# lisvulaczo/lodestar

Hardware: AMD Instinct MI355X
Metric: BLS signature sets verified/sec (whole node) at 1/2/4/8 MI355X; p50 batch latency (higher is better)
Workload: dtype u32

## Files before the change

include/lodestar_bls.h:

```cpp
#ifndef LODESTAR_BLS_H
#define LODESTAR_BLS_H

#include <stddef.h>
#include <stdint.h>

#ifdef __cplusplus
extern "C" {
#endif

#define LSG_OK 0
#define LSG_ERR_INVALID_ARG 1
#define LSG_ERR_NO_DEVICE 2
#define LSG_ERR_DEVICE 3
#define LSG_ERR_NOMEM 4
#define LSG_ERR_CLOSED 5
#define LSG_ERR_BUSY 6
#define LSG_ERR_ENTROPY 7

#define LSG_BLST_SUCCESS 0
#define LSG_BLST_BAD_ENCODING 1
#define LSG_BLST_POINT_NOT_ON_CURVE 2
#define LSG_BLST_POINT_NOT_IN_GROUP 3
#define LSG_BLST_AGGR_TYPE_MISMATCH 4
#define LSG_BLST_VERIFY_FAIL 5
// ... 98 lines not shown
int lsg_final_verify(lsg_ctx* ctx, const uint8_t* partials576, size_t n_partials, int32_t* valid);
int lsg_final_submit(lsg_ctx* ctx, const uint8_t* partials576, size_t n_partials, lsg_ticket* ticket);
int lsg_final_submit_device(lsg_ctx* ctx, const void* dev_partials576, size_t n_partials, lsg_ticket* ticket);
int lsg_final_wait(lsg_ctx* ctx, lsg_ticket ticket, int32_t* valid);
int lsg_final_submit_groups(lsg_ctx* ctx, const uint8_t* partials576, size_t n_groups, size_t per_group,
                            lsg_ticket* ticket);
int lsg_final_wait_groups(lsg_ctx* ctx, lsg_ticket ticket, int32_t* valid );

int lsg_pubkey_table_set(lsg_ctx* ctx, size_t first_index, const uint8_t* pks, uint32_t pk_len, size_t n,
                         int32_t* err);
int lsg_pubkey_table_size(lsg_ctx* ctx, size_t* n);

int lsg_committees_set(lsg_ctx* ctx, uint32_t first_id, const uint32_t* indices,
                       const uint32_t* offsets , size_t n_committees,
                       int32_t* err );
int lsg_committees_clear(lsg_ctx* ctx, uint32_t first_id, size_t n);
int lsg_committee_count(lsg_ctx* ctx, size_t* n);

typedef struct {
  uint64_t lookups, hits, pending, inserts, evictions, bypassed, full;
  uint32_t entries, capacity;
} lsg_msg_cache_stats;
int lsg_msg_cache_set(lsg_ctx* ctx, size_t capacity);
int lsg_msg_cache_clear(lsg_ctx* ctx);
int lsg_msg_cache_get_stats(lsg_ctx* ctx, lsg_msg_cache_stats* out);

int lsg_pubkey_validate(lsg_ctx* ctx, const uint8_t* pks, uint32_t pk_len, size_t n, uint8_t* out96, int32_t* err);

int lsg_aggregate_signatures(lsg_ctx* ctx, const uint8_t* sigs, uint32_t sig_len, const uint32_t* offsets,
                             size_t n_groups, uint8_t* out96, int32_t* err);

int lsg_signing_roots(lsg_ctx* ctx, const uint8_t* roots32, size_t n, const uint8_t* domain32, uint32_t domain_stride,
                      uint8_t* out32);
int lsg_attestation_signing_roots(lsg_ctx* ctx, const uint8_t* data128, size_t n, const uint8_t* domain32,
                                  uint32_t domain_stride, uint8_t* out32);
int lsg_deposit_signing_roots(lsg_ctx* ctx, const uint8_t* msgs88, size_t n, const uint8_t* domain32,
                              uint32_t domain_stride, uint8_t* out32);
int lsg_object_signing_roots(lsg_ctx* ctx, const uint8_t* objs, uint32_t obj_len, size_t n, const uint8_t* domain32,
                             uint32_t domain_stride, uint8_t* out32);

int lsg_verify_deposits(lsg_ctx* ctx, const uint8_t* data184, size_t n, const uint8_t* domain32, uint64_t seed,
                        uint8_t* valid, int32_t* err);

int lsg_sign(lsg_ctx* ctx, const uint8_t* sks32, const uint8_t* msgs, uint32_t msg_len, size_t n, uint8_t* out96);
int lsg_sk_to_pk(lsg_ctx* ctx, const uint8_t* sks32, size_t n, uint8_t* out96);

int lsg_check_fp2_mul(lsg_ctx* ctx, const uint32_t* in, size_t n, uint32_t* out);
int lsg_check_fp_sqr(lsg_ctx* ctx, const uint32_t* in, size_t n, uint32_t* out);
int lsg_check_fp2_sqr(lsg_ctx* ctx, const uint32_t* in, size_t n, uint32_t* out);
int lsg_check_sums(lsg_ctx* ctx, const uint32_t* in, size_t n, uint32_t* out);
int lsg_check_fp2_lanes(lsg_ctx* ctx, const uint32_t* in, size_t n, uint32_t* out);
int lsg_check_g2_lanes(lsg_ctx* ctx, const uint32_t* in, size_t n, uint32_t* out);
int lsg_check_mf_lanes(lsg_ctx* ctx, const uint32_t* in, size_t n, uint32_t* out);
int lsg_check_canon(lsg_ctx* ctx, const uint32_t* in, size_t n, const uint8_t* bytes48, size_t nb, uint32_t* out,
                    uint32_t* out_limbs);
int lsg_check_fp2_roots(lsg_ctx* ctx, const uint32_t* in, size_t n, uint32_t* out);
int lsg_check_batch_inv(lsg_ctx* ctx, const uint32_t* in, size_t n, uint32_t* out);
int lsg_check_map_uniform(lsg_ctx* ctx, const uint8_t* ub256, size_t n, uint8_t* out192);
int lsg_check_batch_partial_rnd(lsg_ctx* ctx, const lsg_set* sets, size_t n_sets,
                                const uint64_t* rnd , uint8_t* out576,
                                int32_t* set_err, int32_t* any_error);

int lsg_probe_fp_mul_rate(lsg_ctx* ctx, double* fp_mul_per_s, double* mad_per_s);

int lsg_probe_mad_peak(lsg_ctx* ctx, double* mad_per_s);

int lsg_last_kernel_times(lsg_ctx* ctx, const char** names, double* ms, int max);

#ifdef __cplusplus
}
#endif
#endif
```

lodestar_amd/_native.py:

```python
import ctypes
import os
import struct
import threading

HERE = os.path.dirname(os.path.abspath(__file__))
LIB_PATH = os.environ.get("LSG_LIB", os.path.join(HERE, "liblodestar_bls.so"))
AB_LIB_PATH = os.path.join(HERE, "liblodestar_bls_ab.so")

LSG_OK = 0
LSG_ERR_INVALID_ARG = 1
LSG_ERR_NO_DEVICE = 2
LSG_ERR_BUSY = 6
LSG_ERR_ENTROPY = 7

LSG_INVALID = 0
LSG_VALID = 1
LSG_ERROR = 2

LSG_JOB_BATCHABLE = 1
LSG_JOB_PRIORITY = 2
LSG_JOB_VALIDATE_KEYS = 4

BLST_NAMES = {
    0: "BLST_SUCCESS", 1: "BLST_BAD_ENCODING", 2: "BLST_POINT_NOT_ON_CURVE", 3: "BLST_POINT_NOT_IN_GROUP",
# ... 98 lines not shown
def _msg_form(msg):
    if isinstance(msg, MsgObject):
        b = msg.tobytes()
        return b, len(b) | LSG_MSG_OBJECT
    return msg, len(msg)


class LsgSet(ctypes.Structure):
    _fields_ = [
        ("pks", ctypes.c_void_p), ("pk_len", ctypes.c_uint32), ("n_pks", ctypes.c_uint32),
        ("msg", ctypes.c_void_p), ("msg_len", ctypes.c_uint32),
        ("sig", ctypes.c_void_p), ("sig_len", ctypes.c_uint32),
    ]


class LsgJob(ctypes.Structure):
    _fields_ = [("sets", ctypes.POINTER(LsgSet)), ("n_sets", ctypes.c_uint32), ("flags", ctypes.c_uint32)]


class LsgJobResult(ctypes.Structure):
    _fields_ = [("status", ctypes.c_int32), ("err_code", ctypes.c_int32)]


class LsgStats(ctypes.Structure):
    _fields_ = [
        ("batch_retries", ctypes.c_uint32), ("batch_sigs_success", ctypes.c_uint32),
        ("start_ns", ctypes.c_uint64), ("end_ns", ctypes.c_uint64),
        ("n_final_exps", ctypes.c_uint32), ("submit_us", ctypes.c_uint32),
        ("key_error", ctypes.c_int32), ("key_error_job", ctypes.c_uint32),
    ]


class LsgMsgCacheStats(ctypes.Structure):
    _fields_ = [(k, ctypes.c_uint64) for k in ("lookups", "hits", "pending", "inserts", "evictions", "bypassed",
                                                "full")] + [("entries", ctypes.c_uint32), ("capacity", ctypes.c_uint32)]


_lib = None
_lib_lock = threading.Lock()

EXPORTS = [
    "lsg_init", "lsg_init_devices", "lsg_destroy", "lsg_device_count", "lsg_last_error", "lsg_device_name",
    "lsg_reserve", "lsg_allocation_count", "lsg_verify_jobs", "lsg_verify_sets",
    "lsg_aggregate_pubkeys", "lsg_hash_to_g2", "lsg_sig_decode", "lsg_batch_partial", "lsg_final_verify",
    "lsg_probe_fp_mul_rate", "lsg_last_kernel_times", "lsg_sign", "lsg_sk_to_pk",
    "lsg_submit_jobs", "lsg_wait_jobs", "lsg_wait_jobs_node", "lsg_jobs_partial", "lsg_assign_jobs", "lsg_poll",
    "lsg_final_submit", "lsg_final_wait", "lsg_pipeline_slots", "lsg_probe_mad_peak",
    "lsg_pubkey_table_set", "lsg_pubkey_table_size", "lsg_pubkey_validate",
    "lsg_final_submit_groups", "lsg_final_wait_groups", "lsg_aggregate_signatures",
    "lsg_signing_roots", "lsg_attestation_signing_roots", "lsg_jobs_partial_device", "lsg_final_submit_device",
    "lsg_set_coalesce", "lsg_aggregate_pubkeys_multi", "lsg_check_fp2_mul",
    "lsg_check_fp_sqr", "lsg_check_fp2_sqr", "lsg_check_sums", "lsg_check_fp2_lanes", "lsg_check_g2_lanes", "lsg_check_mf_lanes",
    "lsg_check_canon", "lsg_check_fp2_roots", "lsg_check_batch_inv", "lsg_check_map_uniform",
    "lsg_check_batch_partial_rnd",
    "lsg_deposit_signing_roots", "lsg_verify_deposits",
    "lsg_committees_set", "lsg_committees_clear", "lsg_committee_count",
    "lsg_object_signing_roots",
    "lsg_submit_jobs_grouped", "lsg_wait_jobs_grouped",
    "lsg_msg_cache_set", "lsg_msg_cache_clear", "lsg_msg_cache_get_stats",
]


def load_library(path=LIB_PATH):
    global _lib
    with _lib_lock:
        if _lib is not None and path == LIB_PATH:
            return _lib
        if not os.path.exists(path):
            raise NativeUnavailable(f"{path} not built (run python -c 'import __graft_entry__; __graft_entry__.build()')")
        lib = ctypes.CDLL(path)
        vp, u32, u64, i32, sz = ctypes.c_void_p, ctypes.c_uint32, ctypes.c_uint64, ctypes.c_int32, ctypes.c_size_t
        pi32 = ctypes.POINTER(ctypes.c_int32)
        lib.lsg_init.argtypes = [ctypes.c_int, ctypes.POINTER(vp)]
        lib.lsg_init_devices.argtypes = [ctypes.POINTER(ctypes.c_int), ctypes.c_int, ctypes.POINTER(vp)]
        lib.lsg_device_count.argtypes = [vp, pi32]
        lib.lsg_reserve.argtypes = [vp, sz, sz, sz, i32]
        lib.lsg_allocation_count.argtypes = [vp, ctypes.POINTER(u64)]
        lib.lsg_wait_jobs_node.argtypes = [vp, u64, i32, ctypes.POINTER(LsgJobResult), ctypes.POINTER(LsgStats)]
        lib.lsg_jobs_partial.argtypes = [vp, u64, ctypes.c_char_p, pi32]
        lib.lsg_jobs_partial_device.argtypes = [vp, u64, vp, pi32]
        lib.lsg_final_submit_device.argtypes = [vp, vp, sz, ctypes.POINTER(u64)]
        lib.lsg_assign_jobs.argtypes = [ctypes.POINTER(u32), sz, i32, pi32]
        lib.lsg_destroy.argtypes = [vp]
        lib.lsg_last_error.argtypes = [vp]
        lib.lsg_last_error.restype = ctypes.c_char_p
        lib.lsg_device_name.argtypes = [vp, ctypes.c_char_p, sz]
        lib.lsg_verify_jobs.argtypes = [vp, ctypes.POINTER(LsgJob), sz, u64, ctypes.POINTER(LsgJobResult),
                                        ctypes.POINTER(LsgStats)]
        lib.lsg_verify_sets.argtypes = [vp, ctypes.POINTER(LsgSet), sz, u64, ctypes.POINTER(LsgJobResult)]
        lib.lsg_aggregate_pubkeys.argtypes = [vp, ctypes.c_char_p, u32, sz, ctypes.c_char_p, pi32]
        lib.lsg_aggregate_pubkeys_multi.argtypes = [vp, ctypes.POINTER(LsgSet), sz, ctypes.c_char_p, pi32]
        lib.lsg_hash_to_g2.argtypes = [vp, ctypes.c_char_p, u32, sz, ctypes.c_char_p, u32, ctypes.c_char_p]
        lib.lsg_sig_decode.argtypes = [vp, ctypes.c_char_p, u32, sz, ctypes.c_char_p, pi32]
        lib.lsg_batch_partial.argtypes = [vp, ctypes.POINTER(LsgSet), sz, u64, ctypes.c_char_p, pi32, pi32]
        lib.lsg_final_verify.argtypes = [vp, ctypes.c_char_p, sz, pi32]
        lib.lsg_probe_fp_mul_rate.argtypes = [vp, ctypes.POINTER(ctypes.c_double), ctypes.POINTER(ctypes.c_double)]
        lib.lsg_last_kernel_times.argtypes = [vp, ctypes.POINTER(ctypes.c_char_p), ctypes.POINTER(ctypes.c_double),
                                              ctypes.c_int]
        lib.lsg_sign.argtypes = [vp, ctypes.c_char_p, ctypes.c_char_p, u32, sz, ctypes.c_char_p]
        lib.lsg_sk_to_pk.argtypes = [vp, ctypes.c_char_p, sz, ctypes.c_char_p]
        pu64 = ctypes.POINTER(u64)
        lib.lsg_submit_jobs.argtypes = [vp, ctypes.POINTER(LsgJob), sz, u64, pu64]
        lib.lsg_wait_jobs.argtypes = [vp, u64, ctypes.POINTER(LsgJobResult), ctypes.POINTER(LsgStats)]
        lib.lsg_submit_jobs_grouped.argtypes = [vp, ctypes.POINTER(LsgJob), sz, u64, ctypes.POINTER(u32), sz, pu64]
        lib.lsg_wait_jobs_grouped.argtypes = [vp, u64, ctypes.POINTER(LsgJobResult), ctypes.POINTER(LsgStats),
                                              ctypes.c_char_p, ctypes.POINTER(u32)]
        lib.lsg_poll.argtypes = [vp, u64, pi32]
        lib.lsg_pubkey_table_set.argtypes = [vp, sz, ctypes.c_char_p, u32, sz, pi32]
        lib.lsg_pubkey_table_size.argtypes = [vp, ctypes.POINTER(sz)]
        lib.lsg_committees_set.argtypes = [vp, u32, ctypes.POINTER(u32), ctypes.POINTER(u32), sz, pi32]
        lib.lsg_committees_clear.argtypes = [vp, u32, sz]
        lib.lsg_committee_count.argtypes = [vp, ctypes.POINTER(sz)]
        lib.lsg_msg_cache_set.argtypes = [vp, sz]
        lib.lsg_msg_cache_clear.argtypes = [vp]
        lib.lsg_msg_cache_get_stats.argtypes = [vp, ctypes.POINTER(LsgMsgCacheStats)]
        lib.lsg_final_submit_groups.argtypes = [vp, ctypes.c_char_p, sz, sz, pu64]
        lib.lsg_final_wait_groups.argtypes = [vp, u64, pi32]
        lib.lsg_pubkey_validate.argtypes = [vp, ctypes.c_char_p, u32, sz, ctypes.c_char_p, pi32]
        lib.lsg_signing_roots.argtypes = [vp, ctypes.c_char_p, sz, ctypes.c_char_p, u32, ctypes.c_char_p]
        lib.lsg_attestation_signing_roots.argtypes = [vp, ctypes.c_char_p, sz, ctypes.c_char_p, u32, ctypes.c_char_p]
        lib.lsg_deposit_signing_roots.argtypes = [vp, ctypes.c_char_p, sz, ctypes.c_char_p, u32, ctypes.c_char_p]
        lib.lsg_object_signing_roots.argtypes = [vp, ctypes.c_char_p, u32, sz, ctypes.c_char_p, u32, ctypes.c_char_p]
        lib.lsg_verify_deposits.argtypes = [vp, ctypes.c_char_p, sz, ctypes.c_char_p, u64, ctypes.c_char_p, pi32]
        lib.lsg_aggregate_signatures.argtypes = [vp, ctypes.c_char_p, u32, ctypes.POINTER(u32), sz,
                                                 ctypes.c_char_p, pi32]
        lib.lsg_final_submit.argtypes = [vp, ctypes.c_char_p, sz, pu64]
        lib.lsg_final_wait.argtypes = [vp, u64, pi32]
        lib.lsg_pipeline_slots.argtypes = [vp, pi32]
        lib.lsg_set_coalesce.argtypes = [vp, u32, i32]
        lib.lsg_check_fp2_mul.argtypes = [vp, ctypes.c_char_p, sz, ctypes.c_char_p]
        lib.lsg_check_fp_sqr.argtypes = [vp, ctypes.c_char_p, sz, ctypes.c_char_p]
        lib.lsg_check_fp2_sqr.argtypes = [vp, ctypes.c_char_p, sz, ctypes.c_char_p]
        lib.lsg_check_sums.argtypes = [vp, ctypes.c_char_p, sz, ctypes.c_char_p]
        lib.lsg_check_fp2_lanes.argtypes = [vp, ctypes.c_char_p, sz, ctypes.c_char_p]
        lib.lsg_check_g2_lanes.argtypes = [vp, ctypes.c_char_p, sz, ctypes.c_char_p]
        lib.lsg_check_mf_lanes.argtypes = [vp, ctypes.c_char_p, sz, ctypes.c_char_p]
        lib.lsg_check_canon.argtypes = [vp, ctypes.c_char_p, sz, ctypes.c_char_p, sz, ctypes.c_char_p, ctypes.c_char_p]
        lib.lsg_check_fp2_roots.argtypes = [vp, ctypes.c_char_p, sz, ctypes.c_char_p]
        lib.lsg_check_batch_inv.argtypes = [vp, ctypes.c_char_p, sz, ctypes.c_char_p]
        lib.lsg_check_map_uniform.argtypes = [vp, ctypes.c_char_p, sz, ctypes.c_char_p]
        lib.lsg_check_batch_partial_rnd.argtypes = [vp, ctypes.POINTER(LsgSet), sz, ctypes.POINTER(u64),
                                                    ctypes.c_char_p, pi32, pi32]
        lib.lsg_probe_mad_peak.argtypes = [vp, ctypes.POINTER(ctypes.c_double)]
        for name in EXPORTS:
            if name != "lsg_last_error":
                getattr(lib, name).restype = ctypes.c_int
        if path == LIB_PATH:
            _lib = lib
        return lib


class SetBuffer:

    def __init__(self, sets):
        self._keep = []
        sets = list(sets)
        self.arr = (LsgSet * max(len(sets), 1))()
        for i, (pks, msg, sig) in enumerate(sets):
            pk_len, n_pks, pkb = _key_form(pks)
            msg, msg_len = _msg_form(msg)
            for b in (pkb, msg, sig):
                self._keep.append(b)
            s = self.arr[i]
            s.pks = ctypes.cast(ctypes.c_char_p(pkb), ctypes.c_void_p) if pkb else None
            s.pk_len = pk_len
            s.n_pks = n_pks
            s.msg = ctypes.cast(ctypes.c_char_p(msg), ctypes.c_void_p) if msg else None
            s.msg_len = msg_len
            s.sig = ctypes.cast(ctypes.c_char_p(sig), ctypes.c_void_p) if sig else None
            s.sig_len = len(sig)
        self.n = len(sets)


def assign_jobs(job_sizes, n_devices):
    lib = load_library()
    n = len(job_sizes)
    sizes = (ctypes.c_uint32 * max(n, 1))(*job_sizes)
    owner = (ctypes.c_int32 * max(n, 1))()
    rc = lib.lsg_assign_jobs(sizes, n, int(n_devices), owner)
    if rc != LSG_OK:
        raise ValueError(f"lsg_assign_jobs failed ({rc})")
    return list(owner[:n])


class PreparedJobs:

    def __init__(self, jobs):
        import numpy as np
        flat = [st for sets, _ in jobs for st in sets]
# ... 447 lines not shown
        out = ctypes.create_string_buffer(96 * len(sks))
        skb = b"".join(int(k).to_bytes(32, "big") for k in sks)
        self._check(self.lib.lsg_sk_to_pk(self.h, skb, len(sks), out), "lsg_sk_to_pk")
        raw = out.raw
        return [raw[96 * i:96 * i + 96] for i in range(len(sks))]

    def check_fp2_mul(self, words):
        n = len(words) // 56
        assert len(words) == 56 * n
        out = ctypes.create_string_buffer(4 * 28 * n)
        src = struct.pack(f"<{len(words)}I", *words)
        self._check(self.lib.lsg_check_fp2_mul(self.h, src, n, out), "lsg_check_fp2_mul")
        return list(struct.unpack(f"<{28 * n}I", out.raw))

    def _check_sqr(self, fn, words, per_item):
        n = len(words) // per_item
        assert len(words) == per_item * n
        out = ctypes.create_string_buffer(4 * per_item * n)
        src = struct.pack(f"<{len(words)}I", *words)
        self._check(getattr(self.lib, fn)(self.h, src, n, out), fn)
        return list(struct.unpack(f"<{per_item * n}I", out.raw))

    def check_fp_sqr(self, words):
        return self._check_sqr("lsg_check_fp_sqr", words, 14)

    def check_fp2_sqr(self, words):
        return self._check_sqr("lsg_check_fp2_sqr", words, 28)

    def check_sums(self, words):
        n = len(words) // (12 * 14)
        assert len(words) == 12 * 14 * n
        out = ctypes.create_string_buffer(4 * 42 * 14 * n)
        src = struct.pack(f"<{len(words)}I", *words)
        self._check(self.lib.lsg_check_sums(self.h, src, n, out), "lsg_check_sums")
        return list(struct.unpack(f"<{42 * 14 * n}I", out.raw))

    def _check_lanes(self, fn, words):
        n = len(words) // (12 * 14)
        assert len(words) == 12 * 14 * n
        out = ctypes.create_string_buffer(4 * 24 * 14 * n)
        src = struct.pack(f"<{len(words)}I", *words)
        self._check(getattr(self.lib, fn)(self.h, src, n, out), fn)
        return list(struct.unpack(f"<{24 * 14 * n}I", out.raw))

    def check_fp2_lanes(self, words):
        return self._check_lanes("lsg_check_fp2_lanes", words)

    def check_g2_lanes(self, words):
        return self._check_lanes("lsg_check_g2_lanes", words)

    def check_mf_lanes(self, words):
        return self._check_lanes("lsg_check_mf_lanes", words)

    def check_canon(self, words, strings=()):
        n, nb = len(words) // 14, len(strings)
        assert len(words) == 14 * n and all(len(b) == 48 for b in strings)
        out = ctypes.create_string_buffer(4 * 54 * max(n, 1))
        limbs = ctypes.create_string_buffer(4 * 14 * max(nb, 1))
        src = struct.pack(f"<{len(words)}I", *words)
        self._check(self.lib.lsg_check_canon(self.h, src, n, b"".join(strings), nb, out, limbs), "lsg_check_canon")
        return (list(struct.unpack(f"<{54 * n}I", out.raw[:4 * 54 * n])),
                list(struct.unpack(f"<{14 * nb}I", limbs.raw[:4 * 14 * nb])))

    def check_fp2_roots(self, words):
        n = len(words) // 28
        assert len(words) == 28 * n
        out = ctypes.create_string_buffer(4 * 58 * n)
        src = struct.pack(f"<{len(words)}I", *words)
        self._check(self.lib.lsg_check_fp2_roots(self.h, src, n, out), "lsg_check_fp2_roots")
        return list(struct.unpack(f"<{58 * n}I", out.raw))

    def check_batch_inv(self, words):
        return self._check_sqr("lsg_check_batch_inv", words, 14)

    def check_map_uniform(self, items):
        n = len(items)
        assert all(len(b) == 256 for b in items)
        if not n:
            return []
        out = ctypes.create_string_buffer(192 * n)
        self._check(self.lib.lsg_check_map_uniform(self.h, b"".join(items), n, out), "lsg_check_map_uniform")
        raw = out.raw
        return [raw[192 * i:192 * i + 192] for i in range(n)]

    def batch_partial_rnd(self, sets, rnd):
        b = SetBuffer(sets)
        assert len(rnd) == b.n
        r = (ctypes.c_uint64 * max(b.n, 1))(*[int(x) for x in rnd])
        out = ctypes.create_string_buffer(576)
        errs = (ctypes.c_int32 * max(b.n, 1))()
        anyerr = ctypes.c_int32()
        self._check(self.lib.lsg_check_batch_partial_rnd(self.h, b.arr, b.n, r, out, errs, ctypes.byref(anyerr)),
                    "lsg_check_batch_partial_rnd")
        return out.raw, [errs[i] for i in range(b.n)], bool(anyerr.value)

    def probe_fp_mul_rate(self):
        a, b = ctypes.c_double(), ctypes.c_double()
        self._check(self.lib.lsg_probe_fp_mul_rate(self.h, ctypes.byref(a), ctypes.byref(b)), "lsg_probe_fp_mul_rate")
        return a.value, b.value

    def last_kernel_times(self, max_entries=1024):
        names = (ctypes.c_char_p * max_entries)()
        ms = (ctypes.c_double * max_entries)()
        n = self.lib.lsg_last_kernel_times(self.h, names, ms, max_entries)
        return [(names[i].decode(), ms[i]) for i in range(n)]
```

lodestar_amd/csrc/lsg_ab.h:

```cpp
#pragma once
#include <stdlib.h>
#include <string.h>

#ifdef LSG_AB
static inline long lsg_ab_long(const char* name, long dflt) {
  const char* e = getenv(name);
  return e ? atol(e) : dflt;
}
static inline bool lsg_ab_str_is(const char* name, const char* v) {
  const char* e = getenv(name);
  return e && strcmp(e, v) == 0;
}
#else
#define lsg_ab_long(name, dflt) ((long)(dflt))
#define lsg_ab_str_is(name, v) false
#endif
```

lodestar_amd/csrc/lsg_curve.hpp:

```cpp
#pragma once
#include "lsg_tower.hpp"

LSG_INL fp_t fadd(const fp_t& a, const fp_t& b) { return fp_add(a, b); }
LSG_INL fp2_t fadd(const fp2_t& a, const fp2_t& b) { return fp2_add(a, b); }
LSG_INL fp_t fsub(const fp_t& a, const fp_t& b) { return fp_sub(a, b); }
LSG_INL fp2_t fsub(const fp2_t& a, const fp2_t& b) { return fp2_sub(a, b); }
LSG_INL fp_t fmul(const fp_t& a, const fp_t& b) { return fp_mul(a, b); }
LSG_INL fp2_t fmul(const fp2_t& a, const fp2_t& b) { return fp2_mul(a, b); }
LSG_INL fp_t fsqr(const fp_t& a) { return fp_sqr(a); }
LSG_INL fp2_t fsqr(const fp2_t& a) { return fp2_sqr(a); }
LSG_INL fp_t fneg(const fp_t& a) { return fp_neg(a); }
LSG_INL fp2_t fneg(const fp2_t& a) { return fp2_neg(a); }
LSG_INL fps_t<1, 0> fsum(const fp_t& a) { return fps(a); }
LSG_INL fp2s_t<1, 0> fsum(const fp2_t& a) { return fp2s(a); }
template <int K, int P, int N>
LSG_INL fps_t<K * P, K * N> fsum_mulk(const fps_t<P, N>& a) { return fps_mulk<K>(a); }
template <int K, int P0, int N0, int P1, int N1>
LSG_INL fp2s_t<K * P0, K * N0, K * P1, K * N1> fsum_mulk(const fp2s_t<P0, N0, P1, N1>& a) { return fp2s_mulk<K>(a); }
template <int K> LSG_INL fp_t fmulk(const fp_t& a) { return fp_mulk<K>(a); }
template <int K> LSG_INL fp2_t fmulk(const fp2_t& a) { return fp2_mulk<K>(a); }
template <class F> LSG_INL F fsub2(const F& a, const F& b, const F& c) { return (fsum(a) - b - c).carry(); }
LSG_INL fp_t fmul_b3(const fp_t& a) { return fp_mul12(a); }
LSG_INL fp2_t fmul_b3(const fp2_t& a) { return fp2_mul_b3(a); }
template <int P0, int N0, int P1, int N1>
// ... 438 lines not shown
  g2p_t r;
  r.X = fp2_mul_fp(p.X, PSI2_CX);
  r.Y = fp2_mul_fp(p.Y, PSI2_CY);
  r.Z = p.Z;
  return r;
}

template <class F = fp2_t, class G>
LSG_INL bool g2_in_group_get(const G& get) {
  if (proj_is_inf(get())) return true;
  const proj_t<F> xp = proj_neg(proj_mul_xabs_get<F>(get));
  return proj_eq(g2_psi(g2_to_pair(get())), g2_to_pair(xp));
}
LSG_BIGFN bool g2_in_group(g2p_t p) {
  return g2_in_group_get([&]() { return p; });
}

LSG_BIGFN bool g1_in_group(g1p_t p) {
  const uint32_t rw[8] = {0x73eda753u, 0x299d7d48u, 0x3339d808u, 0x09a1d805u,
                          0x53bda402u, 0xfffe5bfeu, 0xffffffffu, 0x00000001u};
  g1p_t acc = proj_inf<fp_t>();
#pragma unroll 1
  for (int w = 0; w < 8; w++) {
#pragma unroll 1
    for (int b = 31; b >= 0; b--) {
      acc = g1_dbl(acc);
      if ((rw[w] >> b) & 1u) acc = g1_add(acc, p);
    }
  }
  return proj_is_inf(acc);
}

LSG_INL bool g1_on_curve_aff(const g1a_t& a) {
  fp_t rhs = fp_add(fp_mul(fp_sqr(a.x), a.x), FP_B_G1);
  return fp_eq(fp_sqr(a.y), rhs);
}
LSG_INL bool g2_on_curve_aff(const g2a_t& a) {
  fp2_t rhs = fp2_add(fp2_mul(fp2_sqr(a.x), a.x), FP2_B_G2);
  return fp2_eq(fp2_sqr(a.y), rhs);
}

#ifndef LSG_BLST_SUCCESS
#define LSG_BLST_SUCCESS 0
#define LSG_BLST_BAD_ENCODING 1
#define LSG_BLST_POINT_NOT_ON_CURVE 2
#define LSG_BLST_POINT_NOT_IN_GROUP 3
#define LSG_BLST_AGGR_TYPE_MISMATCH 4
#define LSG_BLST_VERIFY_FAIL 5
#define LSG_BLST_PK_IS_INFINITY 6
#define LSG_BLST_BAD_SCALAR 7
#define LSG_BLST_INVALID_SIZE 10
#endif

LSG_INL int g2_uncompress(g2a_t& out, bool& inf, const uint8_t* in) {
  uint8_t in0 = in[0];
  inf = false;
  if (!(in0 & 0x80)) return LSG_BLST_BAD_ENCODING;
  if (in0 & 0x40) {
    uint32_t acc = in0 & 0x3f;
    for (int i = 1; i < 96; i++) acc |= in[i];
    if (acc == 0) {
      inf = true;
      out.x = fp2_zero();
      out.y = fp2_zero();
      return LSG_BLST_SUCCESS;
    }
    return LSG_BLST_BAD_ENCODING;
  }
  fp_t x1 = fp_from_be48(in);
  x1 = fp_mask_flags(x1);
  fp_t x0 = fp_from_be48(in + 48);
  if (!fp_canon_lt_p(x1) || !fp_canon_lt_p(x0)) return LSG_BLST_BAD_ENCODING;
  fp2_t x = fp2_make(fp_to_mont(x0), fp_to_mont(x1));
  fp2_t rhs = fp2_add(fp2_mul(fp2_sqr(x), x), FP2_B_G2);
  fp2_t y;
  if (!fp2_sqrt(y, rhs)) return LSG_BLST_POINT_NOT_ON_CURVE;
  bool want = (in0 & 0x20) != 0;
  if (fp2_lexi_largest(y) != want) y = fp2_neg(y);
  out.x = x;
  out.y = y;
  if (fp2_is_zero(x)) return LSG_BLST_POINT_NOT_IN_GROUP;
  return LSG_BLST_SUCCESS;
}

LSG_INL int g2_deserialize_uncompressed(g2a_t& out, bool& inf, const uint8_t* in) {
  uint8_t in0 = in[0];
  inf = false;
  if (in0 & 0x80) return LSG_BLST_BAD_ENCODING;
  if (in0 & 0x40) {
    uint32_t acc = in0 & 0x3f;
    for (int i = 1; i < 192; i++) acc |= in[i];
    if (acc == 0) {
      inf = true;
      out.x = fp2_zero();
      out.y = fp2_zero();
      return LSG_BLST_SUCCESS;
    }
    return LSG_BLST_BAD_ENCODING;
  }
  if (in0 & 0x20) return LSG_BLST_BAD_ENCODING;
  fp_t v[4];
  for (int k = 0; k < 4; k++) {
    v[k] = fp_from_be48(in + 48 * k);
    if (k == 0) v[k] = fp_mask_flags(v[k]);
    if (!fp_canon_lt_p(v[k])) return LSG_BLST_BAD_ENCODING;
  }
  out.x = fp2_make(fp_to_mont(v[1]), fp_to_mont(v[0]));
  out.y = fp2_make(fp_to_mont(v[3]), fp_to_mont(v[2]));
  if (!g2_on_curve_aff(out)) return LSG_BLST_POINT_NOT_ON_CURVE;
  if (fp2_is_zero(out.x)) return LSG_BLST_POINT_NOT_IN_GROUP;
  return LSG_BLST_SUCCESS;
}

LSG_INL int g1_deserialize(g1a_t& out, bool& inf, const uint8_t* in, int len) {
  uint8_t in0 = in[0];
  inf = false;
  bool compressed = (in0 & 0x80) != 0;
  if (compressed != (len == 48)) return LSG_BLST_BAD_ENCODING;
  if (in0 & 0x40) {
    uint32_t acc = in0 & 0x3f;
    for (int i = 1; i < len; i++) acc |= in[i];
    if (acc == 0) {
      inf = true;
      out.x = fp_zero();
      out.y = fp_zero();
      return LSG_BLST_SUCCESS;
    }
    return LSG_BLST_BAD_ENCODING;
  }
  if (!compressed && (in0 & 0x20)) return LSG_BLST_BAD_ENCODING;
  fp_t x = fp_from_be48(in);
  x = fp_mask_flags(x);
  if (!fp_canon_lt_p(x)) return LSG_BLST_BAD_ENCODING;
  out.x = fp_to_mont(x);
  if (compressed) {
// ... 49 lines not shown
```

lodestar_amd/csrc/lsg_fp2_lanes.hpp:

```cpp
#pragma once

constexpr int LSG_VL = 14;

#if LSG_PAIR_G == 2
#define LSG_LANES_HIDE(x) asm volatile("" : "+v"(x))
#else
#define LSG_LANES_HIDE(x) ((void)0)
#endif

LSG_PFN void lanes_carry64(int64_t* t) {
#pragma unroll
  for (int j = 0; j < LSG_VL - 1; j++) {
    t[j + 1] += t[j] >> 29;
    t[j] &= (int64_t)LSG_M29;
  }
}
LSG_PFN void lanes_reduce_step(int64_t* t, const uint32_t* p, int i) {
  uint32_t m = ((uint32_t)t[0] * LSG_N0P) & LSG_M29;
  LSG_LANES_HIDE(m);
#pragma unroll
  for (int j = 0; j < LSG_VL; j++) t[j] += (int64_t)(int32_t)m * (int32_t)p[j];
  const int64_t c = t[0] >> 29;
#pragma unroll
  for (int j = 0; j < LSG_VL - 1; j++) t[j] = t[j + 1];
  t[0] += c;
  t[LSG_VL - 1] = 0;
  if (i == 6) lanes_carry64(t);
}
LSG_PFN void lanes_tail(int64_t* t, uint32_t* r) {
  lanes_carry64(t);
#pragma unroll
  for (int j = 0; j < LSG_VL; j++) r[j] = (uint32_t)t[j];
}
template <class OTHER>
LSG_PFN void lanes_sop_pass(uint32_t* r, const uint32_t* P, const uint32_t* Q, const uint32_t* b, const OTHER& other) {
  uint32_t p[LSG_VL];
#pragma unroll
  for (int j = 0; j < LSG_VL; j++) p[j] = LSG_P[j];
  int64_t t[LSG_VL];
#pragma unroll
  for (int j = 0; j < LSG_VL; j++) t[j] = 0;
#pragma unroll
  for (int i = 0; i < LSG_VL; i++) {
    uint32_t bo = b[i], bs = other(i, b[i]);
    LSG_LANES_HIDE(bo);
    LSG_LANES_HIDE(bs);
#pragma unroll
    for (int j = 0; j < LSG_VL; j++) t[j] += (int64_t)(int32_t)P[j] * (int32_t)bo;
#pragma unroll
    for (int j = 0; j < LSG_VL; j++) t[j] += (int64_t)(int32_t)Q[j] * (int32_t)bs;
    lanes_reduce_step(t, p, i);
  }
  lanes_tail(t, r);
}
LSG_PFN void lanes_mul_pass(uint32_t* r, const uint32_t* V, const uint32_t* s) {
  uint32_t p[LSG_VL];
#pragma unroll
  for (int j = 0; j < LSG_VL; j++) p[j] = LSG_P[j];
  int64_t t[LSG_VL];
#pragma unroll
  for (int j = 0; j < LSG_VL; j++) t[j] = 0;
#pragma unroll
  for (int i = 0; i < LSG_VL; i++) {
    uint32_t si = s[i];
    LSG_LANES_HIDE(si);
#pragma unroll
    for (int j = 0; j < LSG_VL; j++) t[j] += (int64_t)(int32_t)V[j] * (int32_t)si;
    lanes_reduce_step(t, p, i);
  }
  lanes_tail(t, r);
}
LSG_PFN void lanes_mul_operand(uint32_t& P, uint32_t& Q, uint32_t own, uint32_t partner, bool odd) {
  P = odd ? partner : own;
  Q = odd ? own : 0u - partner;
}
LSG_PFN void lanes_sqr_operand(uint32_t& V, uint32_t& s, uint32_t own, uint32_t partner, bool odd) {
  V = odd ? own : own + partner;
  s = odd ? partner + partner : own - partner;
}
LSG_PFN uint32_t lanes_xi_operand(uint32_t own, uint32_t partner, bool odd) { return odd ? own + partner : own - partner; }

#if LSG_PAIR_G == 2 && !defined(LSG_NO_FP2_LANES)
#define LSG_FP2_LANES 1
struct fp2v_t {
  uint32_t l[LSG_VL];
};
LSG_PFN bool lanes_odd() { return pair_h() != 0u; }
LSG_PFN uint32_t lanes_swap(uint32_t x) {
  return (uint32_t)__builtin_amdgcn_update_dpp(0, (int)x, 0xB1, 0xf, 0xf, true);
}

typedef uint32_t lanes8_t __attribute__((ext_vector_type(8)));
typedef uint32_t lanes4_t __attribute__((ext_vector_type(4)));
typedef uint32_t lanes2_t __attribute__((ext_vector_type(2)));
#define LSG_LANES_PARAMS(x) lanes8_t x##_a, lanes4_t x##_b, lanes2_t x##_c
#define LSG_LANES_ARGS(v) lanes_pack8(v), lanes_pack4(v), lanes_pack2(v)
#define LSG_LANES_UNPACK(x) lanes_unpack(x##_a, x##_b, x##_c)
LSG_PFN lanes8_t lanes_pack8(const fp2v_t& a) {
  return lanes8_t{a.l[0], a.l[1], a.l[2], a.l[3], a.l[4], a.l[5], a.l[6], a.l[7]};
}
LSG_PFN lanes4_t lanes_pack4(const fp2v_t& a) { return lanes4_t{a.l[8], a.l[9], a.l[10], a.l[11]}; }
LSG_PFN lanes2_t lanes_pack2(const fp2v_t& a) { return lanes2_t{a.l[12], a.l[13]}; }
LSG_PFN fp2v_t lanes_unpack(const lanes8_t& a, const lanes4_t& b, const lanes2_t& c) {
  fp2v_t r;
#pragma unroll
  for (int k = 0; k < 8; k++) r.l[k] = a[k];
#pragma unroll
  for (int k = 0; k < 4; k++) r.l[8 + k] = b[k];
  r.l[12] = c[0];
  r.l[13] = c[1];
  return r;
}

LSG_PLEAF fp2v_t lanes_fp2_mul_v(LSG_LANES_PARAMS(va), LSG_LANES_PARAMS(vb)) {
  const fp2v_t a = LSG_LANES_UNPACK(va), b = LSG_LANES_UNPACK(vb);
  const bool odd = lanes_odd();
  uint32_t P[LSG_VL], Q[LSG_VL];
#pragma unroll
  for (int k = 0; k < LSG_VL; k++) {
    lanes_mul_operand(P[k], Q[k], a.l[k], lanes_swap(a.l[k]), odd);
    LSG_LANES_HIDE(P[k]);
    LSG_LANES_HIDE(Q[k]);
  }
  fp2v_t r;
// ... 198 lines not shown
```

lodestar_amd/csrc/lsg_h2c.hpp:

```cpp
#pragma once
#include "lsg_curve.hpp"

#include "lsg_ssz.hpp"

struct sha256_ctx {
  uint32_t st[8];
  uint32_t blk[16];
  uint32_t n;
  uint32_t total;
};

LSG_INL void sha256_init(sha256_ctx& c) {
  c.st[0] = 0x6a09e667u;
  c.st[1] = 0xbb67ae85u;
  c.st[2] = 0x3c6ef372u;
  c.st[3] = 0xa54ff53au;
  c.st[4] = 0x510e527fu;
  c.st[5] = 0x9b05688cu;
  c.st[6] = 0x1f83d9abu;
  c.st[7] = 0x5be0cd19u;
  for (int i = 0; i < 16; i++) c.blk[i] = 0;
  c.n = 0;
  c.total = 0;
}
// ... 18 lines not shown
  uint32_t bits = c.total * 8;
  sha256_byte(c, 0x80);
  while (c.n != 56) sha256_byte(c, 0);
  c.blk[14] = 0;
  c.blk[15] = bits;
  sha256_compress(c.st, c.blk);
  for (int i = 0; i < 8; i++) out8[i] = c.st[i];
}

LSG_INL void expand_message_xmd_256(uint8_t* out, const uint8_t* msg, uint32_t msg_len, const uint8_t* dst,
                                    uint32_t dst_len) {
  sha256_ctx c;
  uint32_t b0[8], bi[8];
  sha256_init(c);
  for (int i = 0; i < 64; i++) sha256_byte(c, 0);
  sha256_bytes(c, msg, msg_len);
  sha256_byte(c, 1);
  sha256_byte(c, 0);
  sha256_byte(c, 0);
  sha256_bytes(c, dst, dst_len);
  sha256_byte(c, (uint8_t)dst_len);
  sha256_final(c, b0);
  for (int i = 1; i <= 8; i++) {
    sha256_init(c);
    for (int k = 0; k < 8; k++) {
      uint32_t v = (i == 1) ? b0[k] : (b0[k] ^ bi[k]);
      sha256_byte(c, (uint8_t)(v >> 24));
      sha256_byte(c, (uint8_t)(v >> 16));
      sha256_byte(c, (uint8_t)(v >> 8));
      sha256_byte(c, (uint8_t)v);
    }
    sha256_byte(c, (uint8_t)i);
    sha256_bytes(c, dst, dst_len);
    sha256_byte(c, (uint8_t)dst_len);
    sha256_final(c, bi);
    be_words_to_bytes(out + 32 * (i - 1), bi, 8);
  }
}

LSG_INL fp_t fp_from_be64_mod(const uint8_t* b) {
  fp_t lo = fp_from_be_bytes(b + 32, 8);
  fp_t mid = fp_from_be_bytes(b + 16, 4);
  fp_t hi = fp_from_be_bytes(b, 4);
  return fp_add(fp_add(fp_mul(lo, fp_t(FP_R2)), fp_mul(mid, fp_t(FP_R2_SHL256))), fp_mul(hi, fp_t(FP_R3)));
}

LSG_INL fp2_t sswu_tv1(const fp2_t& u) {
  fp2_t zu2 = fp2_mul(SSWU_Z, fp2_sqr(u));
  return fp2_add(fp2_sqr(zu2), zu2);
}
LSG_INL fp2_t fp2_inv_with_norm_inv(const fp2_t& a, const fp_t& ni) {
  return fp2_t(fp_mul(a.c0, ni), fp_neg(fp_mul(a.c1, ni)));
}
LSG_BIGFN g2a_t map_to_curve_sswu_ni(fp2_t u, fp_t ni) {
  fp2_t u2 = fp2_sqr(u);
  fp2_t zu2 = fp2_mul(SSWU_Z, u2);
  fp2_t tv1 = fp2_add(fp2_sqr(zu2), zu2);
  bool exc = fp2_is_zero(tv1);
  fp2_t x1 = fp2_mul(SSWU_MINUS_B_OVER_A, fp2_add(fp2_one(), fp2_inv_with_norm_inv(tv1, ni)));
  x1 = fp2_select(exc, SSWU_B_OVER_ZA, x1);
  fp2_t gx1 = fp2_add(fp2_mul(fp2_add(fp2_sqr(x1), SSWU_A), x1), SSWU_B);
  fp2_t x2 = fp2_mul(zu2, x1);
  fp2_t gx2 = fp2_add(fp2_mul(fp2_add(fp2_sqr(x2), SSWU_A), x2), SSWU_B);
  bool sq1;
  fp_t s1 = fp2_norm_sqrt_candidate(gx1, &sq1);
  fp_t s2 = fp_mul(fp_mul(fp2_norm(zu2), fp2_norm(u)), fp_mul(s1, fp_t(SSWU_NZ_POW_P1D4)));
  g2a_t r;
  r.x = fp2_select(sq1, x1, x2);
  fp2_t y;
  (void)fp2_sqrt_with_norm_root(y, fp2_select(sq1, gx1, gx2), fp_select(sq1, s1, s2));
  if (fp2_sgn0(u) != fp2_sgn0(y)) y = fp2_neg(y);
  r.y = y;
  return r;
}
LSG_BIGFN g2a_t map_to_curve_sswu(fp2_t u) { return map_to_curve_sswu_ni(u, fp_inv(fp2_norm(sswu_tv1(u)))); }

LSG_BIGFN g2p_t iso_map3(g2a_t p) {
  const fp2_t& x = p.x;
  fp2_t xn = fp2_add(fp2_mul(fp2_add(fp2_mul(fp2_add(fp2_mul(ISO_XNUM_3, x), ISO_XNUM_2), x), ISO_XNUM_1), x),
                     ISO_XNUM_0);
  fp2_t xd = fp2_add(fp2_mul(fp2_add(x, ISO_XDEN_1), x), ISO_XDEN_0);
  fp2_t yn = fp2_add(fp2_mul(fp2_add(fp2_mul(fp2_add(fp2_mul(ISO_YNUM_3, x), ISO_YNUM_2), x), ISO_YNUM_1), x),
                     ISO_YNUM_0);
  fp2_t yd = fp2_add(fp2_mul(fp2_add(fp2_mul(fp2_add(x, ISO_YDEN_2), x), ISO_YDEN_1), x), ISO_YDEN_0);
  g2p_t r;
  r.X = fp2_mul(xn, yd);
  r.Y = fp2_mul(fp2_mul(p.y, yn), xd);
  r.Z = fp2_mul(xd, yd);
  if (fp2_is_zero(r.Z)) r = proj_inf<fp2_t>();
  return r;
}

LSG_BIGFN g2p_t clear_cofactor_g2(g2p_t p) {
  const g2p_t u = g2_psi(p);
  g2p_t c = g2_add(g2_psi2(g2_dbl(p)), proj_neg(u));
  c = g2_add(c, proj_neg(p));
  const g2p_t t1 = proj_neg(proj_mul_xabs(p));
  c = g2_add(c, proj_neg(t1));
  const g2p_t t2 = proj_neg(proj_mul_xabs(g2_add(t1, u)));
  return g2_add(c, t2);
}
template <bool LANES = false, class G, class P, class CP, class CG>
LSG_INL g2p_t clear_cofactor_g2_parked(const G& get, const P& put, const CP& cput, const CG& cget) {
  auto xabs = [&]() {
#ifdef LSG_FP2_LANES
    if (LANES) return g2_mul_xabs_get_dbl_lanes(get);
#endif
    return proj_mul_xabs_get<fp2_t>(get);
  };
  cput(proj_neg(xabs()));
  g2p_t c;
  {
    const g2p_t p = get();
    c = g2_add(g2_psi2(g2_dbl(p)), proj_neg(p));
    put(g2_psi(p));
  }
  c = g2_add(c, proj_neg(get()));
  const g2p_t t1 = cget();
  cput(g2_add(c, proj_neg(t1)));
  put(g2_add(t1, get()));
  const g2p_t t2 = proj_neg(xabs());
  return g2_add(cget(), t2);
}
```

lodestar_amd/csrc/lsg_host.hip:

```cpp
#include <hip/hip_runtime.h>
#include <rccl/rccl.h>
#include <stdio.h>
#include <stdlib.h>
#include <errno.h>
#include <string.h>
#include <sys/random.h>
#include <time.h>

#include <algorithm>
#include <atomic>
#include <condition_variable>
#include <chrono>
#include <mutex>
#include <shared_mutex>
#include <thread>
#include <unordered_map>
#include <string>
#include <vector>

#include "../../include/lodestar_bls.h"
#include "lsg_launch.h"
#include "lsg_layout.h"
#include "lsg_serial.h"
#include "lsg_ab.h"
// ... 80 lines not shown
  SLOT_MERGE = 4
};

struct PendingPkg {
  uint64_t serial = 0, seed = 0;
  size_t n_sets = 0;
  std::vector<lsg_job> jobs;
  std::vector<lsg_set> sets;
  std::vector<uint8_t> data;
};
struct MergeTicket {
  int slot = -1;
  int sub = -1;
  int rc = 0;
  std::string err;
};

struct Dev;

constexpr int64_t LSG_ITEMS_PER_BLOCK_HOST = 128;
struct AggPlan {
  bool tree = false;
  int L = 0, T = 1;
  int64_t n_c0 = 0, N0 = 0;
  size_t blk_off = 0, o0_off = 0, len_off = 0, pk0_off = 0, src_off = 0;
};
constexpr size_t AGG_TREE_MIN_KEYS = 32768;

struct Slot : Staged {
  Dev* d = nullptr;
  int index = 0;
  hipStream_t st[2] = {nullptr, nullptr};
  bool own_streams = true;
  hipStream_t st_norm[2] = {nullptr, nullptr}, st_prio[2] = {nullptr, nullptr};
  int cur = 0;
  hipEvent_t ev_xp = nullptr;
  hipEvent_t ev_in = nullptr, ev_sig = nullptr, ev_grp = nullptr, ev_part = nullptr, ev_done = nullptr,
             ev_node = nullptr;
  DevBuf d_sig, d_siglen, d_msg, d_msgoff, d_msglen, d_pk, d_pklen, d_rnd, d_mode, d_dst;
  HostBuf h_arena;
  MsgTable mtab;
  bool mc_ok = false;
  DevBuf d_Hx, d_hinfx;
  SegPlan msum;
  DevBuf d_mmask, d_PmP, d_Pm, d_pinfm, d_errm;
  BitsPlan bplan;
  HostBuf h_cbits;
  DevBuf d_cbits;
  MultiPlan mplan;
  size_t n_kv = 0, kv_off = 0;
  DevBuf d_ub, d_sigaff, d_siginf, d_seterr, d_pkp, d_pkerr, d_agg, d_P, d_pinf, d_H, d_hinf, d_rs, d_rs2, d_fall,
      d_fall2;
  DevBuf d_Pp, d_zP, d_zPi, d_U, d_nrm, d_nrmi, d_Hp, d_zN, d_zNi, d_mid, d_Hm, d_hinfm;
  DevBuf binv_lv[2], binv_iv[2];
  DevBuf d_lines;
  bool rs2_ready = false;
  std::vector<uint8_t> rs2_scaled;
  std::vector<uint8_t> rs_raw;
  DevBuf d_S, d_F, d_verdict, d_Sb, d_fgb, d_Fb, d_bkt, d_bits, d_aux, d_gath, d_nodeF, d_nodeV;
  DevBuf seg_tmp[3][2];
  std::vector<int32_t> plan;
  HostBuf h_plan;
  DevBuf d_plan;
  PhasePlan phA;
  SegPlan pkagg;
  AggPlan agg;
  DevBuf d_agga, d_aggi, d_aggpre, d_aggtot, d_aggflag;
  SegPlan phA_node;
  HostBuf h_mode;
  HostBuf h_err, h_pinf, h_pkerr, h_verdict, h_blob, h_nodeV;
  std::vector<Timer> timers;
  size_t ntimers = 0;
  int kind = SLOT_FREE;
  uint64_t serial = 0;
  GroupPlan gp;
  Switches sw;
  int K = 4;
  std::vector<lsg_job_result> results;
  lsg_stats stats;
  bool has_node = false;
  size_t n_jobs = 0;
  uint64_t seed = 0;
  DevBuf d_xport;
  HostBuf h_xport;
  bool big_fe_pending = false;
  std::vector<uint64_t> sub_serial;
  std::vector<lsg_stats> sub_stats;
  std::vector<int32_t> sub_pkfail;
  std::vector<uint8_t> sub_done;
  bool resolved = false, resolving = false;
  int resolve_rc = LSG_OK;
  size_t grp_n = 0;
  std::vector<uint32_t> set_grp;
  std::vector<int32_t> gplan;
  SigGroupPlan sgp;
  HostBuf h_gplan, h_gagg;
  DevBuf d_gplan, d_gsum, d_gagg, d_gtmp[2];
};

struct Dev {
  lsg_ctx* c = nullptr;
  int device = 0;
  int ord = 0;
  hipStream_t s_util = nullptr;
  hipStream_t s_fe[LSG_FE_STREAMS] = {};
  hipStream_t s_xp = nullptr, s_nfe = nullptr;
// ... 174 lines not shown
hipError_t event_wait(hipEvent_t e) {
  const auto t0 = std::chrono::steady_clock::now();
  for (;;) {
    const hipError_t r = hipEventQuery(e);
    if (r != hipErrorNotReady) return r;
    if (std::chrono::steady_clock::now() - t0 > std::chrono::microseconds(20))
      std::this_thread::sleep_for(std::chrono::microseconds(30));
  }
}

bool blocking_waits() {
  const char* e = getenv("LSG_BLOCKING_WAITS");
  return e && atoi(e) != 0;
}

int slot_create(Dev* d, Slot* s, int index, hipStream_t shared) {
  s->d = d;
  s->index = index;
  if (shared) {
    s->st[0] = s->st[1] = shared;
    s->own_streams = false;
  } else {
    for (int k = 0; k < 2; k++) LSG_HIP(s, hipStreamCreateWithFlags(&s->st_norm[k], hipStreamNonBlocking));
    s->st[0] = s->st_norm[0];
    s->st[1] = s->st_norm[1];
  }
  hipEvent_t* evs[] = {&s->ev_in, &s->ev_sig, &s->ev_grp, &s->ev_part, &s->ev_done, &s->ev_node, &s->ev_xp};
  for (hipEvent_t* e : evs) LSG_HIP(s, hipEventCreateWithFlags(e, hipEventDisableTiming));
  if (blocking_waits()) {
    for (hipEvent_t* e : {&s->ev_part, &s->ev_done}) {
      LSG_HIP(s, hipEventDestroy(*e));
      LSG_HIP(s, hipEventCreateWithFlags(e, hipEventDisableTiming | hipEventBlockingSync));
    }
  }
  LSG_RC(ensure(s, s->d_dst, 256));
  LSG_HIP(s, hipMemcpy(s->d_dst.p, DST_POP, DST_POP_LEN, hipMemcpyHostToDevice));
  return LSG_OK;
}

void slot_destroy(Slot* s) {
  if (!s->d) return;
  for (int k = 0; k < 2; k++)
    if (s->st[k]) (void)hipStreamSynchronize(s->st[k]);
  DevBuf* bufs[] = {&s->d_sig,  &s->d_siglen, &s->d_msg,  &s->d_msgoff, &s->d_msglen, &s->d_pk,    &s->d_pklen,
                    &s->d_rnd,  &s->d_mode,   &s->d_dst,  &s->d_ub,     &s->d_sigaff, &s->d_siginf, &s->d_seterr,
                    &s->d_pkp,  &s->d_pkerr,  &s->d_agg,  &s->d_P,      &s->d_pinf,   &s->d_H,     &s->d_hinf,
                    &s->d_rs,   &s->d_rs2,    &s->d_fall, &s->d_fall2,  &s->d_Pp,     &s->d_zP,    &s->d_zPi,
                    &s->d_U,    &s->d_nrm,    &s->d_nrmi, &s->d_Hp,     &s->d_zN,     &s->d_zNi,   &s->binv_lv[0],
                    &s->binv_lv[1], &s->binv_iv[0], &s->binv_iv[1], &s->d_lines, &s->d_S, &s->d_F, &s->d_verdict,
                    &s->d_Sb,   &s->d_fgb,    &s->d_Fb,   &s->d_bkt,    &s->d_bits,   &s->d_aux,   &s->d_gath,
                    &s->d_nodeF, &s->d_nodeV, &s->d_plan, &s->d_mid, &s->d_Hm, &s->d_hinfm,
                    &s->d_mmask, &s->d_PmP, &s->d_Pm, &s->d_pinfm, &s->d_errm, &s->d_xport,
                    &s->d_agga, &s->d_aggi, &s->d_aggpre, &s->d_aggtot, &s->d_aggflag, &s->d_cbits,
                    &s->d_gplan, &s->d_gsum, &s->d_gagg, &s->d_gtmp[0], &s->d_gtmp[1], &s->d_Hx, &s->d_hinfx};
  for (DevBuf* b : bufs) free_dev(*b);
  for (auto& u : s->seg_tmp)
    for (DevBuf& b : u) free_dev(b);
  HostBuf* hb[] = {&s->h_arena, &s->h_err, &s->h_pinf, &s->h_pkerr, &s->h_verdict, &s->h_blob, &s->h_plan, &s->h_nodeV,
                   &s->h_xport, &s->h_cbits, &s->h_gplan, &s->h_gagg};
  for (HostBuf* b : hb) free_host(*b);
  for (Timer& t : s->timers) {
    (void)hipEventDestroy(t.a);
    (void)hipEventDestroy(t.b);
  }
  s->timers.clear();
  hipEvent_t evs[] = {s->ev_in, s->ev_sig, s->ev_grp, s->ev_part, s->ev_done, s->ev_node, s->ev_xp};
  for (hipEvent_t e : evs)
    if (e) (void)hipEventDestroy(e);
  if (s->own_streams) {
    for (int k = 0; k < 2; k++) {
      if (s->st_prio[k]) (void)hipStreamSynchronize(s->st_prio[k]);
      if (s->st_norm[k]) (void)hipStreamSynchronize(s->st_norm[k]);
    }
    for (int k = 0; k < 2; k++) {
      if (s->st_norm[k]) (void)hipStreamDestroy(s->st_norm[k]);
      s->st_norm[k] = s->st_prio[k] = s->st[k] = nullptr;
    }
  }
  s->d = nullptr;
}

int slot_streams(Slot* s, bool prio) {
  if (!s->own_streams) return LSG_OK;
  if (prio && !s->st_prio[0]) {
    Dev* d = s->d;
    for (int k = 0; k < 2; k++) LSG_RC(prio_stream(d->c, d, &d->s_pp[k]));
    s->st_prio[0] = d->s_pp[0];
    s->st_prio[1] = d->s_pp[1];
  }
  hipStream_t* p = prio ? s->st_prio : s->st_norm;
  s->st[0] = p[0];
  s->st[1] = p[1];
  return LSG_OK;
}

int slot_ready(Dev* d, Slot* s, int index) {
  if (s->d) return LSG_OK;
  const int rc = slot_create(d, s, index, nullptr);
  if (rc) slot_destroy(s);
  return rc;
}

bool miller_fused() { return lsg_ab_long("LSG_MILLER_FUSED", 1) != 0; }
static bool mf_lanes_on() { return lsg_ab_long("LSG_MF_LANES", 1) != 0; }

size_t slp_items_max();
int miller_k_for(size_t n_sets) {
// ... 29 lines not shown
  size_t a, b;
  binv_sizes(n, &a, &b);
  return a;
}
size_t binv_iv_words(size_t n) {
  size_t a, b;
  binv_sizes(n, &a, &b);
  return b;
}

int size_inputs(Slot* s, size_t n, size_t np, size_t mb) {
  const size_t nn = std::max(n, (size_t)1), pp = std::max(np, (size_t)1);
  LSG_RC(ensure_host(s, s->h_arena, stage_layout(n, np, 96, mb).bytes));
  LSG_RC(ensure(s, s->d_sig, 192 * nn));
  LSG_RC(ensure(s, s->d_siglen, 4 * nn));
  LSG_RC(ensure(s, s->d_msg, std::max(mb, (size_t)1)));
  LSG_RC(ensure(s, s->d_msgoff, 4 * nn));
  LSG_RC(ensure(s, s->d_msglen, 4 * nn));
  LSG_RC(ensure(s, s->d_pk, 96 * pp));
  LSG_RC(ensure(s, s->d_pklen, 4 * pp));
  LSG_RC(ensure(s, s->d_rnd, 8 * nn));
  LSG_RC(ensure(s, s->d_mode, nn));
  LSG_RC(ensure(s, s->d_mid, 4 * nn));
  return LSG_OK;
}

int size_state(Slot* s, size_t n, size_t np, size_t ng, size_t n_msm, int pkg = 0) {
  const size_t nn = std::max(n, (size_t)1), pp = std::max(np, (size_t)1), gg = std::max(ng, (size_t)1);
  const size_t g_msm = std::max(n_msm, (size_t)1);
  struct {
    DevBuf* b;
    size_t bytes;
  } dev[] = {{&s->d_ub, 256 * nn},
             {&s->d_sigaff, 4 * W_G2A * nn},
             {&s->d_siginf, nn},
             {&s->d_seterr, 4 * nn},
             {&s->d_pkp, 4 * W_G1P * pp},
             {&s->d_pkerr, 4 * pp},
             {&s->d_agg, 4 * W_G1P * nn},
             {&s->d_P, 4 * W_G1A * nn},
             {&s->d_pinf, nn},
             {&s->d_H, 4 * W_G2A * nn},
             {&s->d_hinf, nn},
             {&s->d_rs, 4 * W_G2P * nn},
             {&s->d_Pp, 4 * W_G1P * nn},
             {&s->d_zP, 4 * W_FP * nn},
             {&s->d_zPi, 4 * W_FP * nn},
             {&s->d_U, 4 * W_H2CU * nn},
             {&s->d_nrm, 4 * W_FP * 2 * nn},
             {&s->d_nrmi, 4 * W_FP * 2 * nn},
             {&s->d_Hp, 4 * W_G2P * nn},
             {&s->d_zN, 4 * W_FP * nn},
             {&s->d_zNi, 4 * W_FP * nn},
             {&s->binv_lv[0], 4 * W_FP * binv_lv_words(2 * nn)},
             {&s->binv_iv[0], 4 * W_FP * binv_iv_words(2 * nn)},
             {&s->binv_lv[1], 4 * W_FP * binv_lv_words(nn)},
             {&s->binv_iv[1], 4 * W_FP * binv_iv_words(nn)},
             {&s->d_S, 4 * W_G2P * gg},
             {&s->d_F, 4 * W_F12 * gg},
             {&s->d_verdict, 4 * gg},
             {&s->d_Sb, (size_t)288 * (MSM_BITS * g_msm + gg)},
             {&s->d_fgb, 576 * gg},
             {&s->d_Fb, 576 * gg},
             {&s->d_bkt, 4 * W_G2P * (size_t)MSM_WINDOWS * MSM_DIGITS * g_msm},
             {&s->d_bits, 4 * W_G2P * (size_t)MSM_BITS * g_msm},
             {&s->d_gath, 576 * (LSG_MAX_DEVICES + 2)},
             {&s->d_nodeF, 4 * W_F12 * (LSG_MAX_DEVICES + 1)},
             {&s->d_nodeV, 64}};
  for (auto& x : dev) LSG_RC(ensure(s, *x.b, x.bytes));
  if (pkg == 1) {
    if (!miller_fused()) LSG_RC(ensure(s, s->d_lines, 4 * (size_t)ML_STEPS * W_LINE * nn));
    LSG_RC(ensure(s, s->d_fall, 4 * W_F12 * (2 * nn + gg + 2)));
  }
  if (pkg) {
    LSG_RC(ensure(s, s->d_fall2, 4 * W_F12 * (nn + std::max(gg, nn))));
    LSG_RC(ensure(s, s->d_rs2, 4 * W_G2P * nn));
  }
  LSG_RC(ensure_host(s, s->h_err, 4 * nn));
  LSG_RC(ensure_host(s, s->h_pinf, nn));
  LSG_RC(ensure_host(s, s->h_pkerr, 4 * pp));
  LSG_RC(ensure_host(s, s->h_verdict, 4 * gg));
  LSG_RC(ensure_host(s, s->h_blob, 576 * gg));
  LSG_RC(ensure_host(s, s->h_nodeV, 64));
  return LSG_OK;
}

int size_seg(Slot* s, int use, const SegPlan& P) {
  if (P.tmp_items == 0) return LSG_OK;
  const size_t W = P.op == 0 ? W_G1P : (P.op == 1 ? W_G2P : W_F12);
  LSG_RC(ensure(s, s->seg_tmp[use][0], 4 * W * P.tmp_items));
  return ensure(s, s->seg_tmp[use][1], 4 * W * P.tmp_items);
}

int upload_plan(Slot* s) {
  const size_t bytes = 4 * std::max(s->plan.size(), (size_t)1);
  LSG_RC(ensure_host(s, s->h_plan, bytes));
  LSG_RC(ensure(s, s->d_plan, bytes));
  if (!s->plan.empty()) {
    memcpy(s->h_plan.p, s->plan.data(), 4 * s->plan.size());
    LSG_HIP(s, hipMemcpyAsync(s->d_plan.p, s->h_plan.p, 4 * s->plan.size(), hipMemcpyHostToDevice, s->st[0]));
  }
  return LSG_OK;
}

int run_seg(Slot* s, int use, const char* name, const SegPlan& P, const uint32_t* src, uint32_t* dst) {
  LSG_RC(size_seg(s, use, P));
// ... 23 lines not shown
      KL(s, "g1_aggregate", lsgk::seg_reduce(S_(s), 0, q.n_chunks, q.ips_log2, PL(s, q.chunk_off), nullptr,
                                             tmp[q.src], dst, tmp[q.tmp_out]));
  }
  return LSG_OK;
}

int size_groups(Slot* s, size_t n, size_t ng) {
  const size_t words = 2 * n + 3 * ng + 64, tmp_items = n / 8 + 64;
  LSG_RC(ensure_host(s, s->h_gplan, 4 * words));
  LSG_RC(ensure(s, s->d_gplan, 4 * words));
  for (DevBuf& b : s->d_gtmp) LSG_RC(ensure(s, b, 4 * W_G2P * tmp_items));
  LSG_RC(ensure(s, s->d_gsum, 4 * W_G2P * std::max(ng, (size_t)1)));
  LSG_RC(ensure(s, s->d_gagg, 96 * std::max(ng, (size_t)1)));
  LSG_RC(ensure_host(s, s->h_gagg, 96 * std::max(ng, (size_t)1)));
  s->gplan.reserve(words);
  return LSG_OK;
}

int run_sig_groups(Slot* s, const uint8_t* mask) {
  const size_t ng = s->grp_n;
  s->gplan.clear();
  s->sgp = plan_sig_groups(s->gplan, s->set_grp.data(), s->n_sets, ng, mask,
                           (int)lsg_ab_long("LSG_SEG_FOLD_WIDE", SEG_FOLD_WIDE));
  const SegPlan& P = s->sgp.seg;
  const size_t bytes = 4 * std::max(s->gplan.size(), (size_t)1);
  LSG_RC(ensure_host(s, s->h_gplan, bytes));
  LSG_RC(ensure(s, s->d_gplan, bytes));
  for (DevBuf& b : s->d_gtmp) LSG_RC(ensure(s, b, 4 * W_G2P * std::max(P.tmp_items, (size_t)1)));
  LSG_RC(ensure(s, s->d_gsum, 4 * W_G2P * ng));
  LSG_RC(ensure(s, s->d_gagg, 96 * ng));
  LSG_RC(ensure_host(s, s->h_gagg, 96 * ng));
  memcpy(s->h_gplan.p, s->gplan.data(), 4 * s->gplan.size());
  LSG_HIP(s, hipMemcpyAsync(s->d_gplan.p, s->h_gplan.p, 4 * s->gplan.size(), hipMemcpyHostToDevice, S_(s)));
  const int32_t* A = P_<int32_t>(s->d_gplan);
  uint32_t* tmp[3] = {nullptr, P_<uint32_t>(s->d_gtmp[0]), P_<uint32_t>(s->d_gtmp[1])};
  uint32_t* dst = P_<uint32_t>(s->d_gsum);
  for (size_t k = 0; k < P.passes.size(); k++) {
    const SegPass& q = P.passes[k];
    if (k == 0)
      KL(s, "k_sig_agg_seg", lsgk::sig_agg_seg(S_(s), q.n_chunks, q.ips_log2, A + q.chunk_off, A + s->sgp.gather_off,
                                               P_<uint32_t>(s->d_sigaff), P_<uint8_t>(s->d_siginf),
                                               P_<int32_t>(s->d_seterr), dst, tmp[q.tmp_out]));
    else
      KL(s, "sig_agg_reduce", lsgk::seg_reduce(S_(s), 1, q.n_chunks, q.ips_log2, A + q.chunk_off, nullptr, tmp[q.src], dst,
                                               tmp[q.tmp_out]));
  }
  KL(s, "k_g2p_compress", lsgk::g2p_compress(S_(s), (int)ng, dst, P_<uint8_t>(s->d_gagg)));
  LSG_HIP(s, hipMemcpyAsync(s->h_gagg.p, s->d_gagg.p, 96 * ng, hipMemcpyDeviceToHost, S_(s)));
  return LSG_OK;
}

static bool binv_block_on() { return lsg_ab_long("LSG_BINV_BLOCK", 1) != 0; }
static bool fp2_lanes_on() { return lsg_ab_long("LSG_FP2_LANES", 1) != 0; }
int launch_sig_subgroup(Slot* s, int n) {
  if (fp2_lanes_on())
    KL(s, "k_sig_subgroup", lsgk::sig_subgroup(S_(s), n, P_<uint32_t>(s->d_sigaff), P_<uint8_t>(s->d_siginf),
                                               P_<int32_t>(s->d_seterr)));
  else
    KL(s, "k_sig_subgroup_pair", lsgk::sig_subgroup(S_(s), n, P_<uint32_t>(s->d_sigaff), P_<uint8_t>(s->d_siginf),
                                                    P_<int32_t>(s->d_seterr), true));
  return LSG_OK;
}

void binv_sizes(size_t n, size_t* lv, size_t* iv) {
  size_t a = 0, b = 0;
  for (size_t m = n; m > 1;) {
    const size_t up = (m + LSG_BINV_T - 1) / LSG_BINV_T;
    a += m + up;
    b += up;
    m = up;
  }
  *lv = std::max(a, (size_t)1);
  *iv = std::max(b, (size_t)1);
}

int batch_inv(Slot* s, int ws, const char* name, const uint32_t* v, size_t n, uint32_t* out) {
  if (n == 0) return LSG_OK;
  size_t lvw, ivw;
  binv_sizes(n, &lvw, &ivw);
  LSG_RC(ensure(s, s->binv_lv[ws], 4 * W_FP * lvw));
  LSG_RC(ensure(s, s->binv_iv[ws], 4 * W_FP * ivw));
  uint32_t* lv = P_<uint32_t>(s->binv_lv[ws]);
  uint32_t* iv = P_<uint32_t>(s->binv_iv[ws]);
  if (binv_block_on()) {
    const int T = (int)std::min<size_t>(64, std::max<size_t>(1, (n + 128 * 64 - 1) / (128 * 64)));
    KL(s, name, lsgk::binv_block(S_(s), (int)n, T, 1, v, lv, out));
    return LSG_OK;
  }
  std::vector<size_t> cnt{n};
  std::vector<uint32_t*> val{(uint32_t*)v}, pre, inv{out};
  size_t lo = 0, io = 0;
  while (cnt.back() > 1) {
    const size_t m = cnt.back(), up = (m + LSG_BINV_T - 1) / LSG_BINV_T;
    pre.push_back(lv + W_FP * lo);
    lo += m;
    val.push_back(lv + W_FP * lo);
    lo += up;
    inv.push_back(iv + W_FP * io);
    io += up;
    cnt.push_back(up);
  }
  const size_t L = cnt.size() - 1;
  if (L == 0) {
    KL(s, name, lsgk::binv_root(S_(s), v, out));
    return LSG_OK;
  }
  for (size_t l = 0; l < L; l++)
    KL(s, name, lsgk::binv_fold(S_(s), (int)cnt[l], l == 0 ? 1 : 0, val[l], pre[l], val[l + 1]));
  KL(s, name, lsgk::binv_root(S_(s), val[L], inv[L]));
  for (size_t l = L; l-- > 0;)
    KL(s, name, lsgk::binv_unfold(S_(s), (int)cnt[l], l == 0 ? 1 : 0, val[l], pre[l], inv[l + 1], inv[l]));
  return LSG_OK;
}


size_t slp_items_max() {
  const long v = lsg_ab_long("LSG_SLP_ITEMS", 2048);
  return lsg_serial_mode() == LSG_SERIAL_SLP && v > 0 ? (size_t)v : 0;
}

int launch_hash(Slot* s, int n, uint32_t* H, uint8_t* hinf) {
  KL(s, "k_h2c_prep", lsgk::h2c_prep(S_(s), n, P_<uint8_t>(s->d_ub), P_<uint32_t>(s->d_U), P_<uint32_t>(s->d_nrm)));
  LSG_RC(batch_inv(s, 0, "binv_sswu", P_<uint32_t>(s->d_nrm), 2 * (size_t)n, P_<uint32_t>(s->d_nrmi)));
  KL(s, "k_h2c_map", lsgk::h2c_map(S_(s), n, P_<uint32_t>(s->d_U), P_<uint32_t>(s->d_nrmi), P_<uint32_t>(s->d_Hp)));
  if ((size_t)n <= slp_items_max()) {
    KL(s, "k_slp_h2c", lsg_slp_h2c_clear(S_(s), n, P_<uint32_t>(s->d_Hp), H, hinf));
    return LSG_OK;
  }
  if (fp2_lanes_on())
    KL(s, "k_h2c_clear", lsgk::h2c_clear(S_(s), n, P_<uint32_t>(s->d_Hp), P_<uint32_t>(s->d_zN), hinf));
  else
    KL(s, "k_h2c_clear_pair", lsgk::h2c_clear(S_(s), n, P_<uint32_t>(s->d_Hp), P_<uint32_t>(s->d_zN), hinf, true));
  LSG_RC(batch_inv(s, 0, "binv_hash", P_<uint32_t>(s->d_zN), (size_t)n, P_<uint32_t>(s->d_zNi)));
  KL(s, "k_h2c_affine", lsgk::h2c_affine(S_(s), n, P_<uint32_t>(s->d_Hp), P_<uint32_t>(s->d_zNi), hinf, H));
  return LSG_OK;
}

int stage_sets(Slot* s, const lsg_set* const* sets, size_t n, uint64_t seed, bool scale,
               const std::vector<uint8_t>* noscale = nullptr, bool dedup = false, bool bits_ok = false,
               const uint64_t* rnd_in = nullptr) {
  const StageSizes z = stage_measure(sets, n, bits_ok);
  if (z.n_bits_sets + z.n_multi) {
    LSG_RC(ensure_host(s, s->h_cbits, 4 * z.bit_words));
    LSG_RC(ensure(s, s->d_cbits, 4 * z.bit_words));
  }
  LSG_RC(size_inputs(s, n, z.npk, z.msg_total));
  const StageLayout L = stage_layout(n, z.npk, z.pk_stride(), z.msg_total);
  static const bool dedup_on = lsg_ab_long("LSG_MSG_DEDUP", 1) != 0;
  StageOpts o;
  o.scale = scale;
  o.noscale = noscale;
  o.dedup = dedup;
  o.dedup_on = dedup_on;
  o.bits_ok = bits_ok;
  o.rnd_in = rnd_in;
  o.seed = seed;
  const lsg_ctx* c = s->d->c;
  const Committees cm{c->cm_len.data(), c->cm_ok.data(), c->cm_ok.size()};
  uint8_t* A = H_<uint8_t>(s->h_arena);
  uint32_t* cbits = H_<uint32_t>(s->h_cbits);
  const int rc = stage_fill(A, L, cbits, sets, n, z, o, s->mc_ok ? &s->d->mc : nullptr, cm, s->mtab, s->plan, *s, MsgKey(),
                            os_random);
  if (rc == LSG_ERR_ENTROPY) set_err(s->d->c, "no entropy for the RLC randomizers (getrandom failed)");
  LSG_RC(rc);
  hipStream_t S = s->st[0];
  struct {
    DevBuf* d;
    size_t off, len;
  } cp[] = {{&s->d_sig, L.sig, 192 * L.nn},      {&s->d_siglen, L.siglen, 4 * L.nn},
            {&s->d_msg, L.msg, std::max(s->mc_on ? s->msg_used : z.msg_total, (size_t)1)},
            {&s->d_msgoff, L.msgoff, 4 * L.nn}, {&s->d_msglen, L.msglen, 4 * L.nn}, {&s->d_pk, L.pk, L.stride * L.np},
            {&s->d_pklen, L.pklen, 4 * L.np},   {&s->d_rnd, L.rnd, 8 * L.nn}};
  for (auto& x : cp) LSG_HIP(s, hipMemcpyAsync(x.d->p, A + x.off, x.len, hipMemcpyHostToDevice, S));
  if (s->msg_dedup) LSG_HIP(s, hipMemcpyAsync(s->d_mid.p, A + L.mid, 4 * n, hipMemcpyHostToDevice, S));
  if (s->bit_words) LSG_HIP(s, hipMemcpyAsync(s->d_cbits.p, cbits, 4 * s->bit_words, hipMemcpyHostToDevice, S));
  return LSG_OK;
}
// ... 81 lines not shown
  }
  KL(s, "k_blobs_to_fp12", lsgk::blobs_to_fp12(S_(s), (int)ng, P_<uint8_t>(s->d_fgb), fall + W_F12 * Ph.term_base));
  LSG_HIP(s, hipEventRecord(s->ev_grp, s->st[1]));
  s->cur = 0;
  LSG_HIP(s, hipStreamWaitEvent(s->st[0], s->ev_grp, 0));
  LSG_RC(run_seg(s, 2, "fp12_product", Ph.prod, fall, P_<uint32_t>(s->d_F)));
  KL(s, "k_fp12_to_canon", lsgk::fp12_to_canon(S_(s), (int)ng, P_<uint32_t>(s->d_F), P_<uint8_t>(s->d_Fb)));
  if (export_blobs) LSG_HIP(s, hipMemcpyAsync(s->h_blob.p, s->d_Fb.p, 576 * ng, hipMemcpyDeviceToHost, s->st[0]));
  LSG_HIP(s, hipEventRecord(s->ev_part, s->st[0]));
  return LSG_OK;
}

int launch_fe_range(Slot* s, size_t g0, size_t g1) {
  if (g1 <= g0) return LSG_OK;
  s->cur = 0;
  const size_t ng = g1 - g0;
  KL(s, SERIAL_LABEL(final_exp),
     lsg_row_final_exp(S_(s), (int)ng, P_<uint8_t>(s->d_Fb) + 576 * g0, P_<int32_t>(s->d_verdict) + g0));
  LSG_HIP(s, hipMemcpyAsync(H_<int32_t>(s->h_verdict) + g0, P_<int32_t>(s->d_verdict) + g0, 4 * ng,
                            hipMemcpyDeviceToHost, s->st[0]));
  return LSG_OK;
}
int launch_fe(Slot* s, size_t ng) { return launch_fe_range(s, 0, ng); }

int launch_agg_tree(Slot* s, const AggPlan& P, uint32_t* agg);

int launch_set_stages(Slot* s, const SegPlan* pkagg, const PhasePlan& Ph, uint32_t* fall) {
  const size_t n_items = Ph.agg_g >= 0 ? Ph.n_set_items : Ph.n_items, item_off = Ph.item_off;
  const int n = (int)s->n_sets, np = (int)s->n_pks;
  if (n == 0) return LSG_OK;
  Dev* d = s->d;
  LSG_HIP(s, hipEventRecord(s->ev_in, s->st[0]));
  s->cur = 1;
  LSG_HIP(s, hipStreamWaitEvent(s->st[1], s->ev_in, 0));
  if (!s->single_keys && s->agg.tree) {
    LSG_RC(launch_agg_tree(s, s->agg, P_<uint32_t>(s->d_agg)));
  } else if (s->single_keys) {
    if (np > 0)
      KL(s, "k_pk_decode", lsgk::pk_decode(S_(s), np, P_<uint8_t>(s->d_pk), s->pk_stride, P_<uint32_t>(s->d_pklen),
                                           P_<uint32_t>(s->d_agg), P_<int32_t>(s->d_pkerr), P_<uint32_t>(d->d_pktab),
                                           P_<uint8_t>(d->d_pktab_ok), (uint32_t)d->pktab_n));
  } else if (!s->pk_all_bits) {
    LSG_RC(run_pk_seg(s, *pkagg, P_<uint32_t>(s->d_agg)));
  }
  LSG_RC(run_pk_bits(s, P_<uint32_t>(s->d_agg)));
  LSG_RC(run_pk_multi(s, P_<uint32_t>(s->d_agg)));
  if (s->n_kv)
    KL(s, "k_pk_keyvalidate", lsgk::pk_keyvalidate(S_(s), (int)s->n_kv, PL(s, s->kv_off), P_<uint8_t>(s->d_pk),
                                                   P_<uint32_t>(s->d_pklen), P_<int32_t>(s->d_pkp)));
  KL(s, "k_pk_scale", lsgk::pk_scale(S_(s), n, P_<uint32_t>(s->d_agg), P_<uint64_t>(s->d_rnd), P_<uint32_t>(s->d_Pp),
                                     P_<uint32_t>(s->d_zP), P_<uint8_t>(s->d_pinf)));
  LSG_RC(batch_inv(s, 1, "binv_pk", P_<uint32_t>(s->d_zP), (size_t)n, P_<uint32_t>(s->d_zPi)));
  KL(s, "k_pk_affine", lsgk::pk_affine(S_(s), n, P_<uint32_t>(s->d_Pp), P_<uint32_t>(s->d_zPi), P_<uint32_t>(s->d_P)));
  KL(s, "k_sig_decode", lsgk::sig_decode(S_(s), n, P_<uint8_t>(s->d_sig), P_<uint32_t>(s->d_siglen),
                                         P_<uint32_t>(s->d_sigaff), P_<uint8_t>(s->d_siginf), P_<int32_t>(s->d_seterr)));
  if ((size_t)n <= slp_items_max())
    KL(s, "k_slp_subgroup", lsg_slp_g2_subgroup(S_(s), n, P_<uint32_t>(s->d_sigaff), P_<uint8_t>(s->d_siginf),
                                                P_<int32_t>(s->d_seterr)));
  else
    LSG_RC(launch_sig_subgroup(s, n));
  if (s->n_kv)
    KL(s, "k_pk_keyvalidate_apply", lsgk::pk_keyvalidate_apply(S_(s), (int)s->n_kv, PL(s, s->kv_off + s->n_kv),
                                                               P_<int32_t>(s->d_pkp), P_<int32_t>(s->d_seterr)));
  if (Ph.agg_g >= 0) {
    const Grp& g = Ph.groups[(size_t)Ph.agg_g];
    const size_t nm = Ph.n_magg;
    LSG_RC(ensure(s, s->d_mmask, 4 * W_G1P * std::max(g.first + g.len, (size_t)1)));
    LSG_RC(ensure(s, s->d_PmP, 4 * W_G1P * nm));
    LSG_RC(ensure(s, s->d_Pm, 4 * W_G1A * nm));
    LSG_RC(ensure(s, s->d_pinfm, nm));
    LSG_RC(ensure(s, s->d_errm, 4 * nm));
    KL(s, "k_pk_mask", lsgk::pk_mask(S_(s), (int)(g.first + g.len), P_<uint32_t>(s->d_Pp), P_<int32_t>(s->d_seterr),
                                     P_<uint8_t>(s->d_pinf), P_<uint32_t>(s->d_mmask)));
    LSG_RC(run_seg(s, 0, "msg_pk_sums", s->msum, P_<uint32_t>(s->d_mmask), P_<uint32_t>(s->d_PmP)));
    KL(s, "k_g1p_affine_inv", lsgk::g1p_affine_inv(S_(s), (int)nm, P_<uint32_t>(s->d_PmP), P_<uint32_t>(s->d_Pm),
                                                   P_<uint8_t>(s->d_pinfm)));
    LSG_HIP(s, hipMemsetAsync(s->d_errm.p, 0, 4 * nm, s->st[1]));
  }
  LSG_HIP(s, hipEventRecord(s->ev_sig, s->st[1]));
  s->cur = 0;
  const int nm = (int)s->n_msgs;
  if (s->mc_on && (s->mc_hits || !s->mc_pend.empty())) {
    const int nx = (int)s->n_miss;
    const bool merge = s->mc_hits > 0;
    uint32_t* Hd = P_<uint32_t>(s->d_H);
    uint8_t* hd = P_<uint8_t>(s->d_hinf);
    if (s->msg_dedup) {
      LSG_RC(ensure(s, s->d_Hm, 4 * W_G2A * (size_t)nm));
      LSG_RC(ensure(s, s->d_hinfm, (size_t)nm));
      Hd = P_<uint32_t>(s->d_Hm);
      hd = P_<uint8_t>(s->d_hinfm);
    }
    uint32_t* Hx = Hd;
    uint8_t* hx = hd;
    if (merge) {
      LSG_RC(ensure(s, s->d_Hx, 4 * W_G2A * (size_t)std::max(nx, 1)));
      LSG_RC(ensure(s, s->d_hinfx, (size_t)std::max(nx, 1)));
      Hx = P_<uint32_t>(s->d_Hx);
      hx = P_<uint8_t>(s->d_hinfx);
    }
    if (nx > 0) {
      if (s->msg_objs)
        KL(s, "k_msg_roots", lsgk::msg_roots(S_(s), nx, P_<uint8_t>(s->d_msg), P_<uint32_t>(s->d_msgoff),
                                             P_<uint32_t>(s->d_msglen)));
      KL(s, "k_expand_msg", lsgk::expand_msg(S_(s), nx, P_<uint8_t>(s->d_msg), P_<uint32_t>(s->d_msgoff),
                                             P_<uint32_t>(s->d_msglen), P_<uint8_t>(s->d_dst), DST_POP_LEN,
                                             P_<uint8_t>(s->d_ub)));
      LSG_RC(launch_hash(s, nx, Hx, hx));
// ... 2094 lines not shown
  Dev* d = c->dev[0];
  Slot* s = &d->util;
  timer_reset(s);
  if (n == 0) return LSG_OK;
  LSG_RC(util_stage_keys(s, pks, pk_len, n));
  LSG_RC(ensure(s, s->d_ub, 96 * n));
  KL(s, "k_pk_validate", lsgk::pk_validate(S_(s), (int)n, P_<uint8_t>(s->d_pk), pk_len, P_<uint32_t>(s->d_pkp),
                                           P_<int32_t>(s->d_pkerr)));
  LSG_HIP(s, hipMemcpyAsync(err, s->d_pkerr.p, 4 * n, hipMemcpyDeviceToHost, s->st[0]));
  if (out96) {
    KL(s, "k_g1p_to_bytes", lsgk::g1p_to_bytes(S_(s), (int)n, P_<uint32_t>(s->d_pkp), P_<uint8_t>(s->d_ub)));
    LSG_HIP(s, hipMemcpyAsync(out96, s->d_ub.p, 96 * n, hipMemcpyDeviceToHost, s->st[0]));
  }
  LSG_HIP(s, hipStreamSynchronize(s->st[0]));
  keep_times(s);
  return LSG_OK;
}

int lsg_hash_to_g2(lsg_ctx* c, const uint8_t* msgs, uint32_t msg_len, size_t n, const uint8_t* dst,
                   uint32_t dst_len, uint8_t* out192) {
  if (!c || !out192 || (n && msg_len && !msgs) || dst_len > 255 || (dst_len && !dst) || msg_marked(msg_len))
    return LSG_ERR_INVALID_ARG;
  LSG_ENTER(c);
  Dev* d = c->dev[0];
  Slot* s = &d->util;
  timer_reset(s);
  if (n == 0) return LSG_OK;
  LSG_RC(util_hash(s, msgs, msg_len, n, dst, dst_len));
  LSG_RC(ensure(s, s->d_aux, 192 * n));
  const int nn = (int)n;
  KL(s, "k_g2a_to_bytes",
     lsgk::g2a_to_bytes(S_(s), nn, P_<uint32_t>(s->d_H), P_<uint8_t>(s->d_hinf), P_<uint8_t>(s->d_aux)));
  LSG_HIP(s, hipMemcpyAsync(out192, s->d_aux.p, 192 * n, hipMemcpyDeviceToHost, s->st[0]));
  LSG_HIP(s, hipStreamSynchronize(s->st[0]));
  keep_times(s);
  return LSG_OK;
}

static int sig_decode_impl(lsg_ctx* c, const uint8_t* sigs, uint32_t sig_len, size_t n, bool validate, Slot** out) {
  Dev* d = c->dev[0];
  Slot* s = &d->util;
  *out = s;
  std::vector<lsg_set> sets(n);
  std::vector<const lsg_set*> sp(n);
  for (size_t i = 0; i < n; i++) {
    memset(&sets[i], 0, sizeof(lsg_set));
    sets[i].sig = sigs + (size_t)sig_len * i;
    sets[i].sig_len = sig_len;
    sp[i] = &sets[i];
  }
  LSG_RC(stage_sets(s, sp.data(), n, 0, false));
  LSG_RC(size_state(s, n, 0, 1, 0));
  const int nn = (int)n;
  KL(s, "k_sig_decode", lsgk::sig_decode(S_(s), nn, P_<uint8_t>(s->d_sig), P_<uint32_t>(s->d_siglen),
                                         P_<uint32_t>(s->d_sigaff), P_<uint8_t>(s->d_siginf), P_<int32_t>(s->d_seterr)));
  if (validate) LSG_RC(launch_sig_subgroup(s, nn));
  return LSG_OK;
}

int lsg_sig_decode(lsg_ctx* c, const uint8_t* sigs, uint32_t sig_len, size_t n, uint8_t* out192, int32_t* err) {
  if (!c || !out192 || !err || (n && !sigs)) return LSG_ERR_INVALID_ARG;
  LSG_ENTER(c);
  timer_reset(&c->dev[0]->util);
  if (n == 0) return LSG_OK;
  Slot* s;
  LSG_RC(sig_decode_impl(c, sigs, sig_len, n, true, &s));
  LSG_RC(ensure(s, s->d_aux, 192 * n));
  KL(s, "k_g2a_to_bytes", lsgk::g2a_to_bytes(S_(s), (int)n, P_<uint32_t>(s->d_sigaff), P_<uint8_t>(s->d_siginf),
                                             P_<uint8_t>(s->d_aux)));
  LSG_HIP(s, hipMemcpyAsync(out192, s->d_aux.p, 192 * n, hipMemcpyDeviceToHost, s->st[0]));
  LSG_HIP(s, hipMemcpyAsync(err, s->d_seterr.p, 4 * n, hipMemcpyDeviceToHost, s->st[0]));
  LSG_HIP(s, hipStreamSynchronize(s->st[0]));
  keep_times(s);
  return LSG_OK;
}

int lsg_aggregate_signatures(lsg_ctx* c, const uint8_t* sigs, uint32_t sig_len, const uint32_t* offsets,
                             size_t n_groups, uint8_t* out96, int32_t* err) {
  if (!c || !offsets || (n_groups && (!out96 || !err)) || offsets[0] != 0 || n_groups > 0x7fffffffull)
    return LSG_ERR_INVALID_ARG;
  for (size_t g = 0; g < n_groups; g++)
    if (offsets[g + 1] < offsets[g]) return LSG_ERR_INVALID_ARG;
  const size_t n = offsets[n_groups];
  if (n && !sigs) return LSG_ERR_INVALID_ARG;
  LSG_ENTER(c);
  timer_reset(&c->dev[0]->util);
  for (size_t g = 0; g < n_groups; g++) {
    err[g] = offsets[g + 1] == offsets[g] ? LSG_ERR_EMPTY_AGGREGATE : 0;
    memset(out96 + 96 * g, 0, 96);
  }
  if (n == 0) return LSG_OK;
  Slot* s;
  LSG_RC(sig_decode_impl(c, sigs, sig_len, n, false, &s));
  LSG_RC(size_state(s, n, 0, n_groups, 0));
  s->plan.clear();
  std::vector<int32_t> off(n_groups), len(n_groups);
  for (size_t g = 0; g < n_groups; g++) {
    off[g] = (int32_t)offsets[g];
    len[g] = (int32_t)(offsets[g + 1] - offsets[g]);
  }
  SegPlan P = slot_seg(s, 1, off, len, false, 0, 0);
  LSG_RC(upload_plan(s));
  LSG_RC(ensure(s, s->d_aux, 96 * n_groups));
  const int nn = (int)n;
  KL(s, "k_sig_prep", lsgk::sig_prep(S_(s), nn, P_<uint32_t>(s->d_sigaff), P_<uint8_t>(s->d_siginf),
                                     P_<int32_t>(s->d_seterr), nullptr, nullptr, nullptr, P_<uint32_t>(s->d_rs)));
  LSG_RC(run_seg(s, 1, "g2_aggregate", P, P_<uint32_t>(s->d_rs), P_<uint32_t>(s->d_S)));
  KL(s, "k_g2p_compress",
// ... 222 lines not shown
  if (E == 1)
    KL(s, "k_check_fp_sqr", lsgk::check_fp_sqr(S_(s), (int)n, P_<uint32_t>(s->d_aux), P_<uint32_t>(s->d_Fb)));
  else
    KL(s, "k_check_fp2_sqr", lsgk::check_fp2_sqr(S_(s), (int)n, P_<uint32_t>(s->d_aux), P_<uint32_t>(s->d_Fb)));
  LSG_HIP(s, hipMemcpyAsync(out, s->d_Fb.p, bytes, hipMemcpyDeviceToHost, s->st[0]));
  LSG_HIP(s, hipStreamSynchronize(s->st[0]));
  return LSG_OK;
}
int lsg_check_fp_sqr(lsg_ctx* c, const uint32_t* in, size_t n, uint32_t* out) { return check_sqr(c, in, n, out, 1); }
int lsg_check_fp2_sqr(lsg_ctx* c, const uint32_t* in, size_t n, uint32_t* out) { return check_sqr(c, in, n, out, 2); }

int lsg_check_sums(lsg_ctx* c, const uint32_t* in, size_t n, uint32_t* out) {
  constexpr size_t EIN = 12, EOUT = 42;
  if (!c || (n && (!in || !out)) || n > 0x7fffffffull / (4 * W_FP * EOUT)) return LSG_ERR_INVALID_ARG;
  LSG_ENTER(c);
  if (n == 0) return LSG_OK;
  Slot* s = &c->dev[0]->util;
  timer_reset(s);
  LSG_RC(ensure(s, s->d_aux, 4 * EIN * W_FP * n));
  LSG_RC(ensure(s, s->d_Fb, 4 * EOUT * W_FP * n));
  LSG_HIP(s, hipMemcpyAsync(s->d_aux.p, in, 4 * EIN * W_FP * n, hipMemcpyHostToDevice, s->st[0]));
  KL(s, "k_check_sums", lsgk::check_sums(S_(s), (int)n, P_<uint32_t>(s->d_aux), P_<uint32_t>(s->d_Fb)));
  LSG_HIP(s, hipMemcpyAsync(out, s->d_Fb.p, 4 * EOUT * W_FP * n, hipMemcpyDeviceToHost, s->st[0]));
  LSG_HIP(s, hipStreamSynchronize(s->st[0]));
  return LSG_OK;
}

static int check_lanes(lsg_ctx* c, const uint32_t* in, size_t n, uint32_t* out, bool g2, bool mf = false) {
  const size_t EIN = g2 ? lsgk::CHECK_G2L_IN : lsgk::CHECK_LANES_IN, EOUT = g2 ? lsgk::CHECK_G2L_OUT : lsgk::CHECK_LANES_OUT;
  if (!c || (n && (!in || !out)) || n > 0x7fffffffull / (4 * W_FP * EOUT)) return LSG_ERR_INVALID_ARG;
  LSG_ENTER(c);
  if (n == 0) return LSG_OK;
  Slot* s = &c->dev[0]->util;
  timer_reset(s);
  LSG_RC(ensure(s, s->d_aux, 4 * EIN * W_FP * n));
  LSG_RC(ensure(s, s->d_Fb, 4 * EOUT * W_FP * n));
  LSG_HIP(s, hipMemcpyAsync(s->d_aux.p, in, 4 * EIN * W_FP * n, hipMemcpyHostToDevice, s->st[0]));
  if (g2)
    KL(s, "k_check_g2_lanes", lsgk::check_g2_lanes(S_(s), (int)n, P_<uint32_t>(s->d_aux), P_<uint32_t>(s->d_Fb)));
  else if (mf)
    KL(s, "k_check_mf_lanes", lsgk::check_mf_lanes(S_(s), (int)n, P_<uint32_t>(s->d_aux), P_<uint32_t>(s->d_Fb)));
  else
    KL(s, "k_check_fp2_lanes", lsgk::check_fp2_lanes(S_(s), (int)n, P_<uint32_t>(s->d_aux), P_<uint32_t>(s->d_Fb)));
  LSG_HIP(s, hipMemcpyAsync(out, s->d_Fb.p, 4 * EOUT * W_FP * n, hipMemcpyDeviceToHost, s->st[0]));
  LSG_HIP(s, hipStreamSynchronize(s->st[0]));
  return LSG_OK;
}
int lsg_check_fp2_lanes(lsg_ctx* c, const uint32_t* in, size_t n, uint32_t* out) { return check_lanes(c, in, n, out, false); }
int lsg_check_g2_lanes(lsg_ctx* c, const uint32_t* in, size_t n, uint32_t* out) { return check_lanes(c, in, n, out, true); }
int lsg_check_mf_lanes(lsg_ctx* c, const uint32_t* in, size_t n, uint32_t* out) {
  return check_lanes(c, in, n, out, false, true);
}

int lsg_check_canon(lsg_ctx* c, const uint32_t* in, size_t n, const uint8_t* bytes48, size_t nb, uint32_t* out,
                    uint32_t* out_limbs) {
  constexpr size_t WOUT = lsgk::CHECK_CANON_OUT;
  if (!c || (n && (!in || !out)) || (nb && (!bytes48 || !out_limbs)) || n > 0x7fffffffull / (4 * WOUT) ||
      nb > 0x7fffffffull / (4 * W_FP))
    return LSG_ERR_INVALID_ARG;
  LSG_ENTER(c);
  Slot* s = &c->dev[0]->util;
  timer_reset(s);
  if (n) {
    LSG_RC(ensure(s, s->d_aux, 4 * W_FP * n));
    LSG_RC(ensure(s, s->d_Fb, 4 * WOUT * n));
    LSG_HIP(s, hipMemcpyAsync(s->d_aux.p, in, 4 * W_FP * n, hipMemcpyHostToDevice, s->st[0]));
    KL(s, "k_check_canon", lsgk::check_canon(S_(s), (int)n, P_<uint32_t>(s->d_aux), P_<uint32_t>(s->d_Fb)));
    LSG_HIP(s, hipMemcpyAsync(out, s->d_Fb.p, 4 * WOUT * n, hipMemcpyDeviceToHost, s->st[0]));
    LSG_HIP(s, hipStreamSynchronize(s->st[0]));
  }
  if (nb) {
    LSG_RC(ensure(s, s->d_aux, 48 * nb));
    LSG_RC(ensure(s, s->d_Fb, 4 * W_FP * nb));
    LSG_HIP(s, hipMemcpyAsync(s->d_aux.p, bytes48, 48 * nb, hipMemcpyHostToDevice, s->st[0]));
    KL(s, "k_check_from_bytes", lsgk::check_from_bytes(S_(s), (int)nb, P_<uint8_t>(s->d_aux), P_<uint32_t>(s->d_Fb)));
    LSG_HIP(s, hipMemcpyAsync(out_limbs, s->d_Fb.p, 4 * W_FP * nb, hipMemcpyDeviceToHost, s->st[0]));
    LSG_HIP(s, hipStreamSynchronize(s->st[0]));
  }
  return LSG_OK;
}

int lsg_check_fp2_roots(lsg_ctx* c, const uint32_t* in, size_t n, uint32_t* out) {
  constexpr size_t WOUT = lsgk::CHECK_ROOTS_OUT;
  if (!c || (n && (!in || !out)) || n > 0x7fffffffull / (4 * WOUT)) return LSG_ERR_INVALID_ARG;
  LSG_ENTER(c);
  if (n == 0) return LSG_OK;
  Slot* s = &c->dev[0]->util;
  timer_reset(s);
  LSG_RC(ensure(s, s->d_aux, 4 * 2 * W_FP * n));
  LSG_RC(ensure(s, s->d_Fb, 4 * WOUT * n));
  LSG_HIP(s, hipMemcpyAsync(s->d_aux.p, in, 4 * 2 * W_FP * n, hipMemcpyHostToDevice, s->st[0]));
  KL(s, "k_check_fp2_roots", lsgk::check_fp2_roots(S_(s), (int)n, P_<uint32_t>(s->d_aux), P_<uint32_t>(s->d_Fb)));
  LSG_HIP(s, hipMemcpyAsync(out, s->d_Fb.p, 4 * WOUT * n, hipMemcpyDeviceToHost, s->st[0]));
  LSG_HIP(s, hipStreamSynchronize(s->st[0]));
  return LSG_OK;
}

int lsg_check_batch_inv(lsg_ctx* c, const uint32_t* in, size_t n, uint32_t* out) {
  if (!c || (n && (!in || !out)) || n > 0x7fffffffull / (4 * W_FP)) return LSG_ERR_INVALID_ARG;
  LSG_ENTER(c);
  if (n == 0) return LSG_OK;
  Slot* s = &c->dev[0]->util;
  timer_reset(s);
  LSG_RC(ensure(s, s->d_aux, 4 * W_FP * n));
  LSG_RC(ensure(s, s->d_Fb, 4 * W_FP * n));
  LSG_HIP(s, hipMemcpyAsync(s->d_aux.p, in, 4 * W_FP * n, hipMemcpyHostToDevice, s->st[0]));
// ... 103 lines not shown
```

lodestar_amd/csrc/lsg_k_hash.hip:

```cpp
#include "lsg_kcommon.hpp"

#ifndef LSG_H2C_WAVES
#define LSG_H2C_WAVES 2
#endif

struct ShaLds {
  uint32_t st[8];
  uint32_t n, total;
  uint8_t* blk;
};
LSG_DEVI void shal_init(ShaLds& c) {
  const uint32_t iv[8] = {0x6a09e667u, 0xbb67ae85u, 0x3c6ef372u, 0xa54ff53au,
                          0x510e527fu, 0x9b05688cu, 0x1f83d9abu, 0x5be0cd19u};
#pragma unroll
  for (int i = 0; i < 8; i++) c.st[i] = iv[i];
  c.n = 0;
  c.total = 0;
}
LSG_DEVI void shal_flush(ShaLds& c) {
  uint32_t w[16];
  const uint32_t* wl = (const uint32_t*)c.blk;
#pragma unroll
  for (int k = 0; k < 16; k++) w[k] = __builtin_bswap32(wl[k * 64]);
  sha256_compress(c.st, w);
// ... 68 lines not shown
  shal_final(c, b0);
  uint32_t* o = (uint32_t*)(ub + 256 * i);
  for (int r = 1; r <= 8; r++) {
    shal_init(c);
#pragma unroll
    for (int k = 0; k < 8; k++) shal_word(c, r == 1 ? b0[k] : (b0[k] ^ bi[k]));
    shal_byte(c, (uint8_t)r);
    shal_bytes(c, s_dst, dst_len);
    shal_byte(c, (uint8_t)dst_len);
    shal_final(c, bi);
#pragma unroll
    for (int k = 0; k < 8; k++) o[8 * (r - 1) + k] = __builtin_bswap32(bi[k]);
  }
}

struct h2c_u_t {
  fp2_t u0, u1;
};
static_assert(lane_words<h2c_u_t>() == lsgl::W_H2CU, "layout: hash_to_field");

__global__ void LSG_KERNEL_ATTR k_h2c_prep(int n, const uint8_t* __restrict__ ub, uint32_t* __restrict__ U,
                                           uint32_t* __restrict__ norms) {
  LANE_ITEM(n);
  (void)lead;
  const uint8_t* b = ub + 256 * item;
  h2c_u_t u;
  u.u0 = fp2_make(fp_from_be64_mod(b), fp_from_be64_mod(b + 64));
  u.u1 = fp2_make(fp_from_be64_mod(b + 128), fp_from_be64_mod(b + 192));
  lane_store(U, item, u);
  lane_store(norms, 2 * item, fp2_norm(sswu_tv1(u.u0)));
  lane_store(norms, 2 * item + 1, fp2_norm(sswu_tv1(u.u1)));
}

template <class T>
LSG_DEVI T quad_swap_pairs(const T& v) {
  constexpr int W = sizeof(T) / 4;
  uint32_t w[W];
  __builtin_memcpy(w, &v, sizeof(T));
#pragma unroll
  for (int k = 0; k < W; k++) w[k] = pdpp<0x4E>(w[k]);
  T r;
  __builtin_memcpy(&r, w, sizeof(T));
  return r;
}
__global__ void LSG_KERNEL_ATTR_W(LSG_H2C_WAVES) k_h2c_map(int n2, const uint32_t* __restrict__ U, const uint32_t* __restrict__ ninv,
                                          uint32_t* __restrict__ Hp) {
  LANE_ITEM(n2);
  (void)lead;
  const g2p_t q = iso_map3(map_to_curve_sswu_ni(lane_load<fp2_t>(U, item), lane_load<fp_t>(ninv, item)));
  const g2p_t o = quad_swap_pairs(q);
  if ((item & 1) == 0) lane_store(Hp, item >> 1, g2_add(q, o));
}

template <bool LANES>
LSG_DEVI void h2c_clear_item(uint32_t* park, int n, uint32_t* __restrict__ Hp, uint32_t* __restrict__ zN,
                             uint8_t* __restrict__ hinf) {
  LANE_ITEM(n);
  lds_park(park, lane_load<g2p_t>(Hp, item));
  g2p_t q = clear_cofactor_g2_parked<LANES>([&]() { return lds_unpark<g2p_t>(park); },
                                            [&](const g2p_t& v) { lds_park(park, v); },
                                            [&](const g2p_t& v) { lane_store(Hp, item, v); },
                                            [&]() { return lane_load<g2p_t>(Hp, item); });
  bool is_inf = proj_is_inf(q);
  lane_store(Hp, item, q);
  lane_store(zN, item, is_inf ? fp_zero() : fp2_norm(q.Z));
  if (lead) hinf[item] = is_inf ? 1 : 0;
}
__global__ void LSG_KERNEL_ATTR_W(LSG_H2C_WAVES) k_h2c_clear(int n, uint32_t* __restrict__ Hp, uint32_t* __restrict__ zN,
                                            uint8_t* __restrict__ hinf) {
  __shared__ uint32_t park[sizeof(g2p_t) / 4 * LSG_TPB];
  h2c_clear_item<true>(park, n, Hp, zN, hinf);
}
#ifdef LSG_FP2_LANES
__global__ void LSG_KERNEL_ATTR_W(LSG_H2C_WAVES) k_h2c_clear_pair(int n, uint32_t* __restrict__ Hp,
                                                                  uint32_t* __restrict__ zN, uint8_t* __restrict__ hinf) {
  __shared__ uint32_t park[sizeof(g2p_t) / 4 * LSG_TPB];
  h2c_clear_item<false>(park, n, Hp, zN, hinf);
}
#endif

__global__ void LSG_KERNEL_ATTR k_h2c_gather(int n, const uint32_t* __restrict__ mid, const uint32_t* __restrict__ Hm,
                                             const uint8_t* __restrict__ hinfm, uint32_t* __restrict__ H,
                                             uint8_t* __restrict__ hinf) {
  LANE_ITEM(n);
  const uint32_t m = mid[item];
  lane_store(H, item, lane_load<g2a_t>(Hm, m));
  if (lead) hinf[item] = hinfm[m];
}

__global__ void LSG_KERNEL_ATTR k_h2c_cache_merge(int nm, const uint32_t* __restrict__ src, uint32_t n_rows,
                                                  const uint32_t* __restrict__ rows, const uint8_t* __restrict__ rinf,
                                                  uint32_t n_miss, const uint32_t* __restrict__ Hx,
                                                  const uint8_t* __restrict__ hinfx, uint32_t* __restrict__ Hm,
                                                  uint8_t* __restrict__ hinfm) {
  LANE_ITEM(nm);
  const uint32_t w = src[item], k = w & ~LSG_MC_ROW;
  const bool hit = (w & LSG_MC_ROW) != 0;
  if (k >= (hit ? n_rows : n_miss)) return;
  lane_store(Hm, item, lane_load<g2a_t>(hit ? rows : Hx, k));
  if (lead) hinfm[item] = hit ? rinf[k] : hinfx[k];
}

__global__ void LSG_KERNEL_ATTR k_h2c_cache_store(int n, const uint32_t* __restrict__ list, uint32_t n_miss,
                                                  const uint32_t* __restrict__ Hx, const uint8_t* __restrict__ hinfx,
                                                  uint32_t n_rows, uint32_t* __restrict__ rows,
                                                  uint8_t* __restrict__ rinf) {
// ... 44 lines not shown
  if (i >= (size_t)n) return;
  ssz_signing_root_deposit(data + (size_t)stride * i, domains + dstride * i, out32 + 32 * i);
}

__global__ void __launch_bounds__(64) k_object_signing_root(int n, const uint8_t* __restrict__ objs, uint32_t obj_len,
                                                            const uint8_t* __restrict__ domains, uint32_t dstride,
                                                            uint8_t* __restrict__ out32) {
  size_t i = gtid();
  if (i >= (size_t)n) return;
  ssz_object_signing_root(obj_len, objs + (size_t)obj_len * i, domains + dstride * i, out32 + 32 * i);
}

__global__ void __launch_bounds__(64) k_msg_roots(int n, uint8_t* msg, const uint32_t* __restrict__ msg_off,
                                                  uint32_t* __restrict__ msg_len) {
  size_t i = gtid();
  if (i >= (size_t)n) return;
  const uint32_t l = msg_len[i];
  if (!(l & LSG_MSG_OBJECT)) return;
  const uint32_t obj_len = (l & ~LSG_MSG_OBJECT) - 32u;
  uint8_t* p = msg + msg_off[i];
  msg_len[i] = ssz_object_signing_root(obj_len, p, p + obj_len, p) ? 32u : 0u;
}

namespace lsgk {
hipError_t deposit_signing_root(hipStream_t st, int n, const uint8_t* data, uint32_t stride, const uint8_t* domains,
                                uint32_t dstride, uint8_t* out32) {
  if (n <= 0) return hipSuccess;
  hipLaunchKernelGGL(k_deposit_signing_root, dim3((n + 63) / 64), dim3(64), 0, st, n, data, stride, domains, dstride,
                     out32);
  return hipGetLastError();
}
hipError_t object_signing_root(hipStream_t st, int n, const uint8_t* objs, uint32_t obj_len, const uint8_t* domains,
                               uint32_t dstride, uint8_t* out32) {
  if (n <= 0) return hipSuccess;
  hipLaunchKernelGGL(k_object_signing_root, dim3((n + 63) / 64), dim3(64), 0, st, n, objs, obj_len, domains, dstride,
                     out32);
  return hipGetLastError();
}
hipError_t msg_roots(hipStream_t st, int n, uint8_t* msg, const uint32_t* off, uint32_t* len) {
  if (n <= 0) return hipSuccess;
  hipLaunchKernelGGL(k_msg_roots, dim3((n + 63) / 64), dim3(64), 0, st, n, msg, off, len);
  return hipGetLastError();
}
hipError_t expand_msg(hipStream_t st, int n, const uint8_t* msg, const uint32_t* off, const uint32_t* len,
                      const uint8_t* dst, uint32_t dst_len, uint8_t* ub) {
  if (n <= 0) return hipSuccess;
  if (dst_len > 255) return hipErrorInvalidValue;
  hipLaunchKernelGGL(k_expand_msg, dim3((n + 63) / 64), dim3(64), 0, st, n, msg, off, len, dst, dst_len, ub);
  return hipGetLastError();
}
hipError_t h2c_prep(hipStream_t st, int n, const uint8_t* ub, uint32_t* U, uint32_t* norms) {
  LSG_LAUNCH_ITEMS(k_h2c_prep, n, st, n, ub, U, norms);
}
hipError_t h2c_map(hipStream_t st, int n, const uint32_t* U, const uint32_t* ninv, uint32_t* Hp) {
  LSG_LAUNCH_ITEMS(k_h2c_map, 2 * n, st, 2 * n, U, ninv, Hp);
}
hipError_t h2c_clear(hipStream_t st, int n, uint32_t* Hp, uint32_t* zN, uint8_t* hinf, bool pair_form) {
#ifdef LSG_FP2_LANES
  if (pair_form) LSG_LAUNCH_ITEMS(k_h2c_clear_pair, n, st, n, Hp, zN, hinf);
#endif
  (void)pair_form;
  LSG_LAUNCH_ITEMS(k_h2c_clear, n, st, n, Hp, zN, hinf);
}
hipError_t h2c_gather(hipStream_t st, int n, const uint32_t* mid, const uint32_t* Hm, const uint8_t* hinfm, uint32_t* H,
                      uint8_t* hinf) {
  LSG_LAUNCH_ITEMS(k_h2c_gather, n, st, n, mid, Hm, hinfm, H, hinf);
}
hipError_t h2c_cache_merge(hipStream_t st, int nm, const uint32_t* src, uint32_t n_rows, const uint32_t* rows,
                           const uint8_t* rinf, uint32_t n_miss, const uint32_t* Hx, const uint8_t* hinfx, uint32_t* Hm,
                           uint8_t* hinfm) {
  LSG_LAUNCH_ITEMS(k_h2c_cache_merge, nm, st, nm, src, n_rows, rows, rinf, n_miss, Hx, hinfx, Hm, hinfm);
}
hipError_t h2c_cache_store(hipStream_t st, int n, const uint32_t* list, uint32_t n_miss, const uint32_t* Hx,
                           const uint8_t* hinfx, uint32_t n_rows, uint32_t* rows, uint8_t* rinf) {
  LSG_LAUNCH_ITEMS(k_h2c_cache_store, n, st, n, list, n_miss, Hx, hinfx, n_rows, rows, rinf);
}
hipError_t h2c_affine(hipStream_t st, int n, const uint32_t* Hp, const uint32_t* ninv, const uint8_t* hinf,
                      uint32_t* H) {
  LSG_LAUNCH_ITEMS(k_h2c_affine, n, st, n, Hp, ninv, hinf, H);
}
hipError_t signing_root(hipStream_t st, int n, const uint8_t* roots, const uint8_t* domains, uint32_t dstride,
                        uint8_t* out32) {
  if (n <= 0) return hipSuccess;
  hipLaunchKernelGGL(k_signing_root, dim3((n + 63) / 64), dim3(64), 0, st, n, roots, domains, dstride, out32);
  return hipGetLastError();
}
hipError_t attestation_signing_root(hipStream_t st, int n, const uint8_t* data, const uint8_t* domains,
                                    uint32_t dstride, uint8_t* out32) {
  if (n <= 0) return hipSuccess;
  hipLaunchKernelGGL(k_attestation_signing_root, dim3((n + 63) / 64), dim3(64), 0, st, n, data, domains, dstride,
                     out32);
  return hipGetLastError();
}
}
```

lodestar_amd/csrc/lsg_k_reduce.hip:

```cpp
#include "lsg_kcommon.hpp"
namespace {
#include "lsg_inv.hpp"
}

template <int OP>
struct seg_op;
template <>
struct seg_op<0> {
  typedef g1p_t T;
  static LSG_DEVI T ident() { return proj_inf<fp_t>(); }
  static LSG_DEVI T op(const T& a, const T& b) { return g1_add(a, b); }
};
template <>
struct seg_op<1> {
  typedef g2p_t T;
  static LSG_DEVI T ident() { return proj_inf<fp2_t>(); }
  static LSG_DEVI T op(const T& a, const T& b) { return g2_add(a, b); }
};
template <>
struct seg_op<2> {
  typedef fp12_t T;
  static LSG_DEVI T ident() { return fp12_one(); }
  static LSG_DEVI T op(const T& a, const T& b) { return fp12_mul(a, b); }
};
// ... 316 lines not shown
  const fp2v_t A = fp2v_from_pair(Ap), B = fp2v_from_pair(Bp), C = fp2v_from_pair(Cp);
  const fpv_t k = fpv_from_pair(Bp.c0);
  put(fmul_fp(A, k));
  put2(fp2_mul_fp(Ap, Bp.c0));
  put(fmul_xi(A));
  put2(fp2_mul_xi(Ap));
  put((fsum(A) + fsum_mul_xi(fsum(B) - C)).carry());
  put2((fp2s(Ap) + fp2s_mul_xi(fp2s(Bp) - Cp)).carry());
  const fp6v_t v = fp6_mul_v(fp6_make(A, B, C));
  put(v.c0);
  put(v.c1);
  put(v.c2);
  put(fone<fp2v_t>());
  put(fzero<fp2v_t>());
  lane_store(out + (size_t)lsgk::CHECK_LANES_OUT * lsgl::W_FP * item + (size_t)o * lsgl::W_FP, 0, k);
}
#endif

constexpr int LSG_CHECK_CANON_OUT = lsgk::CHECK_CANON_OUT;
__global__ void LSG_KERNEL_ATTR k_check_canon(int n, const uint32_t* __restrict__ in, uint32_t* __restrict__ out) {
  LANE_ITEM(n);
  const fp_t a = lane_load<fp_t>(in, item);
  uint32_t* o = out + (size_t)LSG_CHECK_CANON_OUT * item;
  const fp_t c = fp_canonical(a);
  lane_store(o, 0, pair_canon(a));
  lane_store(o + 14, 0, c);
  fp_to_be48((uint8_t*)(o + 28), c);
  fp_to_be48((uint8_t*)(o + 42), a);
  const uint32_t f = (fp_is_zero(a) ? 1u : 0u) | (fp_canon_lt_p(a) ? 2u : 0u) | (fp_canon_gt_half(a) ? 4u : 0u) |
                     (fp_canon_parity(a) ? 8u : 0u);
  o[40 + (lead ? 0 : 1)] = lead ? f : 0u;
}
__global__ void LSG_KERNEL_ATTR k_check_from_bytes(int n, const uint8_t* __restrict__ in, uint32_t* __restrict__ out) {
  LANE_ITEM(n);
  (void)lead;
  lane_store(out, item, fp_from_be_bytes(in + 48 * item, 12));
}
constexpr int LSG_CHECK_ROOTS_OUT = lsgk::CHECK_ROOTS_OUT;
__global__ void LSG_KERNEL_ATTR k_check_fp2_roots(int n, const uint32_t* __restrict__ in, uint32_t* __restrict__ out) {
  LANE_ITEM(n);
  const fp2_t a(lane_load<fp_t>(in, 2 * item), lane_load<fp_t>(in, 2 * item + 1));
  uint32_t* o = out + (size_t)LSG_CHECK_ROOTS_OUT * item;
  fp2_t r;
  const bool ok = fp2_sqrt(r, a);
  lane_store(o, 0, r.c0);
  lane_store(o + 14, 0, r.c1);
  lane_store(o + 28, 0, fp_inv(a.c0));
  lane_store(o + 42, 0, pair_mont_mul(pair_inv_gcd(pair_canon(a.c0)), fp_t(FP_RCUBE)));
  const uint32_t f = (ok ? 1u : 0u) | (fp2_sgn0(a) ? 2u : 0u) | (fp2_lexi_largest(a) ? 4u : 0u) |
                     (fp2_is_zero(a) ? 8u : 0u);
  o[56 + (lead ? 0 : 1)] = lead ? f : 0u;
}

__global__ void LSG_KERNEL_ATTR k_probe_fp_mul(int n, int iters, uint32_t* __restrict__ io) {
  LANE_ITEM(n);
  (void)lead;
  fp_t a = lane_load<fp_t>(io, item), b = fp_t(FP_R2), c = fp_t(FP_R3), d = fp_t(FP_HALF);
  for (int k = 0; k < iters; k++) {
    a = fp_mul(a, b);
    b = fp_mul(b, c);
    c = fp_mul(c, d);
    d = fp_mul(d, a);
  }
  lane_store(io, item, fp_add(fp_add(a, b), fp_add(c, d)));
}

__global__ void __launch_bounds__(256) k_probe_mad(int iters, uint32_t seed, uint64_t* __restrict__ io) {
  const uint32_t t = blockIdx.x * blockDim.x + threadIdx.x;
  uint64_t acc[16];
  uint32_t x[16];
#pragma unroll
  for (int k = 0; k < 16; k++) {
    acc[k] = t + k;
    x[k] = (t * 2654435761u) ^ (seed + 977u * k);
  }
  const uint32_t y = seed | 1u;
  for (int i = 0; i < iters; i++) {
#pragma unroll
    for (int k = 0; k < 16; k++) acc[k] = (uint64_t)x[k] * y + acc[k];
  }
  uint64_t r = 0;
#pragma unroll
  for (int k = 0; k < 16; k++) r ^= acc[k];
  io[t] = r;
}

namespace lsgk {
hipError_t seg_reduce(hipStream_t st, int op, int n_chunks, int ips_log2, const int32_t* chunks, const int32_t* idx,
                      const uint32_t* src, uint32_t* dst, uint32_t* tmp) {
  const size_t items = (size_t)n_chunks << ips_log2;
  if (op == 0) LSG_LAUNCH_ITEMS(k_seg_reduce<0>, items, st, n_chunks, ips_log2, chunks, idx, src, dst, tmp);
  if (op == 1) LSG_LAUNCH_ITEMS(k_seg_reduce<1>, items, st, n_chunks, ips_log2, chunks, idx, src, dst, tmp);
  LSG_LAUNCH_ITEMS(k_seg_reduce<2>, items, st, n_chunks, ips_log2, chunks, idx, src, dst, tmp);
}
hipError_t binv_fold(hipStream_t st, int n, int zero_to_one, const uint32_t* in, uint32_t* pre, uint32_t* tot) {
  LSG_LAUNCH_ITEMS(k_binv_fold, (n + LSG_BINV_T - 1) / LSG_BINV_T, st, n, zero_to_one, in, pre, tot);
}
hipError_t binv_block(hipStream_t st, int n, int T, int zero_to_one, const uint32_t* in, uint32_t* pre, uint32_t* out) {
  if (n <= 0) return hipSuccess;
  const size_t chunks = ((size_t)n + T - 1) / T;
  hipLaunchKernelGGL(k_binv_block, dim3(lane_blocks(chunks)), dim3(LSG_TPB), 0, st, n, T, zero_to_one, in, pre, out);
  return hipGetLastError();
}
hipError_t binv_root(hipStream_t st, const uint32_t* top, uint32_t* inv) {
  LSG_LAUNCH_ITEMS(k_binv_root, 1, st, top, inv);
}
hipError_t binv_unfold(hipStream_t st, int n, int zero_to_one, const uint32_t* in, const uint32_t* pre,
                       const uint32_t* tinv, uint32_t* out) {
  LSG_LAUNCH_ITEMS(k_binv_unfold, (n + LSG_BINV_T - 1) / LSG_BINV_T, st, n, zero_to_one, in, pre, tinv, out);
}
hipError_t blobs_to_fp12(hipStream_t st, int n, const uint8_t* blobs, uint32_t* out) {
  LSG_LAUNCH_ITEMS(k_blobs_to_fp12, n, st, n, blobs, out);
}
hipError_t fp12_to_canon(hipStream_t st, int n, const uint32_t* in, uint8_t* out576) {
  LSG_LAUNCH_ITEMS(k_fp12_to_canon, n, st, n, in, out576);
}
hipError_t fp12_pow_u64(hipStream_t st, const uint8_t* in576, uint64_t r, uint8_t* out576) {
  LSG_LAUNCH_ITEMS(k_fp12_pow_u64, 1, st, in576, r, out576);
}
hipError_t check_fp2_mul(hipStream_t st, int n, const uint32_t* in, uint32_t* out) {
  LSG_LAUNCH_ITEMS(k_check_fp2_mul, n, st, n, in, out);
}
hipError_t check_fp_sqr(hipStream_t st, int n, const uint32_t* in, uint32_t* out) {
  LSG_LAUNCH_ITEMS(k_check_fp_sqr, n, st, n, in, out);
}
hipError_t check_fp2_sqr(hipStream_t st, int n, const uint32_t* in, uint32_t* out) {
  LSG_LAUNCH_ITEMS(k_check_fp2_sqr, n, st, n, in, out);
}
hipError_t check_sums(hipStream_t st, int n, const uint32_t* in, uint32_t* out) {
  LSG_LAUNCH_ITEMS(k_check_sums, n, st, n, in, out);
}
#ifdef LSG_FP2_LANES
hipError_t check_fp2_lanes(hipStream_t st, int n, const uint32_t* in, uint32_t* out) {
  LSG_LAUNCH_ITEMS(k_check_fp2_lanes, n, st, n, in, out);
}
hipError_t check_g2_lanes(hipStream_t st, int n, const uint32_t* in, uint32_t* out) {
  LSG_LAUNCH_ITEMS(k_check_g2_lanes, n, st, n, in, out);
}
hipError_t check_mf_lanes(hipStream_t st, int n, const uint32_t* in, uint32_t* out) {
  LSG_LAUNCH_ITEMS(k_check_mf_lanes, n, st, n, in, out);
}
#else
hipError_t check_mf_lanes(hipStream_t, int, const uint32_t*, uint32_t*) { return hipErrorNotSupported; }
hipError_t check_fp2_lanes(hipStream_t, int, const uint32_t*, uint32_t*) { return hipErrorNotSupported; }
hipError_t check_g2_lanes(hipStream_t, int, const uint32_t*, uint32_t*) { return hipErrorNotSupported; }
#endif
hipError_t check_canon(hipStream_t st, int n, const uint32_t* in, uint32_t* out) {
  LSG_LAUNCH_ITEMS(k_check_canon, n, st, n, in, out);
}
hipError_t check_from_bytes(hipStream_t st, int n, const uint8_t* in, uint32_t* out) {
  LSG_LAUNCH_ITEMS(k_check_from_bytes, n, st, n, in, out);
}
hipError_t check_fp2_roots(hipStream_t st, int n, const uint32_t* in, uint32_t* out) {
  LSG_LAUNCH_ITEMS(k_check_fp2_roots, n, st, n, in, out);
}
hipError_t probe_fp_mul(hipStream_t st, int items, int iters, uint32_t* io) {
  LSG_LAUNCH_ITEMS(k_probe_fp_mul, items, st, items, iters, io);
}
hipError_t probe_mad(hipStream_t st, int blocks, int iters, uint32_t seed, uint64_t* io) {
  if (blocks <= 0) return hipSuccess;
  hipLaunchKernelGGL(k_probe_mad, dim3(blocks), dim3(256), 0, st, iters, seed, io);
  return hipGetLastError();
}
}
```

lodestar_amd/csrc/lsg_k_sig.hip:

```cpp
#include "lsg_kcommon.hpp"

__global__ void LSG_KERNEL_ATTR k_sig_decode(int n, const uint8_t* __restrict__ sig, const uint32_t* __restrict__ sig_len,
                                             uint32_t* __restrict__ sig_aff, uint8_t* __restrict__ inf,
                                             int32_t* __restrict__ err) {
  LANE_ITEM(n);
  uint32_t len = sig_len[item];
  g2a_t p;
  p.x = fp2_zero();
  p.y = fp2_zero();
  bool is_inf = false;
  int e;
  if (len == 96)
    e = g2_uncompress(p, is_inf, sig + 192 * item);
  else if (len == 192)
    e = g2_deserialize_uncompressed(p, is_inf, sig + 192 * item);
  else
    e = LSG_BLST_INVALID_SIZE;
  lane_store(sig_aff, item, p);
  if (lead) {
    inf[item] = is_inf ? 1 : 0;
    err[item] = e;
  }
}

template <class F>
LSG_DEVI void sig_subgroup_item(uint32_t* park, int n, const uint32_t* __restrict__ sig_aff,
                                const uint8_t* __restrict__ inf, int32_t* __restrict__ err) {
  LANE_ITEM(n);
  if (err[item] != 0 || inf[item]) return;
  lds_park(park, g2_layout<F>::in(lane_load<g2a_t>(sig_aff, item)));
  bool ok = g2_in_group_get<F>([&]() { return proj_from_aff(lds_unpark<aff_t<F>>(park)); });
  if (lead && !ok) err[item] = LSG_BLST_POINT_NOT_IN_GROUP;
}
__global__ void LSG_KERNEL_ATTR k_sig_subgroup(int n, const uint32_t* __restrict__ sig_aff,
                                               const uint8_t* __restrict__ inf, int32_t* __restrict__ err) {
  __shared__ uint32_t park[sizeof(g2a_t) / 4 * LSG_TPB];
  sig_subgroup_item<chain_fp2_t>(park, n, sig_aff, inf, err);
}
#ifdef LSG_FP2_LANES
__global__ void LSG_KERNEL_ATTR k_sig_subgroup_pair(int n, const uint32_t* __restrict__ sig_aff,
                                                    const uint8_t* __restrict__ inf, int32_t* __restrict__ err) {
  __shared__ uint32_t park[sizeof(g2a_t) / 4 * LSG_TPB];
  sig_subgroup_item<fp2_t>(park, n, sig_aff, inf, err);
}
#endif

LSG_DEVI bool sig_usable(size_t i, const uint8_t* inf, const int32_t* err, const uint8_t* pinf) {
  return err[i] == 0 && !inf[i] && !(pinf && pinf[i]);
}
__global__ void LSG_KERNEL_ATTR k_sig_proj(int n, const uint32_t* __restrict__ sig_aff, const uint8_t* __restrict__ inf,
                                           const int32_t* __restrict__ err, const uint8_t* __restrict__ pinf,
                                           uint32_t* __restrict__ out) {
  LANE_ITEM(n);
  (void)lead;
  g2p_t r = proj_inf<fp2_t>();
  if (sig_usable(item, inf, err, pinf)) r = proj_from_aff(lane_load<g2a_t>(sig_aff, item));
  lane_store(out, item, r);
}
__global__ void LSG_KERNEL_ATTR_W(1) k_sig_scale3(int n, const uint32_t* __restrict__ sig_aff, const uint8_t* __restrict__ inf,
                                                  const int32_t* __restrict__ err, const uint8_t* __restrict__ pinf,
                                                  const uint64_t* __restrict__ rnd, const uint8_t* __restrict__ mode,
                                                  uint32_t* __restrict__ out) {
  LANE_ITEM(n);
  (void)lead;
  if (mode && !mode[item]) return;
  g2p_t r = proj_inf<fp2_t>();
  if (sig_usable(item, inf, err, pinf)) {
    r = proj_from_aff(lane_load<g2a_t>(sig_aff, item));
    if (rnd[item] != 0) r = proj_mul_u64_s3(r, rnd[item]);
  }
  lane_store(out, item, r);
}

// ... 50 lines not shown
  g2p_t p = lane_load<g2p_t>(pts, item);
  bool is_inf = proj_is_inf(p);
  g2a_t a;
  if (is_inf) {
    a.x = fp2_zero();
    a.y = fp2_zero();
  } else {
    a = proj_to_aff(p);
  }
  g2_compress(out96 + 96 * item, a, is_inf);
}

__global__ void LSG_KERNEL_ATTR k_g2p_to_canon(int n, const uint32_t* __restrict__ in, uint8_t* __restrict__ out) {
  LANE_ITEM(n);
  (void)lead;
  g2p_to_canon_bytes(out + 288 * item, lane_load<g2p_t>(in, item));
}

template <class F>
__device__ proj_t<F> proj_mul_be256(const proj_t<F>& p, const uint8_t* k) {
  proj_t<F> acc = proj_inf<F>();
  for (int byte = 0; byte < 32; byte++) {
    uint32_t v = k[byte];
    for (int b = 7; b >= 0; b--) {
      acc = gdbl(acc);
      proj_t<F> s = gadd(acc, p);
      bool bit = (v >> b) & 1u;
      acc.X = fselect(bit, s.X, acc.X);
      acc.Y = fselect(bit, s.Y, acc.Y);
      acc.Z = fselect(bit, s.Z, acc.Z);
    }
  }
  return acc;
}

__global__ void LSG_KERNEL_ATTR k_sign(int n, const uint8_t* __restrict__ sks, const uint32_t* __restrict__ H,
                                       uint8_t* __restrict__ out96) {
  LANE_ITEM(n);
  (void)lead;
  g2p_t s = proj_mul_be256(proj_from_aff(lane_load<g2a_t>(H, item)), sks + 32 * item);
  bool is_inf = proj_is_inf(s);
  g2a_t a;
  if (is_inf) {
    a.x = fp2_zero();
    a.y = fp2_zero();
  } else {
    a = proj_to_aff(s);
  }
  g2_compress(out96 + 96 * item, a, is_inf);
}

namespace lsgk {
hipError_t sig_decode(hipStream_t st, int n, const uint8_t* sig, const uint32_t* sig_len, uint32_t* sig_aff,
                      uint8_t* inf, int32_t* err) {
  LSG_LAUNCH_ITEMS(k_sig_decode, n, st, n, sig, sig_len, sig_aff, inf, err);
}
hipError_t sig_subgroup(hipStream_t st, int n, const uint32_t* sig_aff, const uint8_t* inf, int32_t* err, bool pair_form) {
#ifdef LSG_FP2_LANES
  if (pair_form) LSG_LAUNCH_ITEMS(k_sig_subgroup_pair, n, st, n, sig_aff, inf, err);
#endif
  (void)pair_form;
  LSG_LAUNCH_ITEMS(k_sig_subgroup, n, st, n, sig_aff, inf, err);
}
hipError_t sig_prep(hipStream_t st, int n, const uint32_t* sig_aff, const uint8_t* inf, const int32_t* err,
                    const uint8_t* pinf, const uint64_t* rnd, const uint8_t* mode, uint32_t* out) {
  if (n <= 0) return hipSuccess;
  if (!rnd || mode) {
    hipLaunchKernelGGL(k_sig_proj, dim3(lane_blocks((size_t)n)), dim3(LSG_TPB), 0, st, n, sig_aff, inf, err, pinf, out);
    hipError_t e = hipGetLastError();
    if (e != hipSuccess || !rnd) return e;
  }
  return sig_scale_only(st, n, sig_aff, inf, err, pinf, rnd, mode, out);
}
hipError_t sig_scale_only(hipStream_t st, int n, const uint32_t* sig_aff, const uint8_t* inf, const int32_t* err,
                          const uint8_t* pinf, const uint64_t* rnd, const uint8_t* mode, uint32_t* out) {
  LSG_LAUNCH_ITEMS(k_sig_scale3, n, st, n, sig_aff, inf, err, pinf, rnd, mode, out);
}
hipError_t sig_agg_seg(hipStream_t st, int n_chunks, int ips_log2, const int32_t* chunks, const int32_t* gather,
                       const uint32_t* sig_aff, const uint8_t* inf, const int32_t* err, uint32_t* dst, uint32_t* tmp) {
  LSG_LAUNCH_ITEMS(k_sig_agg_seg, (size_t)n_chunks << ips_log2, st, n_chunks, ips_log2, chunks, gather, sig_aff, inf, err,
                   dst, tmp);
}
hipError_t g2a_to_bytes(hipStream_t st, int n, const uint32_t* pts, const uint8_t* inf, uint8_t* out192) {
  LSG_LAUNCH_ITEMS(k_g2a_to_bytes, n, st, n, pts, inf, out192);
}
hipError_t g2p_compress(hipStream_t st, int n, const uint32_t* pts, uint8_t* out96) {
  LSG_LAUNCH_ITEMS(k_g2p_compress, n, st, n, pts, out96);
}
hipError_t g2p_to_canon(hipStream_t st, int n, const uint32_t* pts, uint8_t* out288) {
  LSG_LAUNCH_ITEMS(k_g2p_to_canon, n, st, n, pts, out288);
}
hipError_t sign(hipStream_t st, int n, const uint8_t* sks, const uint32_t* H, uint8_t* out96) {
  LSG_LAUNCH_ITEMS(k_sign, n, st, n, sks, H, out96);
}
}
```

lodestar_amd/csrc/lsg_launch.h:

```cpp
#pragma once
#include <hip/hip_runtime.h>
#include <stddef.h>
#include <stdint.h>

constexpr uint32_t LSG_MC_ROW = 0x80000000u;

namespace lsgk {
hipError_t expand_msg(hipStream_t st, int n, const uint8_t* msg, const uint32_t* off, const uint32_t* len,
                      const uint8_t* dst, uint32_t dst_len, uint8_t* ub);
hipError_t h2c_prep(hipStream_t st, int n, const uint8_t* ub, uint32_t* U, uint32_t* norms);
hipError_t h2c_map(hipStream_t st, int n, const uint32_t* U, const uint32_t* ninv, uint32_t* Hp);
hipError_t h2c_clear(hipStream_t st, int n, uint32_t* Hp, uint32_t* zN, uint8_t* hinf, bool pair_form = false);
hipError_t h2c_gather(hipStream_t st, int n, const uint32_t* mid, const uint32_t* Hm, const uint8_t* hinfm, uint32_t* H,
                      uint8_t* hinf);
hipError_t h2c_affine(hipStream_t st, int n, const uint32_t* Hp, const uint32_t* ninv, const uint8_t* hinf,
                      uint32_t* H);
hipError_t h2c_cache_merge(hipStream_t st, int nm, const uint32_t* src, uint32_t n_rows, const uint32_t* rows,
                           const uint8_t* rinf, uint32_t n_miss, const uint32_t* Hx, const uint8_t* hinfx, uint32_t* Hm,
                           uint8_t* hinfm);
hipError_t h2c_cache_store(hipStream_t st, int n, const uint32_t* list, uint32_t n_miss, const uint32_t* Hx,
                           const uint8_t* hinfx, uint32_t n_rows, uint32_t* rows, uint8_t* rinf);
hipError_t signing_root(hipStream_t st, int n, const uint8_t* roots, const uint8_t* domains, uint32_t dstride,
                        uint8_t* out32);
hipError_t attestation_signing_root(hipStream_t st, int n, const uint8_t* data, const uint8_t* domains,
                                    uint32_t dstride, uint8_t* out32);
hipError_t deposit_signing_root(hipStream_t st, int n, const uint8_t* data, uint32_t stride, const uint8_t* domains,
                                uint32_t dstride, uint8_t* out32);
hipError_t object_signing_root(hipStream_t st, int n, const uint8_t* objs, uint32_t obj_len, const uint8_t* domains,
                               uint32_t dstride, uint8_t* out32);
hipError_t msg_roots(hipStream_t st, int n, uint8_t* msg, const uint32_t* off, uint32_t* len);

hipError_t sig_decode(hipStream_t st, int n, const uint8_t* sig, const uint32_t* sig_len, uint32_t* sig_aff,
                      uint8_t* inf, int32_t* err);
hipError_t sig_subgroup(hipStream_t st, int n, const uint32_t* sig_aff, const uint8_t* inf, int32_t* err,
                        bool pair_form = false);
hipError_t sig_prep(hipStream_t st, int n, const uint32_t* sig_aff, const uint8_t* inf, const int32_t* err,
                    const uint8_t* pinf, const uint64_t* rnd, const uint8_t* mode, uint32_t* out);
hipError_t sig_scale_only(hipStream_t st, int n, const uint32_t* sig_aff, const uint8_t* inf, const int32_t* err,
                          const uint8_t* pinf, const uint64_t* rnd, const uint8_t* mode, uint32_t* out);
hipError_t sig_agg_seg(hipStream_t st, int n_chunks, int ips_log2, const int32_t* chunks, const int32_t* gather,
                       const uint32_t* sig_aff, const uint8_t* inf, const int32_t* err, uint32_t* dst, uint32_t* tmp);
hipError_t g2a_to_bytes(hipStream_t st, int n, const uint32_t* pts, const uint8_t* inf, uint8_t* out192);
hipError_t g2p_compress(hipStream_t st, int n, const uint32_t* pts, uint8_t* out96);
hipError_t g2p_to_canon(hipStream_t st, int n, const uint32_t* pts, uint8_t* out288);
hipError_t sign(hipStream_t st, int n, const uint8_t* sks, const uint32_t* H, uint8_t* out96);

hipError_t pk_decode(hipStream_t st, int n, const uint8_t* pk, uint32_t stride, const uint32_t* pk_len, uint32_t* pts,
                     int32_t* err, const uint32_t* tab, const uint8_t* tab_ok, uint32_t tab_n);
hipError_t pk_validate(hipStream_t st, int n, const uint8_t* pk, uint32_t len, uint32_t* pts, int32_t* err);
hipError_t pk_keyvalidate(hipStream_t st, int n, const int32_t* keys, const uint8_t* pk, const uint32_t* pk_len,
                          int32_t* code);
hipError_t pk_keyvalidate_apply(hipStream_t st, int n, const int32_t* sets, const int32_t* code, int32_t* set_err);
hipError_t pk_gather_aff(hipStream_t st, int n, const uint8_t* pk, uint32_t stride, const uint32_t* pk_len, uint32_t* pts,
                         uint8_t* inf, int32_t* err, const uint32_t* tab, const uint8_t* tab_ok, uint32_t tab_n);
hipError_t pk_agg_seg(hipStream_t st, int n_chunks, int ips_log2, const int32_t* chunks, const uint8_t* pk, uint32_t stride,
                      const uint32_t* pk_len, int32_t* err, const uint32_t* tab, const uint8_t* tab_ok, uint32_t tab_n,
                      uint32_t* dst, uint32_t* tmp);
hipError_t pk_agg_bits(hipStream_t st, int n_pairs, const int32_t* pair_set, const int32_t* plan, const uint32_t* bits,
                       const uint32_t* cm_idx, const uint32_t* cm_off, const uint32_t* cm_sum, const uint32_t* tab,
                       const uint8_t* tab_ok, uint32_t tab_n, uint32_t* dst);
hipError_t pk_agg_bits_multi(hipStream_t st, int n_pairs, const int32_t* pair_set, const int32_t* set_plan,
                             const int32_t* part_plan, const uint32_t* bits, const uint32_t* cm_idx, const uint32_t* cm_off,
                             const uint32_t* cm_sum, const uint32_t* tab, const uint8_t* tab_ok, uint32_t tab_n,
                             uint32_t* dst);
struct AggTreeArgs {
  int L = 0, T = 1;
  int64_t n_c0 = 0, N0 = 0;
  const int32_t* blk_set = nullptr;
  const int32_t* set_o0 = nullptr;
  const int32_t* set_len = nullptr;
  const int32_t* set_pk0 = nullptr;
  const uint8_t* pk = nullptr;
  uint32_t stride = 0;
  const uint32_t* pk_len = nullptr;
  int32_t* pk_err = nullptr;
  const uint32_t* tab = nullptr;
  const uint8_t* tab_ok = nullptr;
  uint32_t tab_n = 0;
  uint32_t* pts = nullptr;
  uint8_t* inf = nullptr;
  uint32_t* pre[2] = {nullptr, nullptr};
  uint32_t* cinv[2] = {nullptr, nullptr};
  uint8_t* flag[2] = {nullptr, nullptr};
};
hipError_t agg_leaf(hipStream_t st, const AggTreeArgs& a);
hipError_t agg_step(hipStream_t st, const AggTreeArgs& a, int t);
hipError_t agg_final(hipStream_t st, const AggTreeArgs& a, int n_sets, const int32_t* src, uint32_t* agg);
hipError_t pk_scale(hipStream_t st, int n, const uint32_t* agg, const uint64_t* rnd, uint32_t* Pp, uint32_t* zP,
                    uint8_t* pinf);
hipError_t pk_affine(hipStream_t st, int n, const uint32_t* Pp, const uint32_t* zinv, uint32_t* P);
hipError_t pk_mask(hipStream_t st, int n, const uint32_t* Pp, const int32_t* err, const uint8_t* pinf, uint32_t* out);
hipError_t g1p_affine_inv(hipStream_t st, int n, const uint32_t* Pp, uint32_t* P, uint8_t* pinf);
hipError_t g1p_to_bytes(hipStream_t st, int n, const uint32_t* pts, uint8_t* out96);
hipError_t sk_to_pk(hipStream_t st, int n, const uint8_t* sks, uint8_t* out96);

hipError_t miller_fused(hipStream_t st, int n_items, const int32_t* item_first, const int32_t* item_cnt,
                        const uint32_t* P, const uint8_t* pinf, const uint8_t* hinf, const int32_t* err,
                        const uint32_t* H, uint32_t* f, bool pair_form = false);
hipError_t miller_lines(hipStream_t st, int n, const uint32_t* H, uint32_t* lines);
hipError_t miller_lines_list(hipStream_t st, int n, const int32_t* list, const uint32_t* H, uint32_t* lines);
hipError_t miller_accum_list(hipStream_t st, int n, const int32_t* list, const uint32_t* P, const uint8_t* pinf,
                             const uint8_t* hinf, const int32_t* err, const uint32_t* lines, uint32_t* f);
hipError_t miller_accum(hipStream_t st, int K, int n_items, const int32_t* item_first, const int32_t* item_cnt,
                        const uint32_t* P, const uint8_t* pinf, const uint8_t* hinf, const int32_t* err, int n_sets,
                        const uint32_t* lines, uint32_t* f);

hipError_t seg_reduce(hipStream_t st, int op, int n_chunks, int ips_log2, const int32_t* chunks, const int32_t* idx,
                      const uint32_t* src, uint32_t* dst, uint32_t* tmp);
hipError_t binv_fold(hipStream_t st, int n, int zero_to_one, const uint32_t* in, uint32_t* pre, uint32_t* tot);
hipError_t binv_root(hipStream_t st, const uint32_t* top, uint32_t* inv);
hipError_t binv_block(hipStream_t st, int n, int T, int zero_to_one, const uint32_t* in, uint32_t* pre, uint32_t* out);
hipError_t binv_unfold(hipStream_t st, int n, int zero_to_one, const uint32_t* in, const uint32_t* pre,
                       const uint32_t* tinv, uint32_t* out);
hipError_t blobs_to_fp12(hipStream_t st, int n, const uint8_t* blobs, uint32_t* out);
hipError_t fp12_to_canon(hipStream_t st, int n, const uint32_t* in, uint8_t* out576);
hipError_t fp12_pow_u64(hipStream_t st, const uint8_t* in576, uint64_t r, uint8_t* out576);
hipError_t probe_fp_mul(hipStream_t st, int items, int iters, uint32_t* io);
hipError_t check_fp2_mul(hipStream_t st, int n, const uint32_t* in, uint32_t* out);
hipError_t check_fp_sqr(hipStream_t st, int n, const uint32_t* in, uint32_t* out);
hipError_t check_fp2_sqr(hipStream_t st, int n, const uint32_t* in, uint32_t* out);
hipError_t check_sums(hipStream_t st, int n, const uint32_t* in, uint32_t* out);
constexpr int CHECK_LANES_IN = 12, CHECK_LANES_OUT = 24, CHECK_G2L_IN = 12, CHECK_G2L_OUT = 24;
hipError_t check_fp2_lanes(hipStream_t st, int n, const uint32_t* in, uint32_t* out);
hipError_t check_g2_lanes(hipStream_t st, int n, const uint32_t* in, uint32_t* out);
hipError_t check_mf_lanes(hipStream_t st, int n, const uint32_t* in, uint32_t* out);
constexpr int CHECK_CANON_OUT = 54, CHECK_ROOTS_OUT = 58;
hipError_t check_canon(hipStream_t st, int n, const uint32_t* in, uint32_t* out);
hipError_t check_from_bytes(hipStream_t st, int n, const uint8_t* in48, uint32_t* out);
hipError_t check_fp2_roots(hipStream_t st, int n, const uint32_t* in, uint32_t* out);
hipError_t probe_mad(hipStream_t st, int blocks, int iters, uint32_t seed, uint64_t* io);
}
```

lodestar_amd/csrc/lsg_tower.hpp:

```cpp
#pragma once

#ifndef LSG_BIGFN
#define LSG_BIGFN LSG_NOINL
#endif

LSG_INL fp_t fp_one() { return fp_t(FP_ONE); }
LSG_INL fp_t fp_dbl(const fp_t& a) { return fp_add(a, a); }
#ifdef LSG_SQR_LEAF
LSG_INL fp_t fp_sqr(const fp_t& a) { return pair_mont_sqr(a); }
#else
LSG_INL fp_t fp_sqr(const fp_t& a) { return fp_mul(a, a); }
#endif
LSG_INL fp_t fp_to_mont(const fp_t& a) { return fp_mul(a, fp_t(FP_R2)); }
LSG_INL fp_t fp_from_mont(const fp_t& a) { return fp_canonical(fp_mul(a, fp_t(FP_ONE_CANON))); }
LSG_INL fp_t fp_from_be48(const uint8_t* b) { return fp_from_be_bytes(b, 12); }

LSG_BIGFN fp_t fp_pow_fixed(fp_t a, const uint32_t* e) {
#ifdef LSG_POW_LEAF
  return pair_pow_fixed(a, e);
#else
  fp_t T[8];
  T[0] = a;
  const fp_t a2 = fp_sqr(a);
#pragma unroll
// ... 236 lines not shown
  fp_mul_list<3 * K>(z, x, y);
#pragma unroll
  for (int k = 0; k < K; k++)
    r[k] = fp2_t(fp_sub(z[3 * k], z[3 * k + 1]), fp_sub(fp_sub(z[3 * k + 2], z[3 * k]), z[3 * k + 1]));
}

template <int K>
LSG_INL void fp2_sqr_n(fp2_t* r, const fp2_t* a) {
  fp_t x[2 * K], y[2 * K], z[2 * K];
#pragma unroll
  for (int k = 0; k < K; k++) {
    x[2 * k] = fp_add(a[k].c0, a[k].c1);
    y[2 * k] = fp_sub(a[k].c0, a[k].c1);
    x[2 * k + 1] = a[k].c0;
    y[2 * k + 1] = a[k].c1;
  }
  fp_mul_list<2 * K>(z, x, y);
#pragma unroll
  for (int k = 0; k < K; k++) r[k] = fp2_t(z[2 * k], fp_dbl(z[2 * k + 1]));
}

LSG_INL fp2_t fp2_mul_xi(const fp2_t& a) { return fp2s_mul_xi(a).carry(); }

LSG_INL fp_t fp2_norm(const fp2_t& a) {
#ifdef LSG_SQR_LEAF
  const fp_t s0 = fp_sqr(a.c0), s1 = fp_sqr(a.c1);
#else
  fp_t s0, s1;
  fp_mul2(s0, s1, a.c0, a.c0, a.c1, a.c1);
#endif
  return fp_add(s0, s1);
}

LSG_INL fp2_t fp2_inv(const fp2_t& a) {
  fp_t ni = fp_inv(fp2_norm(a));
  return fp2_t(fp_mul(a.c0, ni), fp_neg(fp_mul(a.c1, ni)));
}

LSG_INL fp2_t fp2_mul_b3(const fp2_t& a) { return fp2_mulk<12>(fp2_mul_xi(a)); }

LSG_INL uint32_t fp2_sgn0(const fp2_t& a) {
  fp_t c0 = fp_from_mont(a.c0), c1 = fp_from_mont(a.c1);
  uint32_t sign0 = fp_canon_parity(c0);
  uint32_t zero0 = fp_is_zero(c0) ? 1u : 0u;
  uint32_t sign1 = fp_canon_parity(c1);
  return sign0 | (zero0 & sign1);
}

LSG_INL bool fp2_lexi_largest(const fp2_t& y) {
  fp_t c0 = fp_from_mont(y.c0), c1 = fp_from_mont(y.c1);
  return fp_is_zero(c1) ? fp_canon_gt_half(c0) : fp_canon_gt_half(c1);
}

LSG_INL fp_t fp2_norm_sqrt_candidate(const fp2_t& a, bool* is_sq) {
  fp_t n = fp2_norm(a);
  fp_t s = fp_pow_id(n, LSG_POW_SQRT);
  *is_sq = fp_eq(fp_sqr(s), n);
  return s;
}
LSG_BIGFN bool fp2_sqrt_with_norm_root(fp2_t& out, fp2_t a, fp_t s) {
  fp_t c = fp_mul(fp_add(a.c0, s), fp_t(FP_HALF));
  c = fp_select(fp_is_zero(c), a.c0, c);
  fp_t t = fp_pow_id(c, LSG_POW_SQRT34);
  fp_t ct = fp_mul(c, t);
  bool c_sq = fp_eq(fp_mul(ct, t), fp_one()) || fp_is_zero(c);
  fp_t h = fp_mul(fp_mul(a.c1, t), fp_t(FP_HALF));
  fp2_t r = c_sq ? fp2_t(ct, h) : fp2_t(h, fp_neg(ct));
  out = r;
  return fp2_eq(fp2_sqr(r), a);
}
LSG_BIGFN bool fp2_sqrt(fp2_t& out, fp2_t a) {
  bool ok;
  fp_t s = fp2_norm_sqrt_candidate(a, &ok);
  bool r = fp2_sqrt_with_norm_root(out, a, s);
  return ok && r;
}

LSG_INL fp6_t fp6_make(const fp2_t& a, const fp2_t& b, const fp2_t& c) {
  fp6_t r;
  r.c0 = a;
  r.c1 = b;
  r.c2 = c;
  return r;
}
LSG_INL fp6_t fp6_zero() { return fp6_make(fp2_zero(), fp2_zero(), fp2_zero()); }
LSG_INL fp6_t fp6_one() { return fp6_make(fp2_one(), fp2_zero(), fp2_zero()); }
LSG_INL fp6_t fp6_add(const fp6_t& a, const fp6_t& b) {
  return fp6_make(fp2_add(a.c0, b.c0), fp2_add(a.c1, b.c1), fp2_add(a.c2, b.c2));
}
LSG_INL fp6_t fp6_sub(const fp6_t& a, const fp6_t& b) {
  return fp6_make(fp2_sub(a.c0, b.c0), fp2_sub(a.c1, b.c1), fp2_sub(a.c2, b.c2));
}
LSG_INL fp6_t fp6_neg(const fp6_t& a) { return fp6_make(fp2_neg(a.c0), fp2_neg(a.c1), fp2_neg(a.c2)); }

LSG_INL void fp6_mul_prep(fp2_t* A, fp2_t* B, const fp6_t& a, const fp6_t& b) {
  A[0] = a.c0;
  B[0] = b.c0;
  A[1] = a.c1;
  B[1] = b.c1;
  A[2] = a.c2;
  B[2] = b.c2;
  A[3] = fp2_add(a.c1, a.c2);
  B[3] = fp2_add(b.c1, b.c2);
  A[4] = fp2_add(a.c0, a.c1);
  B[4] = fp2_add(b.c0, b.c1);
  A[5] = fp2_add(a.c0, a.c2);
  B[5] = fp2_add(b.c0, b.c2);
}
LSG_INL fp2s_t<2, 1, 3, 0> fp6_kar_s0(const fp2_t& v0, const fp2_t& v1, const fp2_t& v2, const fp2_t& m0) {
  return fp2s(v0) + fp2s_mul_xi(fp2_sub2(m0, v1, v2));
}
LSG_INL fp2s_t<2, 3, 3, 2> fp6_kar_s1(const fp2_t& v0, const fp2_t& v1, const fp2_t& v2, const fp2_t& m1) {
  return (fp2s(m1) - v0 - v1) + fp2s_mul_xi(v2);
}
LSG_INL fp2s_t<2, 2> fp6_kar_s2(const fp2_t& v0, const fp2_t& v1, const fp2_t& v2, const fp2_t& m2) {
  return (fp2s(m2) - v0 - v2) + v1;
}
LSG_INL fp6_t fp6_mul_fin(const fp2_t* V) {
  fp6_t r;
  r.c0 = fp6_kar_s0(V[0], V[1], V[2], V[3]).carry();
  r.c1 = fp6_kar_s1(V[0], V[1], V[2], V[4]).carry();
  r.c2 = fp6_kar_s2(V[0], V[1], V[2], V[5]).carry();
// ... 240 lines not shown
```

Measured before the change: 3.857 million.

## Split sqrt exponentiations in sig decode and SSWU map into lane-parallel pow kernels

```diff
diff --git a/include/lodestar_bls.h b/include/lodestar_bls.h
--- a/include/lodestar_bls.h
+++ b/include/lodestar_bls.h
@@ -174,6 +174,8 @@
 int lsg_check_fp2_lanes(lsg_ctx* ctx, const uint32_t* in, size_t n, uint32_t* out);
 int lsg_check_g2_lanes(lsg_ctx* ctx, const uint32_t* in, size_t n, uint32_t* out);
 int lsg_check_mf_lanes(lsg_ctx* ctx, const uint32_t* in, size_t n, uint32_t* out);
+int lsg_check_pow_lanes(lsg_ctx* ctx, int32_t id, const uint32_t* in, size_t n, uint32_t* out);
+int lsg_check_pow_pair(lsg_ctx* ctx, int32_t id, const uint32_t* in, size_t n, uint32_t* out);
 int lsg_check_canon(lsg_ctx* ctx, const uint32_t* in, size_t n, const uint8_t* bytes48, size_t nb, uint32_t* out,
                     uint32_t* out_limbs);
 int lsg_check_fp2_roots(lsg_ctx* ctx, const uint32_t* in, size_t n, uint32_t* out);
diff --git a/lodestar_amd/_native.py b/lodestar_amd/_native.py
--- a/lodestar_amd/_native.py
+++ b/lodestar_amd/_native.py
@@ -174,7 +174,7 @@
     "lsg_set_coalesce", "lsg_aggregate_pubkeys_multi", "lsg_check_fp2_mul",
     "lsg_check_fp_sqr", "lsg_check_fp2_sqr", "lsg_check_sums", "lsg_check_fp2_lanes", "lsg_check_g2_lanes", "lsg_check_mf_lanes",
     "lsg_check_canon", "lsg_check_fp2_roots", "lsg_check_batch_inv", "lsg_check_map_uniform",
-    "lsg_check_batch_partial_rnd",
+    "lsg_check_batch_partial_rnd", "lsg_check_pow_lanes", "lsg_check_pow_pair",
     "lsg_deposit_signing_roots", "lsg_verify_deposits",
     "lsg_committees_set", "lsg_committees_clear", "lsg_committee_count",
     "lsg_object_signing_roots",
@@ -257,6 +257,8 @@
         lib.lsg_check_fp2_lanes.argtypes = [vp, ctypes.c_char_p, sz, ctypes.c_char_p]
         lib.lsg_check_g2_lanes.argtypes = [vp, ctypes.c_char_p, sz, ctypes.c_char_p]
         lib.lsg_check_mf_lanes.argtypes = [vp, ctypes.c_char_p, sz, ctypes.c_char_p]
+        lib.lsg_check_pow_lanes.argtypes = [vp, i32, ctypes.c_char_p, sz, ctypes.c_char_p]
+        lib.lsg_check_pow_pair.argtypes = [vp, i32, ctypes.c_char_p, sz, ctypes.c_char_p]
         lib.lsg_check_canon.argtypes = [vp, ctypes.c_char_p, sz, ctypes.c_char_p, sz, ctypes.c_char_p, ctypes.c_char_p]
         lib.lsg_check_fp2_roots.argtypes = [vp, ctypes.c_char_p, sz, ctypes.c_char_p]
         lib.lsg_check_batch_inv.argtypes = [vp, ctypes.c_char_p, sz, ctypes.c_char_p]
@@ -810,6 +812,15 @@
     def check_mf_lanes(self, words):
         return self._check_lanes("lsg_check_mf_lanes", words)
 
+    def check_pow(self, pow_id, words, lanes=True):
+        n = len(words) // 14
+        assert len(words) == 14 * n
+        fn = "lsg_check_pow_lanes" if lanes else "lsg_check_pow_pair"
+        out = ctypes.create_string_buffer(4 * 14 * max(n, 1))
+        src = struct.pack(f"<{len(words)}I", *words)
+        self._check(getattr(self.lib, fn)(self.h, pow_id, src, n, out), fn)
+        return list(struct.unpack(f"<{14 * n}I", out.raw[:4 * 14 * n]))
+
     def check_canon(self, words, strings=()):
         n, nb = len(words) // 14, len(strings)
         assert len(words) == 14 * n and all(len(b) == 48 for b in strings)
diff --git a/lodestar_amd/csrc/lsg_ab.h b/lodestar_amd/csrc/lsg_ab.h
--- a/lodestar_amd/csrc/lsg_ab.h
+++ b/lodestar_amd/csrc/lsg_ab.h
@@ -1,6 +1,9 @@
 #pragma once
 #include <stdlib.h>
 #include <string.h>
+
+#define LSG_POW_LANES_DEFAULT 1
+#define LSG_POW_LANES_MIN_DEFAULT 65536
 
 #ifdef LSG_AB
 static inline long lsg_ab_long(const char* name, long dflt) {
diff --git a/lodestar_amd/csrc/lsg_curve.hpp b/lodestar_amd/csrc/lsg_curve.hpp
--- a/lodestar_amd/csrc/lsg_curve.hpp
+++ b/lodestar_amd/csrc/lsg_curve.hpp
@@ -514,7 +514,8 @@
 #define LSG_BLST_INVALID_SIZE 10
 #endif
 
-LSG_INL int g2_uncompress(g2a_t& out, bool& inf, const uint8_t* in) {
+#define LSG_UNCOMPRESS_PENDING (-1)
+LSG_INL int g2_uncompress_parse(g2a_t& out, bool& inf, fp2_t& x, fp2_t& rhs, bool& want, const uint8_t* in) {
   uint8_t in0 = in[0];
   inf = false;
   if (!(in0 & 0x80)) return LSG_BLST_BAD_ENCODING;
@@ -533,16 +534,26 @@
   x1 = fp_mask_flags(x1);
   fp_t x0 = fp_from_be48(in + 48);
   if (!fp_canon_lt_p(x1) || !fp_canon_lt_p(x0)) return LSG_BLST_BAD_ENCODING;
-  fp2_t x = fp2_make(fp_to_mont(x0), fp_to_mont(x1));
-  fp2_t rhs = fp2_add(fp2_mul(fp2_sqr(x), x), FP2_B_G2);
-  fp2_t y;
-  if (!fp2_sqrt(y, rhs)) return LSG_BLST_POINT_NOT_ON_CURVE;
-  bool want = (in0 & 0x20) != 0;
+  x = fp2_make(fp_to_mont(x0), fp_to_mont(x1));
+  rhs = fp2_add(fp2_mul(fp2_sqr(x), x), FP2_B_G2);
+  want = (in0 & 0x20) != 0;
+  return LSG_UNCOMPRESS_PENDING;
+}
+LSG_INL int g2_uncompress_finish(g2a_t& out, const fp2_t& x, fp2_t y, bool ok, bool want) {
+  if (!ok) return LSG_BLST_POINT_NOT_ON_CURVE;
   if (fp2_lexi_largest(y) != want) y = fp2_neg(y);
   out.x = x;
   out.y = y;
   if (fp2_is_zero(x)) return LSG_BLST_POINT_NOT_IN_GROUP;
   return LSG_BLST_SUCCESS;
+}
+LSG_INL int g2_uncompress(g2a_t& out, bool& inf, const uint8_t* in) {
+  fp2_t x, rhs, y;
+  bool want;
+  int e = g2_uncompress_parse(out, inf, x, rhs, want, in);
+  if (e != LSG_UNCOMPRESS_PENDING) return e;
+  bool ok = fp2_sqrt(y, rhs);
+  return g2_uncompress_finish(out, x, y, ok, want);
 }
 
 LSG_INL int g2_deserialize_uncompressed(g2a_t& out, bool& inf, const uint8_t* in) {
diff --git a/lodestar_amd/csrc/lsg_fp2_lanes.hpp b/lodestar_amd/csrc/lsg_fp2_lanes.hpp
--- a/lodestar_amd/csrc/lsg_fp2_lanes.hpp
+++ b/lodestar_amd/csrc/lsg_fp2_lanes.hpp
@@ -70,6 +70,108 @@
   }
   lanes_tail(t, r);
 }
+LSG_PFN void lanes_sqr_pass(uint32_t* r, const uint32_t* a) {
+  uint32_t p[LSG_VL];
+#pragma unroll
+  for (int j = 0; j < LSG_VL; j++) p[j] = LSG_P[j];
+  int64_t t[LSG_VL];
+#pragma unroll
+  for (int j = 0; j < LSG_VL; j++) t[j] = 0;
+#pragma unroll
+  for (int i = 0; i < LSG_VL; i++) {
+    uint32_t ai = a[i], di = a[i] + a[i];
+    LSG_LANES_HIDE(ai);
+    LSG_LANES_HIDE(di);
+    t[i] += (int64_t)(int32_t)a[i] * (int32_t)ai;
+#pragma unroll
+    for (int w = i + 1; w < LSG_VL; w++) t[w] += (int64_t)(int32_t)a[w] * (int32_t)di;
+    lanes_reduce_step(t, p, i);
+  }
+  lanes_tail(t, r);
+}
+
+struct fpl_t {
+  uint32_t l[LSG_VL];
+};
+LSG_PFN fpl_t lanes_fp_hide(fpl_t a) {
+#pragma unroll
+  for (int k = 0; k < LSG_VL; k++) LSG_LANES_HIDE(a.l[k]);
+  return a;
+}
+LSG_PFN fpl_t lanes_fp_mul(const fpl_t& a, const fpl_t& b) {
+  const fpl_t x = lanes_fp_hide(a), y = lanes_fp_hide(b);
+  fpl_t r;
+  lanes_mul_pass(r.l, x.l, y.l);
+  return r;
+}
+LSG_PFN fpl_t lanes_fp_sqr(const fpl_t& a) {
+  const fpl_t x = lanes_fp_hide(a);
+  fpl_t r;
+  lanes_sqr_pass(r.l, x.l);
+  return r;
+}
+LSG_PFN fpl_t lanes_fp_select(bool c, const fpl_t& a, const fpl_t& b) {
+  fpl_t r;
+#pragma unroll
+  for (int k = 0; k < LSG_VL; k++) r.l[k] = c ? a.l[k] : b.l[k];
+  return r;
+}
+#ifdef LSG_POW_IDS
+LSG_PFN fpl_t lanes_pow_plan(const fpl_t& a, int id) {
+  const pow_plan_t& P = LSG_POW_PLANS[id];
+  const fpl_t a2 = lanes_fp_sqr(a);
+  const fpl_t T0 = a;
+  const fpl_t T1 = lanes_fp_mul(T0, a2);
+  const fpl_t T2 = lanes_fp_mul(T1, a2);
+  const fpl_t T3 = lanes_fp_mul(T2, a2);
+  const fpl_t T4 = lanes_fp_mul(T3, a2);
+  const fpl_t T5 = lanes_fp_mul(T4, a2);
+  const fpl_t T6 = lanes_fp_mul(T5, a2);
+  const fpl_t T7 = lanes_fp_mul(T6, a2);
+  auto pick = [&](uint32_t k) {
+    fpl_t tv = T0;
+    tv = lanes_fp_select(k == 1u, T1, tv);
+    tv = lanes_fp_select(k == 2u, T2, tv);
+    tv = lanes_fp_select(k == 3u, T3, tv);
+    tv = lanes_fp_select(k == 4u, T4, tv);
+    tv = lanes_fp_select(k == 5u, T5, tv);
+    tv = lanes_fp_select(k == 6u, T6, tv);
+    tv = lanes_fp_select(k == 7u, T7, tv);
+    return tv;
+  };
+  fpl_t r = pick(P.step[0] & 0xffu);
+  const int n = P.n;
+#pragma unroll 1
+  for (int w = 1; w < n; w++) {
+    const uint32_t s = P.step[w];
+#pragma unroll 1
+    for (uint32_t b = s >> 8; b; b--) r = lanes_fp_sqr(r);
+    r = lanes_fp_mul(r, pick(s & 0xffu));
+  }
+#pragma unroll 1
+  for (int b = P.tail; b; b--) r = lanes_fp_sqr(r);
+  return r;
+}
+#endif
+LSG_PFN fpl_t lanes_fp_load(const uint32_t* mem, size_t i) {
+  const uint32_t* w = mem + i * LSG_VL;
+  fpl_t r;
+#pragma unroll
+  for (int k = 0; k < LSG_VL / 2; k++) {
+    r.l[k] = w[2 * k];
+    r.l[LSG_VL / 2 + k] = w[2 * k + 1];
+  }
+  return r;
+}
+LSG_PFN void lanes_fp_store(uint32_t* mem, size_t i, const fpl_t& a) {
+  uint32_t* w = mem + i * LSG_VL;
+#pragma unroll
+  for (int k = 0; k < LSG_VL / 2; k++) {
+    w[2 * k] = a.l[k];
+    w[2 * k + 1] = a.l[LSG_VL / 2 + k];
+  }
+}
+
 LSG_PFN void lanes_mul_operand(uint32_t& P, uint32_t& Q, uint32_t own, uint32_t partner, bool odd) {
   P = odd ? partner : own;
   Q = odd ? own : 0u - partner;
diff --git a/lodestar_amd/csrc/lsg_h2c.hpp b/lodestar_amd/csrc/lsg_h2c.hpp
--- a/lodestar_amd/csrc/lsg_h2c.hpp
+++ b/lodestar_amd/csrc/lsg_h2c.hpp
@@ -94,26 +94,46 @@
 LSG_INL fp2_t fp2_inv_with_norm_inv(const fp2_t& a, const fp_t& ni) {
   return fp2_t(fp_mul(a.c0, ni), fp_neg(fp_mul(a.c1, ni)));
 }
-LSG_BIGFN g2a_t map_to_curve_sswu_ni(fp2_t u, fp_t ni) {
+struct sswu_mid_t {
+  fp2_t zu2, x1, x2, gx1, gx2;
+};
+LSG_BIGFN sswu_mid_t sswu_stage_a(fp2_t u, fp_t ni) {
+  sswu_mid_t m;
   fp2_t u2 = fp2_sqr(u);
-  fp2_t zu2 = fp2_mul(SSWU_Z, u2);
-  fp2_t tv1 = fp2_add(fp2_sqr(zu2), zu2);
+  m.zu2 = fp2_mul(SSWU_Z, u2);
+  fp2_t tv1 = fp2_add(fp2_sqr(m.zu2), m.zu2);
   bool exc = fp2_is_zero(tv1);
   fp2_t x1 = fp2_mul(SSWU_MINUS_B_OVER_A, fp2_add(fp2_one(), fp2_inv_with_norm_inv(tv1, ni)));
-  x1 = fp2_select(exc, SSWU_B_OVER_ZA, x1);
-  fp2_t gx1 = fp2_add(fp2_mul(fp2_add(fp2_sqr(x1), SSWU_A), x1), SSWU_B);
-  fp2_t x2 = fp2_mul(zu2, x1);
-  fp2_t gx2 = fp2_add(fp2_mul(fp2_add(fp2_sqr(x2), SSWU_A), x2), SSWU_B);
-  bool sq1;
-  fp_t s1 = fp2_norm_sqrt_candidate(gx1, &sq1);
-  fp_t s2 = fp_mul(fp_mul(fp2_norm(zu2), fp2_norm(u)), fp_mul(s1, fp_t(SSWU_NZ_POW_P1D4)));
+  m.x1 = fp2_select(exc, SSWU_B_OVER_ZA, x1);
+  m.gx1 = fp2_add(fp2_mul(fp2_add(fp2_sqr(m.x1), SSWU_A), m.x1), SSWU_B);
+  m.x2 = fp2_mul(m.zu2, m.x1);
+  m.gx2 = fp2_add(fp2_mul(fp2_add(fp2_sqr(m.x2), SSWU_A), m.x2), SSWU_B);
+  return m;
+}
+LSG_BIGFN fp_t sswu_stage_b(fp2_t& x, fp2_t& gx, const sswu_mid_t& m, const fp2_t& u, const fp_t& n, const fp_t& s1) {
+  bool sq1 = fp_is_root_of(s1, n);
+  fp_t s2 = fp_mul(fp_mul(fp2_norm(m.zu2), fp2_norm(u)), fp_mul(s1, fp_t(SSWU_NZ_POW_P1D4)));
+  x = fp2_select(sq1, m.x1, m.x2);
+  gx = fp2_select(sq1, m.gx1, m.gx2);
+  return fp2_sqrt_root_c(gx, fp_select(sq1, s1, s2));
+}
+LSG_BIGFN g2a_t sswu_stage_c(const fp2_t& u, const fp2_t& x, const fp2_t& gx, const fp_t& c, const fp_t& t) {
   g2a_t r;
-  r.x = fp2_select(sq1, x1, x2);
+  r.x = x;
   fp2_t y;
-  (void)fp2_sqrt_with_norm_root(y, fp2_select(sq1, gx1, gx2), fp_select(sq1, s1, s2));
+  (void)fp2_sqrt_root_finish(y, gx, c, t);
   if (fp2_sgn0(u) != fp2_sgn0(y)) y = fp2_neg(y);
   r.y = y;
   return r;
+}
+LSG_BIGFN g2a_t map_to_curve_sswu_ni(fp2_t u, fp_t ni) {
+  const sswu_mid_t m = sswu_stage_a(u, ni);
+  fp_t n = fp2_norm(m.gx1);
+  fp_t s1 = fp_pow_id(n, LSG_POW_SQRT);
+  fp2_t x, gx;
+  fp_t c = sswu_stage_b(x, gx, m, u, n, s1);
+  fp_t t = fp_pow_id(c, LSG_POW_SQRT34);
+  return sswu_stage_c(u, x, gx, c, t);
 }
 LSG_BIGFN g2a_t map_to_curve_sswu(fp2_t u) { return map_to_curve_sswu_ni(u, fp_inv(fp2_norm(sswu_tv1(u)))); }
 
diff --git a/lodestar_amd/csrc/lsg_host.hip b/lodestar_amd/csrc/lsg_host.hip
--- a/lodestar_amd/csrc/lsg_host.hip
+++ b/lodestar_amd/csrc/lsg_host.hip
@@ -156,6 +156,7 @@
   DevBuf d_ub, d_sigaff, d_siginf, d_seterr, d_pkp, d_pkerr, d_agg, d_P, d_pinf, d_H, d_hinf, d_rs, d_rs2, d_fall,
       d_fall2;
   DevBuf d_Pp, d_zP, d_zPi, d_U, d_nrm, d_nrmi, d_Hp, d_zN, d_zNi, d_mid, d_Hm, d_hinfm;
+  DevBuf d_pwsig, d_pwmap;
   DevBuf binv_lv[2], binv_iv[2];
   DevBuf d_lines;
   bool rs2_ready = false;
@@ -436,7 +437,8 @@
                     &s->d_nodeF, &s->d_nodeV, &s->d_plan, &s->d_mid, &s->d_Hm, &s->d_hinfm,
                     &s->d_mmask, &s->d_PmP, &s->d_Pm, &s->d_pinfm, &s->d_errm, &s->d_xport,
                     &s->d_agga, &s->d_aggi, &s->d_aggpre, &s->d_aggtot, &s->d_aggflag, &s->d_cbits,
-                    &s->d_gplan, &s->d_gsum, &s->d_gagg, &s->d_gtmp[0], &s->d_gtmp[1], &s->d_Hx, &s->d_hinfx};
+                    &s->d_gplan, &s->d_gsum, &s->d_gagg, &s->d_gtmp[0], &s->d_gtmp[1], &s->d_Hx, &s->d_hinfx,
+                    &s->d_pwsig, &s->d_pwmap};
   for (DevBuf* b : bufs) free_dev(*b);
   for (auto& u : s->seg_tmp)
     for (DevBuf& b : u) free_dev(b);
@@ -572,6 +574,8 @@
              {&s->d_Hp, 4 * W_G2P * nn},
              {&s->d_zN, 4 * W_FP * nn},
              {&s->d_zNi, 4 * W_FP * nn},
+             {&s->d_pwsig, 4 * (lsgk::POW_SIG_STATE + 2 * W_FP) * nn},
+             {&s->d_pwmap, 4 * (lsgk::POW_MAP_STATE + 2 * W_FP) * 2 * nn},
              {&s->binv_lv[0], 4 * W_FP * binv_lv_words(2 * nn)},
              {&s->binv_iv[0], 4 * W_FP * binv_iv_words(2 * nn)},
              {&s->binv_lv[1], 4 * W_FP * binv_lv_words(nn)},
@@ -701,6 +705,20 @@
 
 static bool binv_block_on() { return lsg_ab_long("LSG_BINV_BLOCK", 1) != 0; }
 static bool fp2_lanes_on() { return lsg_ab_long("LSG_FP2_LANES", 1) != 0; }
+lsgk::PowLanes pow_lanes(const DevBuf& b, size_t items, size_t state) {
+  lsgk::PowLanes pw;
+  if (lsg_ab_long("LSG_POW_LANES", LSG_POW_LANES_DEFAULT) == 0 || b.cap < 4 * (state + 2 * W_FP) * items) return pw;
+  pw.min_items = (int)std::max(1L, std::min(lsg_ab_long("LSG_POW_LANES_MIN", LSG_POW_LANES_MIN_DEFAULT), 0x7fffffffL));
+  pw.state = P_<uint32_t>(b);
+  pw.pa = pw.state + state * items;
+  pw.pb = pw.pa + W_FP * items;
+  return pw;
+}
+#define KL_POW(s, pw, items)                                          \
+  do {                                                                \
+    if ((pw).on((int)(items))) KL(s, "k_fp_pow_lanes", hipSuccess);   \
+  } while (0)
+
 int launch_sig_subgroup(Slot* s, int n) {
   if (fp2_lanes_on())
     KL(s, "k_sig_subgroup", lsgk::sig_subgroup(S_(s), n, P_<uint32_t>(s->d_sigaff), P_<uint8_t>(s->d_siginf),
@@ -771,7 +789,9 @@
 int launch_hash(Slot* s, int n, uint32_t* H, uint8_t* hinf) {
   KL(s, "k_h2c_prep", lsgk::h2c_prep(S_(s), n, P_<uint8_t>(s->d_ub), P_<uint32_t>(s->d_U), P_<uint32_t>(s->d_nrm)));
   LSG_RC(batch_inv(s, 0, "binv_sswu", P_<uint32_t>(s->d_nrm), 2 * (size_t)n, P_<uint32_t>(s->d_nrmi)));
-  KL(s, "k_h2c_map", lsgk::h2c_map(S_(s), n, P_<uint32_t>(s->d_U), P_<uint32_t>(s->d_nrmi), P_<uint32_t>(s->d_Hp)));
+  const lsgk::PowLanes pw = pow_lanes(s->d_pwmap, 2 * (size_t)n, lsgk::POW_MAP_STATE);
+  KL(s, "k_h2c_map", lsgk::h2c_map(S_(s), n, P_<uint32_t>(s->d_U), P_<uint32_t>(s->d_nrmi), P_<uint32_t>(s->d_Hp), pw));
+  KL_POW(s, pw, 2 * (size_t)n);
   if ((size_t)n <= slp_items_max()) {
     KL(s, "k_slp_h2c", lsg_slp_h2c_clear(S_(s), n, P_<uint32_t>(s->d_Hp), H, hinf));
     return LSG_OK;
@@ -959,8 +979,10 @@
                                      P_<uint32_t>(s->d_zP), P_<uint8_t>(s->d_pinf)));
   LSG_RC(batch_inv(s, 1, "binv_pk", P_<uint32_t>(s->d_zP), (size_t)n, P_<uint32_t>(s->d_zPi)));
   KL(s, "k_pk_affine", lsgk::pk_affine(S_(s), n, P_<uint32_t>(s->d_Pp), P_<uint32_t>(s->d_zPi), P_<uint32_t>(s->d_P)));
+  const lsgk::PowLanes pw = pow_lanes(s->d_pwsig, (size_t)n, lsgk::POW_SIG_STATE);
   KL(s, "k_sig_decode", lsgk::sig_decode(S_(s), n, P_<uint8_t>(s->d_sig), P_<uint32_t>(s->d_siglen),
-                                         P_<uint32_t>(s->d_sigaff), P_<uint8_t>(s->d_siginf), P_<int32_t>(s->d_seterr)));
+                                         P_<uint32_t>(s->d_sigaff), P_<uint8_t>(s->d_siginf), P_<int32_t>(s->d_seterr), pw));
+  KL_POW(s, pw, n);
   if ((size_t)n <= slp_items_max())
     KL(s, "k_slp_subgroup", lsg_slp_g2_subgroup(S_(s), n, P_<uint32_t>(s->d_sigaff), P_<uint8_t>(s->d_siginf),
                                                 P_<int32_t>(s->d_seterr)));
@@ -3161,8 +3183,10 @@
   LSG_RC(stage_sets(s, sp.data(), n, 0, false));
   LSG_RC(size_state(s, n, 0, 1, 0));
   const int nn = (int)n;
+  const lsgk::PowLanes pw = pow_lanes(s->d_pwsig, n, lsgk::POW_SIG_STATE);
   KL(s, "k_sig_decode", lsgk::sig_decode(S_(s), nn, P_<uint8_t>(s->d_sig), P_<uint32_t>(s->d_siglen),
-                                         P_<uint32_t>(s->d_sigaff), P_<uint8_t>(s->d_siginf), P_<int32_t>(s->d_seterr)));
+                                         P_<uint32_t>(s->d_sigaff), P_<uint8_t>(s->d_siginf), P_<int32_t>(s->d_seterr), pw));
+  KL_POW(s, pw, nn);
   if (validate) LSG_RC(launch_sig_subgroup(s, nn));
   return LSG_OK;
 }
@@ -3491,6 +3515,31 @@
   return check_lanes(c, in, n, out, false, true);
 }
 
+static int check_pow(lsg_ctx* c, int32_t id, const uint32_t* in, size_t n, uint32_t* out, bool lanes) {
+  if (!c || id < 0 || id > 2 || (n && (!in || !out)) || n > 0x7fffffffull / (4 * W_FP)) return LSG_ERR_INVALID_ARG;
+  LSG_ENTER(c);
+  if (n == 0) return LSG_OK;
+  Slot* s = &c->dev[0]->util;
+  timer_reset(s);
+  LSG_RC(ensure(s, s->d_aux, 4 * W_FP * n));
+  LSG_RC(ensure(s, s->d_Fb, 4 * W_FP * n));
+  LSG_HIP(s, hipMemcpyAsync(s->d_aux.p, in, 4 * W_FP * n, hipMemcpyHostToDevice, s->st[0]));
+  if (lanes)
+    KL(s, "k_fp_pow_lanes", lsgk::fp_pow_lanes(S_(s), (int)n, id, P_<uint32_t>(s->d_aux), P_<uint32_t>(s->d_Fb)));
+  else
+    KL(s, "k_check_pow_pair", lsgk::check_pow_pair(S_(s), (int)n, id, P_<uint32_t>(s->d_aux), P_<uint32_t>(s->d_Fb)));
+  LSG_HIP(s, hipMemcpyAsync(out, s->d_Fb.p, 4 * W_FP * n, hipMemcpyDeviceToHost, s->st[0]));
+  LSG_HIP(s, hipStreamSynchronize(s->st[0]));
+  keep_times(s);
+  return LSG_OK;
+}
+int lsg_check_pow_lanes(lsg_ctx* c, int32_t id, const uint32_t* in, size_t n, uint32_t* out) {
+  return check_pow(c, id, in, n, out, true);
+}
+int lsg_check_pow_pair(lsg_ctx* c, int32_t id, const uint32_t* in, size_t n, uint32_t* out) {
+  return check_pow(c, id, in, n, out, false);
+}
+
 int lsg_check_canon(lsg_ctx* c, const uint32_t* in, size_t n, const uint8_t* bytes48, size_t nb, uint32_t* out,
                     uint32_t* out_limbs) {
   constexpr size_t WOUT = lsgk::CHECK_CANON_OUT;
diff --git a/lodestar_amd/csrc/lsg_k_hash.hip b/lodestar_amd/csrc/lsg_k_hash.hip
--- a/lodestar_amd/csrc/lsg_k_hash.hip
+++ b/lodestar_amd/csrc/lsg_k_hash.hip
@@ -144,6 +144,39 @@
   if ((item & 1) == 0) lane_store(Hp, item >> 1, g2_add(q, o));
 }
 
+static_assert(lane_words<sswu_mid_t>() == lsgk::POW_MAP_STATE, "layout: map stage state");
+__global__ void LSG_KERNEL_ATTR_W(LSG_H2C_WAVES) k_h2c_map_a(int n2, const uint32_t* __restrict__ U, const uint32_t* __restrict__ ninv,
+                                                             uint32_t* __restrict__ state, uint32_t* __restrict__ pa) {
+  LANE_ITEM(n2);
+  (void)lead;
+  const sswu_mid_t m = sswu_stage_a(lane_load<fp2_t>(U, item), lane_load<fp_t>(ninv, item));
+  lane_store(state, item, m);
+  lane_store(pa, item, fp2_norm(m.gx1));
+}
+__global__ void LSG_KERNEL_ATTR_W(LSG_H2C_WAVES) k_h2c_map_b(int n2, const uint32_t* __restrict__ U, uint32_t* __restrict__ state,
+                                                             uint32_t* __restrict__ pa, const uint32_t* __restrict__ pb) {
+  LANE_ITEM(n2);
+  (void)lead;
+  sswu_mid_t m = lane_load<sswu_mid_t>(state, item);
+  fp2_t x, gx;
+  const fp_t c = sswu_stage_b(x, gx, m, lane_load<fp2_t>(U, item), lane_load<fp_t>(pa, item), lane_load<fp_t>(pb, item));
+  m.x1 = x;
+  m.gx1 = gx;
+  lane_store(state, item, m);
+  lane_store(pa, item, c);
+}
+__global__ void LSG_KERNEL_ATTR_W(LSG_H2C_WAVES) k_h2c_map_c(int n2, const uint32_t* __restrict__ U, const uint32_t* __restrict__ state,
+                                                             const uint32_t* __restrict__ pa, const uint32_t* __restrict__ pb,
+                                                             uint32_t* __restrict__ Hp) {
+  LANE_ITEM(n2);
+  (void)lead;
+  const sswu_mid_t m = lane_load<sswu_mid_t>(state, item);
+  const g2p_t q = iso_map3(sswu_stage_c(lane_load<fp2_t>(U, item), m.x1, m.gx1, lane_load<fp_t>(pa, item),
+                                        lane_load<fp_t>(pb, item)));
+  const g2p_t o = quad_swap_pairs(q);
+  if ((item & 1) == 0) lane_store(Hp, item >> 1, g2_add(q, o));
+}
+
 template <bool LANES>
 LSG_DEVI void h2c_clear_item(uint32_t* park, int n, uint32_t* __restrict__ Hp, uint32_t* __restrict__ zN,
                              uint8_t* __restrict__ hinf) {
@@ -294,8 +327,19 @@
 hipError_t h2c_prep(hipStream_t st, int n, const uint8_t* ub, uint32_t* U, uint32_t* norms) {
   LSG_LAUNCH_ITEMS(k_h2c_prep, n, st, n, ub, U, norms);
 }
-hipError_t h2c_map(hipStream_t st, int n, const uint32_t* U, const uint32_t* ninv, uint32_t* Hp) {
-  LSG_LAUNCH_ITEMS(k_h2c_map, 2 * n, st, 2 * n, U, ninv, Hp);
+hipError_t h2c_map(hipStream_t st, int n, const uint32_t* U, const uint32_t* ninv, uint32_t* Hp, const PowLanes& pw) {
+  if (n <= 0) return hipSuccess;
+  const int n2 = 2 * n;
+  if (!pw.on(n2)) LSG_LAUNCH_ITEMS(k_h2c_map, n2, st, n2, U, ninv, Hp);
+  const dim3 grid(lane_blocks((size_t)n2)), block(LSG_TPB);
+  hipLaunchKernelGGL(k_h2c_map_a, grid, block, 0, st, n2, U, ninv, pw.state, pw.pa);
+  hipError_t e = fp_pow_lanes(st, n2, LSG_POW_SQRT, pw.pa, pw.pb);
+  if (e != hipSuccess) return e;
+  hipLaunchKernelGGL(k_h2c_map_b, grid, block, 0, st, n2, U, pw.state, pw.pa, pw.pb);
+  e = fp_pow_lanes(st, n2, LSG_POW_SQRT34, pw.pa, pw.pb);
+  if (e != hipSuccess) return e;
+  hipLaunchKernelGGL(k_h2c_map_c, grid, block, 0, st, n2, U, pw.state, pw.pa, pw.pb, Hp);
+  return hipGetLastError();
 }
 hipError_t h2c_clear(hipStream_t st, int n, uint32_t* Hp, uint32_t* zN, uint8_t* hinf, bool pair_form) {
 #ifdef LSG_FP2_LANES
diff --git a/lodestar_amd/csrc/lsg_k_reduce.hip b/lodestar_amd/csrc/lsg_k_reduce.hip
--- a/lodestar_amd/csrc/lsg_k_reduce.hip
+++ b/lodestar_amd/csrc/lsg_k_reduce.hip
@@ -392,6 +392,22 @@
   o[56 + (lead ? 0 : 1)] = lead ? f : 0u;
 }
 
+#ifndef LSG_POW_LANES_WAVES
+#define LSG_POW_LANES_WAVES 2
+#endif
+__global__ void LSG_KERNEL_ATTR_W(LSG_POW_LANES_WAVES) k_fp_pow_lanes(int n, int id, const uint32_t* __restrict__ in,
+                                                                      uint32_t* __restrict__ out) {
+  const size_t i = gtid();
+  if (i >= (size_t)n) return;
+  id = __builtin_amdgcn_readfirstlane(id);
+  lanes_fp_store(out, i, lanes_pow_plan(lanes_fp_load(in, i), id));
+}
+__global__ void LSG_KERNEL_ATTR k_check_pow_pair(int n, int id, const uint32_t* __restrict__ in, uint32_t* __restrict__ out) {
+  LANE_ITEM(n);
+  (void)lead;
+  lane_store(out, item, fp_pow_id(lane_load<fp_t>(in, item), id));
+}
+
 __global__ void LSG_KERNEL_ATTR k_probe_fp_mul(int n, int iters, uint32_t* __restrict__ io) {
   LANE_ITEM(n);
   (void)lead;
@@ -494,6 +510,17 @@
 hipError_t check_fp2_roots(hipStream_t st, int n, const uint32_t* in, uint32_t* out) {
   LSG_LAUNCH_ITEMS(k_check_fp2_roots, n, st, n, in, out);
 }
+hipError_t fp_pow_lanes(hipStream_t st, int n, int id, const uint32_t* in, uint32_t* out) {
+  if (n <= 0) return hipSuccess;
+  if (id < 0 || id > 2) return hipErrorInvalidValue;
+  hipLaunchKernelGGL(k_fp_pow_lanes, dim3((unsigned)(((size_t)n + LSG_TPB - 1) / LSG_TPB)), dim3(LSG_TPB), 0, st, n, id,
+                     in, out);
+  return hipGetLastError();
+}
+hipError_t check_pow_pair(hipStream_t st, int n, int id, const uint32_t* in, uint32_t* out) {
+  if (id < 0 || id > 2) return hipErrorInvalidValue;
+  LSG_LAUNCH_ITEMS(k_check_pow_pair, n, st, n, id, in, out);
+}
 hipError_t probe_fp_mul(hipStream_t st, int items, int iters, uint32_t* io) {
   LSG_LAUNCH_ITEMS(k_probe_fp_mul, items, st, items, iters, io);
 }
diff --git a/lodestar_amd/csrc/lsg_k_sig.hip b/lodestar_amd/csrc/lsg_k_sig.hip
--- a/lodestar_amd/csrc/lsg_k_sig.hip
+++ b/lodestar_amd/csrc/lsg_k_sig.hip
@@ -19,6 +19,77 @@
   lane_store(sig_aff, item, p);
   if (lead) {
     inf[item] = is_inf ? 1 : 0;
+    err[item] = e;
+  }
+}
+
+struct sigdec_state_t {
+  fp2_t x, rhs;
+  uint32_t w;
+};
+static_assert(lane_words<sigdec_state_t>() == lsgk::POW_SIG_STATE, "layout: decode stage state");
+__global__ void LSG_KERNEL_ATTR k_sig_decode_a(int n, const uint8_t* __restrict__ sig, const uint32_t* __restrict__ sig_len,
+                                               uint32_t* __restrict__ sig_aff, uint8_t* __restrict__ inf,
+                                               int32_t* __restrict__ err, uint32_t* __restrict__ state,
+                                               uint32_t* __restrict__ pa) {
+  LANE_ITEM(n);
+  uint32_t len = sig_len[item];
+  g2a_t p;
+  p.x = fp2_zero();
+  p.y = fp2_zero();
+  sigdec_state_t s;
+  s.x = fp2_zero();
+  s.rhs = fp2_zero();
+  s.w = 0;
+  fp_t pw = fp_zero();
+  bool is_inf = false;
+  int e;
+  if (len == 96) {
+    bool want = false;
+    e = g2_uncompress_parse(p, is_inf, s.x, s.rhs, want, sig + 192 * item);
+    if (e == LSG_UNCOMPRESS_PENDING) {
+      s.w = 1u | (want ? 2u : 0u);
+      pw = fp2_norm(s.rhs);
+    }
+  } else if (len == 192)
+    e = g2_deserialize_uncompressed(p, is_inf, sig + 192 * item);
+  else
+    e = LSG_BLST_INVALID_SIZE;
+  lane_store(state, item, s);
+  lane_store(pa, item, pw);
+  if (e == LSG_UNCOMPRESS_PENDING) return;
+  lane_store(sig_aff, item, p);
+  if (lead) {
+    inf[item] = is_inf ? 1 : 0;
+    err[item] = e;
+  }
+}
+__global__ void LSG_KERNEL_ATTR k_sig_decode_b(int n, uint32_t* __restrict__ state, uint32_t* __restrict__ pa,
+                                               const uint32_t* __restrict__ pb) {
+  LANE_ITEM(n);
+  (void)lead;
+  sigdec_state_t s = lane_load<sigdec_state_t>(state, item);
+  if (!(s.w & 1u)) return;
+  const fp_t cand = lane_load<fp_t>(pb, item);
+  if (fp_is_root_of(cand, lane_load<fp_t>(pa, item))) s.w |= 4u;
+  lane_store(pa, item, fp2_sqrt_root_c(s.rhs, cand));
+  lane_store(state, item, s);
+}
+__global__ void LSG_KERNEL_ATTR k_sig_decode_c(int n, const uint32_t* __restrict__ state, const uint32_t* __restrict__ pa,
+                                               const uint32_t* __restrict__ pb, uint32_t* __restrict__ sig_aff,
+                                               uint8_t* __restrict__ inf, int32_t* __restrict__ err) {
+  LANE_ITEM(n);
+  const sigdec_state_t s = lane_load<sigdec_state_t>(state, item);
+  if (!(s.w & 1u)) return;
+  fp2_t y;
+  const bool root = fp2_sqrt_root_finish(y, s.rhs, lane_load<fp_t>(pa, item), lane_load<fp_t>(pb, item));
+  g2a_t p;
+  p.x = fp2_zero();
+  p.y = fp2_zero();
+  const int e = g2_uncompress_finish(p, s.x, y, (s.w & 4u) != 0 && root, (s.w & 2u) != 0);
+  lane_store(sig_aff, item, p);
+  if (lead) {
+    inf[item] = 0;
     err[item] = e;
   }
 }
@@ -175,8 +246,18 @@
 
 namespace lsgk {
 hipError_t sig_decode(hipStream_t st, int n, const uint8_t* sig, const uint32_t* sig_len, uint32_t* sig_aff,
-                      uint8_t* inf, int32_t* err) {
-  LSG_LAUNCH_ITEMS(k_sig_decode, n, st, n, sig, sig_len, sig_aff, inf, err);
+                      uint8_t* inf, int32_t* err, const PowLanes& pw) {
+  if (n <= 0) return hipSuccess;
+  if (!pw.on(n)) LSG_LAUNCH_ITEMS(k_sig_decode, n, st, n, sig, sig_len, sig_aff, inf, err);
+  const dim3 grid(lane_blocks((size_t)n)), block(LSG_TPB);
+  hipLaunchKernelGGL(k_sig_decode_a, grid, block, 0, st, n, sig, sig_len, sig_aff, inf, err, pw.state, pw.pa);
+  hipError_t e = fp_pow_lanes(st, n, LSG_POW_SQRT, pw.pa, pw.pb);
+  if (e != hipSuccess) return e;
+  hipLaunchKernelGGL(k_sig_decode_b, grid, block, 0, st, n, pw.state, pw.pa, pw.pb);
+  e = fp_pow_lanes(st, n, LSG_POW_SQRT34, pw.pa, pw.pb);
+  if (e != hipSuccess) return e;
+  hipLaunchKernelGGL(k_sig_decode_c, grid, block, 0, st, n, pw.state, pw.pa, pw.pb, sig_aff, inf, err);
+  return hipGetLastError();
 }
 hipError_t sig_subgroup(hipStream_t st, int n, const uint32_t* sig_aff, const uint8_t* inf, int32_t* err, bool pair_form) {
 #ifdef LSG_FP2_LANES
diff --git a/lodestar_amd/csrc/lsg_launch.h b/lodestar_amd/csrc/lsg_launch.h
--- a/lodestar_amd/csrc/lsg_launch.h
+++ b/lodestar_amd/csrc/lsg_launch.h
@@ -6,10 +6,19 @@
 constexpr uint32_t LSG_MC_ROW = 0x80000000u;
 
 namespace lsgk {
+struct PowLanes {
+  int min_items = 0;
+  uint32_t* state = nullptr;
+  uint32_t* pa = nullptr;
+  uint32_t* pb = nullptr;
+  bool on(int items) const { return min_items > 0 && items >= min_items && state && pa && pb; }
+};
+constexpr size_t POW_SIG_STATE = 4 * 14 + 2, POW_MAP_STATE = 10 * 14;
 hipError_t expand_msg(hipStream_t st, int n, const uint8_t* msg, const uint32_t* off, const uint32_t* len,
                       const uint8_t* dst, uint32_t dst_len, uint8_t* ub);
 hipError_t h2c_prep(hipStream_t st, int n, const uint8_t* ub, uint32_t* U, uint32_t* norms);
-hipError_t h2c_map(hipStream_t st, int n, const uint32_t* U, const uint32_t* ninv, uint32_t* Hp);
+hipError_t h2c_map(hipStream_t st, int n, const uint32_t* U, const uint32_t* ninv, uint32_t* Hp,
+                   const PowLanes& pw = PowLanes());
 hipError_t h2c_clear(hipStream_t st, int n, uint32_t* Hp, uint32_t* zN, uint8_t* hinf, bool pair_form = false);
 hipError_t h2c_gather(hipStream_t st, int n, const uint32_t* mid, const uint32_t* Hm, const uint8_t* hinfm, uint32_t* H,
                       uint8_t* hinf);
@@ -31,7 +40,7 @@
 hipError_t msg_roots(hipStream_t st, int n, uint8_t* msg, const uint32_t* off, uint32_t* len);
 
 hipError_t sig_decode(hipStream_t st, int n, const uint8_t* sig, const uint32_t* sig_len, uint32_t* sig_aff,
-                      uint8_t* inf, int32_t* err);
+                      uint8_t* inf, int32_t* err, const PowLanes& pw = PowLanes());
 hipError_t sig_subgroup(hipStream_t st, int n, const uint32_t* sig_aff, const uint8_t* inf, int32_t* err,
                         bool pair_form = false);
 hipError_t sig_prep(hipStream_t st, int n, const uint32_t* sig_aff, const uint8_t* inf, const int32_t* err,
@@ -115,6 +124,8 @@
 hipError_t blobs_to_fp12(hipStream_t st, int n, const uint8_t* blobs, uint32_t* out);
 hipError_t fp12_to_canon(hipStream_t st, int n, const uint32_t* in, uint8_t* out576);
 hipError_t fp12_pow_u64(hipStream_t st, const uint8_t* in576, uint64_t r, uint8_t* out576);
+hipError_t fp_pow_lanes(hipStream_t st, int n, int id, const uint32_t* in, uint32_t* out);
+hipError_t check_pow_pair(hipStream_t st, int n, int id, const uint32_t* in, uint32_t* out);
 hipError_t probe_fp_mul(hipStream_t st, int items, int iters, uint32_t* io);
 hipError_t check_fp2_mul(hipStream_t st, int n, const uint32_t* in, uint32_t* out);
 hipError_t check_fp_sqr(hipStream_t st, int n, const uint32_t* in, uint32_t* out);
diff --git a/lodestar_amd/csrc/lsg_tower.hpp b/lodestar_amd/csrc/lsg_tower.hpp
--- a/lodestar_amd/csrc/lsg_tower.hpp
+++ b/lodestar_amd/csrc/lsg_tower.hpp
@@ -312,22 +312,29 @@
   return fp_is_zero(c1) ? fp_canon_gt_half(c0) : fp_canon_gt_half(c1);
 }
 
+LSG_INL bool fp_is_root_of(const fp_t& s, const fp_t& n) { return fp_eq(fp_sqr(s), n); }
 LSG_INL fp_t fp2_norm_sqrt_candidate(const fp2_t& a, bool* is_sq) {
   fp_t n = fp2_norm(a);
   fp_t s = fp_pow_id(n, LSG_POW_SQRT);
-  *is_sq = fp_eq(fp_sqr(s), n);
+  *is_sq = fp_is_root_of(s, n);
   return s;
 }
-LSG_BIGFN bool fp2_sqrt_with_norm_root(fp2_t& out, fp2_t a, fp_t s) {
+LSG_INL fp_t fp2_sqrt_root_c(const fp2_t& a, const fp_t& s) {
   fp_t c = fp_mul(fp_add(a.c0, s), fp_t(FP_HALF));
-  c = fp_select(fp_is_zero(c), a.c0, c);
-  fp_t t = fp_pow_id(c, LSG_POW_SQRT34);
+  return fp_select(fp_is_zero(c), a.c0, c);
+}
+LSG_BIGFN bool fp2_sqrt_root_finish(fp2_t& out, fp2_t a, fp_t c, fp_t t) {
   fp_t ct = fp_mul(c, t);
   bool c_sq = fp_eq(fp_mul(ct, t), fp_one()) || fp_is_zero(c);
   fp_t h = fp_mul(fp_mul(a.c1, t), fp_t(FP_HALF));
   fp2_t r = c_sq ? fp2_t(ct, h) : fp2_t(h, fp_neg(ct));
   out = r;
   return fp2_eq(fp2_sqr(r), a);
+}
+LSG_BIGFN bool fp2_sqrt_with_norm_root(fp2_t& out, fp2_t a, fp_t s) {
+  fp_t c = fp2_sqrt_root_c(a, s);
+  fp_t t = fp_pow_id(c, LSG_POW_SQRT34);
+  return fp2_sqrt_root_finish(out, a, c, t);
 }
 LSG_BIGFN bool fp2_sqrt(fp2_t& out, fp2_t a) {
   bool ok;
```

Result: faster. 3.949 million, median of 6 (+2.4%).
